# LCSL/nys-koop-lqr

Hardware: AMD Instinct MI355X
Metric: Nyström-Koopman fits/sec (K_nm build + A,B,C solve), N=1e5 m=2000 d=384 (higher is better)
Workload: dtype f64

## Files before the change

include/nyskoop.h:

```cpp
#ifndef NYSKOOP_H
#define NYSKOOP_H

#include <stdint.h>

#ifdef __cplusplus
extern "C" {
#endif

#define NK_ABI_VERSION 2

enum {
  NK_OK = 0,
  NK_ERR_BAD_ARG = -1,
  NK_ERR_HIP = -2,
  NK_ERR_NOT_SPD = -3,
  NK_ERR_OOM = -4,
  NK_ERR_NO_CONVERGENCE = -5,
  NK_ERR_NO_DEVICE = -6
};

enum { NK_KERNEL_RBF = 0, NK_KERNEL_MATERN52 = 1, NK_KERNEL_LINEAR = 2, NK_KERNEL_TPS = 3 };

typedef struct nk_kernel_desc {
  int32_t type;
  int32_t d;
  int32_t n_lengthscale;
  int32_t reserved;
  const double* lengthscale;
  double sigma0;
} nk_kernel_desc;

typedef struct nk_fit_stats {
  double ms_total;
  double ms_upload;
  double ms_kmat;
  double ms_gram;
  double ms_sqrt;
  double ms_solve;
  double ms_gram_kernel_avg;
  int32_t gram_kernel_launches;
  int32_t sqrt_iters;
  double sqrt_residual;
  double gram_flops;
  double kmat_pairs;
  int32_t rank_inner;
  int32_t rank_inner_rec;
  double pivot_ratio_inner;
  double pivot_ratio_inner_rec;
  int32_t refined;
  int32_t reserved_;
  double refine_ratio_inner;
  double refine_ratio_inner_rec;
} nk_fit_stats;

typedef struct nk_ctx nk_ctx;
typedef struct nk_model nk_model;

int nk_version(void);
const char* nk_last_error(void);
int nk_device_count(void);
int nk_create(int device, nk_ctx** out);
int nk_destroy(nk_ctx* ctx);
int nk_synchronize(nk_ctx* ctx);
void* nk_stream(nk_ctx* ctx);
int nk_set_kmat_mode(nk_ctx* ctx, int mode);
int nk_set_strict_spd(nk_ctx* ctx, int strict);
int nk_set_refine(nk_ctx* ctx, double pivot_ratio, int32_t steps);
#define NK_DTYPE_F64 0
#define NK_DTYPE_F32 1
int nk_set_compute_dtype(nk_ctx* ctx, int dtype);
int nk_wait_stream(nk_ctx* ctx, void* producer_stream);
int nk_group_create(int device, int size, nk_ctx** members);
typedef struct nk_cv_unit {
  const nk_kernel_desc* kernel;
  double gamma;
  double jitter;
  int32_t m;
  int32_t reserved;
  int64_t test_begin, test_end;
  const int64_t* landmark_rows;
} nk_cv_unit;
int nk_cv_grid(nk_ctx* const* members, int32_t n_members, const double* X, int64_t ldx, const double* Y, int64_t ldy,
               int64_t n, int32_t d, int32_t p, const nk_cv_unit* units, int32_t n_units, double* scores, int32_t* status);
typedef struct nk_spline_cv_unit {
  double gamma;
  int32_t m;
  int32_t reserved;
  int64_t test_begin, test_end;
  const double* centers;
} nk_spline_cv_unit;
int nk_spline_cv_grid(nk_ctx* const* members, int32_t n_members, const double* X, int64_t ldx, const double* Y,
                      int64_t ldy, int64_t n, int32_t d, int32_t p, const nk_spline_cv_unit* units, int32_t n_units,
                      double* scores, int32_t* status);
typedef struct nk_sysid_unit {
  const nk_kernel_desc* kernel;
  double gamma, jitter;
  int32_t m, n_ranges;
  const int64_t* row_ranges;
  const int64_t* landmark_rows;
  const double* centers;
  const int32_t* traj;
  int32_t n_traj, reserved;
} nk_sysid_unit;
int nk_sysid_grid(nk_ctx* const* members, int32_t n_members, const double* X, int64_t ldx, const double* Y, int64_t ldy,
                  int64_t n, int32_t d, int32_t p, const double* trajs, const double* U, int32_t n_trajs, int32_t T,
                  const nk_sysid_unit* units, int32_t n_units, double* err_abs, double* err_rel, int32_t* status);
int nk_group_enter(nk_ctx* member);
int nk_group_leave(nk_ctx* member);
int nk_group_stats(nk_ctx* member, uint64_t* out4);
int nk_runtime_counters(uint64_t* out, int32_t n);
int nk_shutdown(void);

void* nk_host_alloc(uint64_t bytes);
void nk_host_free(void* ptr);

int nk_kernel_matrix(nk_ctx* ctx, const nk_kernel_desc* kd,
                     const double* A, int64_t lda, int64_t nA,
                     const double* B, int64_t ldb, int64_t nB,
                     double* out, int64_t ldo);

int nk_nystrom_fit(nk_ctx* ctx, const nk_kernel_desc* kd,
                   const double* X, int64_t ldx, const double* Y, int64_t ldy,
                   int64_t n, int32_t d, int32_t p,
                   const int64_t* row_ranges, int32_t n_ranges,
                   const double* Zin, int64_t ldzi, const double* Zout, int64_t ldzo, int32_t m,
                   double gamma, double jitter,
                   nk_model** model, nk_fit_stats* stats);

int nk_gram_doubles(int32_t m, int32_t d, int32_t p, int64_t* count);
int nk_nystrom_gram(nk_ctx* ctx, const nk_kernel_desc* kd,
                    const double* X, int64_t ldx, const double* Y, int64_t ldy,
                    int64_t n, int32_t d, int32_t p,
                    const int64_t* row_ranges, int32_t n_ranges,
                    const double* Zin, int64_t ldzi, const double* Zout, int64_t ldzo, int32_t m,
                    double* gram, nk_fit_stats* stats);
// ... 100 lines not shown
```

nys_koop_lqr_amd/_lib.py:

```python
import atexit
import ctypes as C
import os
import sys
import threading

import numpy as np

_HERE = os.path.dirname(os.path.abspath(__file__))

NK_KERNEL_RBF, NK_KERNEL_MATERN52, NK_KERNEL_LINEAR, NK_KERNEL_TPS = 0, 1, 2, 3
NK_PLANT_DUFFING, NK_PLANT_DOUBLE_INTEGRATOR, NK_PLANT_HJB = 0, 1, 2
NK_OK = 0
_ERR_NAMES = {-1: "NK_ERR_BAD_ARG", -2: "NK_ERR_HIP", -3: "NK_ERR_NOT_SPD", -4: "NK_ERR_OOM",
              -5: "NK_ERR_NO_CONVERGENCE", -6: "NK_ERR_NO_DEVICE"}


class NyskoopError(RuntimeError):
    def __init__(self, code, msg):
        super().__init__(f"{_ERR_NAMES.get(code, code)}: {msg}")
        self.code = code


class KernelDesc(C.Structure):
    _fields_ = [("type", C.c_int32), ("d", C.c_int32), ("n_lengthscale", C.c_int32), ("reserved", C.c_int32),
                ("lengthscale", C.POINTER(C.c_double)), ("sigma0", C.c_double)]


class CvUnit(C.Structure):
    _fields_ = [("kernel", C.POINTER(KernelDesc)), ("gamma", C.c_double), ("jitter", C.c_double), ("m", C.c_int32),
                ("reserved", C.c_int32), ("test_begin", C.c_int64), ("test_end", C.c_int64),
                ("landmark_rows", C.POINTER(C.c_int64))]


class SplineCvUnit(C.Structure):
    _fields_ = [("gamma", C.c_double), ("m", C.c_int32), ("reserved", C.c_int32), ("test_begin", C.c_int64),
                ("test_end", C.c_int64), ("centers", C.POINTER(C.c_double))]


class SysidUnit(C.Structure):
    _fields_ = [("kernel", C.POINTER(KernelDesc)), ("gamma", C.c_double), ("jitter", C.c_double), ("m", C.c_int32),
                ("n_ranges", C.c_int32), ("row_ranges", C.POINTER(C.c_int64)), ("landmark_rows", C.POINTER(C.c_int64)),
                ("centers", C.POINTER(C.c_double)), ("traj", C.POINTER(C.c_int32)), ("n_traj", C.c_int32),
                ("reserved", C.c_int32)]


class PlantUnit(C.Structure):
    _fields_ = [("model", C.c_void_p), ("K", C.c_void_p), ("x0", C.c_void_p), ("x_ref", C.c_void_p),
                ("uopt", C.c_int32), ("reserved", C.c_int32)]


class DareProblem(C.Structure):
    _fields_ = [("m", C.c_int32), ("p", C.c_int32), ("A", C.c_void_p), ("lda", C.c_int64), ("B", C.c_void_p),
                ("ldb", C.c_int64), ("Q", C.c_void_p), ("ldq", C.c_int64), ("R", C.c_void_p), ("ldr", C.c_int64),
                ("out_K", C.c_void_p), ("out_P", C.c_void_p), ("out_delta", C.c_void_p)]


class FitStats(C.Structure):
    _fields_ = [("ms_total", C.c_double), ("ms_upload", C.c_double), ("ms_kmat", C.c_double),
                ("ms_gram", C.c_double), ("ms_sqrt", C.c_double), ("ms_solve", C.c_double),
                ("ms_gram_kernel_avg", C.c_double), ("gram_kernel_launches", C.c_int32),
                ("sqrt_iters", C.c_int32), ("sqrt_residual", C.c_double), ("gram_flops", C.c_double),
                ("kmat_pairs", C.c_double), ("rank_inner", C.c_int32), ("rank_inner_rec", C.c_int32),
                ("pivot_ratio_inner", C.c_double), ("pivot_ratio_inner_rec", C.c_double), ("refined", C.c_int32),
                ("reserved_", C.c_int32), ("refine_ratio_inner", C.c_double), ("refine_ratio_inner_rec", C.c_double)]

    def as_dict(self):
        return {k: getattr(self, k) for k, _ in self._fields_}


_P = C.c_void_p
_I64 = C.c_int64
_I32 = C.c_int32
_D = C.c_double

SIGNATURES = {
    "nk_version": (C.c_int, []),
    "nk_last_error": (C.c_char_p, []),
    "nk_device_count": (C.c_int, []),
    "nk_create": (C.c_int, [C.c_int, C.POINTER(_P)]),
    "nk_destroy": (C.c_int, [_P]),
    "nk_synchronize": (C.c_int, [_P]),
    "nk_stream": (_P, [_P]),
    "nk_set_kmat_mode": (C.c_int, [_P, C.c_int]),
    "nk_set_strict_spd": (C.c_int, [_P, C.c_int]),
    "nk_set_refine": (C.c_int, [_P, C.c_double, C.c_int32]),
    "nk_wait_stream": (C.c_int, [_P, _P]),
    "nk_shutdown": (C.c_int, []),
    "nk_group_create": (C.c_int, [C.c_int, C.c_int, C.POINTER(_P)]),
    "nk_group_enter": (C.c_int, [_P]),
    "nk_group_leave": (C.c_int, [_P]),
    "nk_set_compute_dtype": (C.c_int, [_P, C.c_int]),
    "nk_group_stats": (C.c_int, [_P, C.POINTER(C.c_uint64)]),
    "nk_runtime_counters": (C.c_int, [C.POINTER(C.c_uint64), C.c_int32]),
    "nk_cv_grid": (C.c_int, [C.POINTER(_P), _I32, _P, _I64, _P, _I64, _I64, _I32, _I32, C.POINTER(CvUnit), _I32,
                             C.POINTER(_D), C.POINTER(_I32)]),
    "nk_spline_cv_grid": (C.c_int, [C.POINTER(_P), _I32, _P, _I64, _P, _I64, _I64, _I32, _I32, C.POINTER(SplineCvUnit),
                                    _I32, C.POINTER(_D), C.POINTER(_I32)]),
    "nk_sysid_grid": (C.c_int, [C.POINTER(_P), _I32, _P, _I64, _P, _I64, _I64, _I32, _I32, _P, _P, _I32, _I32,
                                C.POINTER(SysidUnit), _I32, C.POINTER(_D), C.POINTER(_D), C.POINTER(_I32)]),
    "nk_host_alloc": (_P, [C.c_uint64]),
    "nk_host_free": (None, [_P]),
    "nk_kernel_matrix": (C.c_int, [_P, C.POINTER(KernelDesc), _P, _I64, _I64, _P, _I64, _I64, _P, _I64]),
    "nk_nystrom_fit": (C.c_int, [_P, C.POINTER(KernelDesc), _P, _I64, _P, _I64, _I64, _I32, _I32,
                                 C.POINTER(_I64), _I32, _P, _I64, _P, _I64, _I32, _D, _D,
                                 C.POINTER(_P), C.POINTER(FitStats)]),
    "nk_gram_doubles": (C.c_int, [_I32, _I32, _I32, C.POINTER(_I64)]),
    "nk_nystrom_gram": (C.c_int, [_P, C.POINTER(KernelDesc), _P, _I64, _P, _I64, _I64, _I32, _I32,
                                  C.POINTER(_I64), _I32, _P, _I64, _P, _I64, _I32, _P, C.POINTER(FitStats)]),
    "nk_nystrom_solve": (C.c_int, [_P, C.POINTER(KernelDesc), _P, _I64, _P, _I64, _I32, _I32, _I32, _P, _I64, _D, _D,
                                   C.POINTER(_P), C.POINTER(FitStats)]),
    "nk_model_create": (C.c_int, [_P, C.POINTER(KernelDesc), _P, _I64, _I32, _I32, _I32, _D, _P, _P, _P, _P,
                                  C.POINTER(_P)]),
    "nk_spline_fit": (C.c_int, [_P, _P, _I64, _P, _I64, _I64, _I32, _I32, C.POINTER(_I64), _I32, _P, _I64, _I32, _D,
                                C.POINTER(_P), C.POINTER(FitStats)]),
    "nk_spline_model_create": (C.c_int, [_P, _P, _I64, _I32, _I32, _I32, _P, _P, _P, _P, C.POINTER(_P)]),
    "nk_model_destroy": (C.c_int, [_P]),
    "nk_model_get": (C.c_int, [_P, _P, C.c_char, _P, _I64]),
    "nk_model_dims": (C.c_int, [_P, C.POINTER(_I32), C.POINTER(_I32), C.POINTER(_I32)]),
    "nk_model_get_ops": (C.c_int, [_P, _P, _P, _I64, _P, _I64, _P, _I64]),
    "nk_model_get_ops_async": (C.c_int, [_P, _P, _P, _I64, _P, _I64, _P, _I64]),
    "nk_model_wait": (C.c_int, [_P]),
    "nk_lift": (C.c_int, [_P, _P, _P, _I64, _I64, _P, _I64]),
    "nk_predict": (C.c_int, [_P, _P, _P, _I64, _I64, _P, _I64]),
    "nk_score_neg_rmse": (C.c_int, [_P, _P, _P, _I64, _P, _I64, _I64, C.POINTER(_D)]),
    "nk_rollout": (C.c_int, [_P, _P, _P, _I64, _P, _I32, _I32, _P, _P]),
    "nk_rollout_err": (C.c_int, [_P, _P, _P, _P, _I32, _I32, C.POINTER(_D), C.POINTER(_D)]),
    "nk_closed_loop": (C.c_int, [_P, _P, _P, _P, _P, _I32, _P, _P]),
    "nk_closed_loop_batch": (C.c_int, [_P, _P, _P, _P, _P, _I32, _I32, _P, _P]),
    "nk_plant_step": (C.c_int, [C.c_int, _D, _P, _P, _P]),
    "nk_plant_loop": (C.c_int, [_P, _P, C.c_int, _D, _P, _P, _P, _I32, _I32, _P, _P]),
    "nk_plant_loop_multi": (C.c_int, [_P, C.c_int, _D, _I32, C.POINTER(PlantUnit), _I32, _P, _I32, _P, _P, _P]),
    "nk_dare_batch": (C.c_int, [_P, C.POINTER(DareProblem), _I32, _D, _I32, C.POINTER(_I32), C.POINTER(_I32)]),
    "nk_model_lqr_gain_batch": (C.c_int, [_P, C.POINTER(_P), _I32, _D, _P, _D, _I32, _P, C.POINTER(_I32),
                                          C.POINTER(_I32)]),
    "nk_model_lqr_cost": (C.c_int, [_P, _P, _D, _P, _I64]),
    "nk_linear_rollout": (C.c_int, [_P, _P, _P, _P, _I32, _I32, _I32, _P, _P, _I32, _I32, _P, _P]),
    "nk_gemm_f32": (C.c_int, [_P, _I64, _I64, _I64, _P, _I64, _P, _I64, _P, _I64]),
    "nk_gemm": (C.c_int, [_P, C.c_int, C.c_int, _I64, _I64, _I64, _D, _P, _I64, _P, _I64, _D, _P, _I64]),
    "nk_sqrtm_spd": (C.c_int, [_P, _P, _I64, _I32, _P, _P, C.POINTER(_I32), C.POINTER(_D)]),
    "nk_solve_spd": (C.c_int, [_P, _P, _I64, _I32, _P, _I64, _I32, _P, _I64]),
    "nk_bench_gram": (C.c_int, [_P, _I64, _I32, _I32, _I32, _I32, C.POINTER(_D), C.POINTER(_D)]),
    "nk_chol_aug": (C.c_int, [_P, _I32, _P, _P, _P, _P, _P, _P, _P, _P, _P]),
}

_lib = None
_lib_lock = threading.Lock()

# ... 553 lines not shown
```

nys_koop_lqr_amd/csrc/nk_api.hip:

```cpp
#include "nk_common.h"
#include "nk_api_internal.h"

#include <cmath>
#include <cstdarg>
#include <cstdio>
#include <cstring>
#include <cstdlib>
#include <algorithm>
#include <mutex>
#include <set>

namespace nk {

static thread_local std::string g_err;

void set_error(const char* fmt, ...) {
  char buf[1024];
  va_list ap;
  va_start(ap, fmt);
  vsnprintf(buf, sizeof(buf), fmt, ap);
  va_end(ap);
  g_err = buf;
}

// ... 279 lines not shown
      NK_TRY(launch_gemm(ctx, false, true, len, d, p, 1.0, Xaug + r0 * ldx + d, ldx, mdl->W + m, m + p, 1.0,
                         out + r0 * ldo, ldo));
  }
  arena_release(ctx, mk);
  return NK_OK;
}


float ev_ms(nk_ctx* ctx, int a, int b) {
  float ms = 0.f;
  (void)hipEventElapsedTime(&ms, ctx->ev[a], ctx->ev[b]);
  return ms;
}


int small_reserve(nk_ctx* ctx, size_t bytes) {
  if (ctx->h_stage_bytes >= bytes) return NK_OK;
  if (ctx->h_stage) (void)hipHostFree(ctx->h_stage);
  ctx->h_stage = nullptr;
  ctx->h_stage_bytes = 0;
  NK_HIP(hipHostMalloc(reinterpret_cast<void**>(&ctx->h_stage), bytes, hipHostMallocDefault));
  ctx->h_stage_bytes = bytes;
  return NK_OK;
}
const double* small_in(SmallStage& st, const double* host, int64_t ld, int64_t rows, int64_t cols) {
  double* dst = reinterpret_cast<double*>(reinterpret_cast<char*>(st.ctx->h_stage) + st.off);
  for (int64_t r = 0; r < rows; ++r) memcpy(dst + r * cols, host + r * ld, (size_t)cols * 8);
  st.off += (((size_t)rows * cols * 8) + 255) & ~(size_t)255;
  return dst;
}
double* small_out(SmallStage& st, double* user, int64_t user_ld, int64_t rows, int64_t cols) {
  double* dst = reinterpret_cast<double*>(reinterpret_cast<char*>(st.ctx->h_stage) + st.off);
  st.off += (((size_t)rows * cols * 8) + 255) & ~(size_t)255;
  st.outs.push_back(SmallStage::Out{dst, user, user_ld, rows, cols});
  return dst;
}
void small_finish(SmallStage& st) {
  for (auto& o : st.outs)
    for (int64_t r = 0; r < o.rows; ++r) memcpy(o.user + r * o.user_ld, o.stage + r * o.cols, (size_t)o.cols * 8);
}

}

using namespace nk;

extern "C" {

int nk_version(void) { return NK_ABI_VERSION; }

const char* nk_last_error(void) { return g_err.c_str(); }

int nk_device_count(void) {
  int n = 0;
  if (hipGetDeviceCount(&n) != hipSuccess) {
    (void)hipGetLastError();
    return 0;
  }
  return n;
}

int nk_create(int device, nk_ctx** out) {
  NK_REQUIRE(out != nullptr, "nk_create: null output pointer");
  *out = nullptr;
  int n = nk_device_count();
  if (n <= 0) {
    set_error("no HIP device visible: libnyskoop has no CPU fallback");
    return NK_ERR_NO_DEVICE;
  }
  NK_REQUIRE(device >= 0 && device < n, "nk_create: device %d out of range (0..%d)", device, n - 1);
  NK_HIP(hipSetDevice(device));
  hipDeviceProp_t prop;
  NK_HIP(hipGetDeviceProperties(&prop, device));
  if (strncmp(prop.gcnArchName, "gfx950", 6) != 0) {
    set_error("device %d is %s; libnyskoop is built for gfx950 (MI355X) only", device, prop.gcnArchName);
    return NK_ERR_NO_DEVICE;
  }
  nk_ctx* ctx = new nk_ctx();
  ctx->device = device;
  ctx->num_cu = prop.multiProcessorCount;
  int prio_lo = 0, prio_hi = 0;
  NK_HIP(hipDeviceGetStreamPriorityRange(&prio_lo, &prio_hi));
  const int prio_mid = (prio_lo - prio_hi >= 2) ? (prio_lo + prio_hi) / 2 : prio_hi;
  NK_HIP(hipStreamCreateWithPriority(&ctx->stream_main, hipStreamNonBlocking, prio_mid));
  NK_HIP(hipStreamCreateWithPriority(&ctx->stream_side, hipStreamNonBlocking, prio_lo));
  NK_HIP(hipStreamCreateWithPriority(&ctx->stream_prep, hipStreamNonBlocking, prio_hi));
  NK_HIP(hipStreamCreateWithFlags(&ctx->stream_copy, hipStreamNonBlocking));
  NK_HIP(hipStreamCreateWithPriority(&ctx->stream_la[0], hipStreamNonBlocking, prio_hi));
  NK_HIP(hipStreamCreateWithPriority(&ctx->stream_la[1], hipStreamNonBlocking, prio_mid));
  for (int q = 0; q < 2; ++q)
    for (int i = 0; i < 4; ++i) NK_HIP(hipEventCreateWithFlags(&ctx->ev_la[q][i], hipEventDisableTiming));
  ctx->stream = ctx->stream_main;
  ctx->cur_arena = &ctx->arena;
  NK_HIP(hipEventCreateWithFlags(&ctx->ev_fork, hipEventDisableTiming));
  NK_HIP(hipEventCreateWithFlags(&ctx->ev_join, hipEventDisableTiming));
  NK_HIP(hipEventCreateWithFlags(&ctx->ev_chain, hipEventDisableTiming));
  NK_HIP(hipMalloc(reinterpret_cast<void**>(&ctx->d_info), 256));
  ctx->d_piv = reinterpret_cast<unsigned long long*>(ctx->d_info + 16);
  NK_HIP(hipMalloc(reinterpret_cast<void**>(&ctx->d_scalars), 64 * sizeof(double)));
  NK_HIP(hipHostMalloc(reinterpret_cast<void**>(&ctx->h_scalars), 64 * sizeof(double), hipHostMallocMapped | hipHostMallocCoherent));
  NK_HIP(hipHostMalloc(reinterpret_cast<void**>(&ctx->h_info), 256, hipHostMallocMapped | hipHostMallocCoherent));
  ctx->h_piv = reinterpret_cast<unsigned long long*>(ctx->h_info + 16);
  for (int i = 0; i < EV_COUNT; ++i) NK_HIP(hipEventCreate(&ctx->ev[i]));
  NK_HIP(hipEventCreateWithFlags(&ctx->ev_ext, hipEventDisableTiming));
  for (int i = 0; i < 8; ++i) NK_HIP(hipEventCreateWithFlags(&ctx->ev_up[i], hipEventDisableTiming));
  const char* km = getenv("NYSKOOP_KMAT");
  ctx->kmat_mode = (km && strcmp(km, "direct") == 0) ? 1 : 0;
  const char* st = getenv("NYSKOOP_STRICT_SPD");
  ctx->strict_spd = (st && atoi(st) != 0) ? 1 : 0;
  if (const char* rp = getenv("NYSKOOP_REFINE_PIVOT")) ctx->refine_pivot = atof(rp);
  if (const char* rs = getenv("NYSKOOP_REFINE_STEPS")) ctx->refine_steps = std::max(0, atoi(rs));
  {
    std::lock_guard<std::mutex> lk(g_reg_mu);
    g_ctxs.insert(ctx);
  }
  *out = ctx;
  return NK_OK;
}

static void destroy_ctx_unregistered(nk_ctx* ctx) {
  (void)hipSetDevice(ctx->device);
  if (tl_ctx == ctx) tl_ctx = nullptr;
  group_detach(ctx);
  (void)hipStreamSynchronize(ctx->stream_main);
  (void)hipStreamSynchronize(ctx->stream_side);
  (void)hipStreamSynchronize(ctx->stream_prep);
  (void)hipStreamSynchronize(ctx->stream_copy);
  for (int q = 0; q < 2; ++q) {
    if (ctx->stream_la[q]) { (void)hipStreamSynchronize(ctx->stream_la[q]); (void)hipStreamDestroy(ctx->stream_la[q]); }
    for (int i = 0; i < 4; ++i) if (ctx->ev_la[q][i]) (void)hipEventDestroy(ctx->ev_la[q][i]);
  }
  for (auto& c : ctx->arena.chunks) (void)hipFree(c.base);
  for (auto& c : ctx->arena_side.chunks) (void)hipFree(c.base);
  (void)hipEventDestroy(ctx->ev_fork);
  (void)hipEventDestroy(ctx->ev_join);
  if (ctx->ev_chain) (void)hipEventDestroy(ctx->ev_chain);
  if (ctx->ev_ext) (void)hipEventDestroy(ctx->ev_ext);
  for (int i = 0; i < 8; ++i) if (ctx->ev_up[i]) (void)hipEventDestroy(ctx->ev_up[i]);
  (void)hipStreamDestroy(ctx->stream_side);
  (void)hipStreamDestroy(ctx->stream_prep);
  (void)hipStreamDestroy(ctx->stream_copy);
  (void)hipFree(ctx->d_info);
  for (int i = 0; i < 2; ++i) if (ctx->d_flow[i]) (void)hipFree(ctx->d_flow[i]);
  (void)hipFree(ctx->d_scalars);
  if (ctx->d_zeros) (void)hipFree(ctx->d_zeros);
  if (ctx->h_stage) (void)hipHostFree(ctx->h_stage);
  (void)hipHostFree(ctx->h_scalars);
  (void)hipHostFree(ctx->h_info);
  for (int i = 0; i < EV_COUNT; ++i) (void)hipEventDestroy(ctx->ev[i]);
  (void)hipStreamDestroy(ctx->stream_main);
  delete ctx;
}

int nk_destroy(nk_ctx* ctx) {
  if (!ctx) return NK_OK;
  {
    std::lock_guard<std::mutex> lk(g_reg_mu);
    if (g_ctxs.erase(ctx) == 0) return NK_OK;
  }
  destroy_ctx_unregistered(ctx);
  return NK_OK;
}

static int model_wait_unchecked(nk_model* mdl);
static void destroy_model_unregistered(nk_model* model, bool to_pool) {
  (void)model_wait_unchecked(model);
  if (to_pool) {
    pool_give(model->device, model->bytes, model->buf);
// ... 705 lines not shown
```

nys_koop_lqr_amd/csrc/nk_chol_flow.hip:

```cpp
#include <cstdio>
#include <cstdlib>

#include "nk_common.h"
#include "nk_panel_body.h"
#include "nk_potrf_body.h"

namespace nk {

namespace {

constexpr int FLOW_THREADS = 256;
constexpr int FLOW_HDR = 16;
constexpr int FLOW_POLL_LIMIT = 1 << 22;

struct FlowSys {
  double* P;
  int64_t ldp;
  int m, extra;
  double* Linv;
  double* pivlog;
  int* info;
  unsigned long long* piv;
  int* flags;
  int nblk;
  int nex;
};
struct FlowArgs {
  FlowSys s[2];
  int nsys;
  int total;
  int fix;
  int test_giveup;
  int* hdr;
};

__device__ __forceinline__ int ld_flag(const int* f) { return __hip_atomic_load(f, __ATOMIC_RELAXED, __HIP_MEMORY_SCOPE_AGENT); }

__device__ __forceinline__ int col_items(const FlowSys& s, int c) {
  if (c < 0 || c >= s.nblk) return 0;
  return max(0, s.nblk - c - 2) + s.nex;
}

__device__ void item_of(const FlowArgs& a, int t, int& q, int& i, int& k) {
  for (int g = 0;; ++g) {
    for (int p = 0; p < a.nsys; ++p)
      if (g < a.s[p].nblk) {
        if (t == 0) { q = p; i = k = g; return; }
        --t;
      }
    for (int p = 0; p < a.nsys; ++p) {
      const int n = col_items(a.s[p], g - 1);
      if (t < n) {
        q = p; k = g - 1;
        const int nsq = max(0, a.s[p].nblk - k - 2);
        i = t < nsq ? k + 2 + t : a.s[p].nblk + (t - nsq);
        return;
      }
      t -= n;
    }
  }
}

__device__ __forceinline__ void tile_rows(const FlowSys& s, int i, int& r0, int& r1) {
  if (i < s.nblk) { r0 = CHOL_NB * i; r1 = min(r0 + CHOL_NB, s.m); }
  else { r0 = s.m + CHOL_NB * (i - s.nblk); r1 = min(r0 + CHOL_NB, s.m + s.extra); }
}

typedef d4 Quarter[2][2];

__device__ __forceinline__ void load_quarter(const FlowSys& s, int r0, int r1, int c0, int c1, int wm, int wn, int l15, int l4,
                                             Quarter& C) {
#pragma unroll
  for (int a = 0; a < 2; ++a)
#pragma unroll
    for (int b = 0; b < 2; ++b)
#pragma unroll
      for (int reg = 0; reg < 4; ++reg) {
        const int row = r0 + 32 * wm + 16 * a + l4 + 4 * reg, col = c0 + 32 * wn + 16 * b + l15;
        C[a][b][reg] = (row < r1 && col < c1) ? s.P[(int64_t)row * s.ldp + col] : 0.0;
      }
}
__device__ __forceinline__ void store_quarter(const FlowSys& s, int r0, int r1, int c0, int c1, int wm, int wn, int l15, int l4,
                                              const Quarter& C) {
#pragma unroll
  for (int a = 0; a < 2; ++a)
#pragma unroll
    for (int b = 0; b < 2; ++b)
#pragma unroll
      for (int reg = 0; reg < 4; ++reg) {
        const int row = r0 + 32 * wm + 16 * a + l4 + 4 * reg, col = c0 + 32 * wn + 16 * b + l15;
        if (row < r1 && col < c1) s.P[(int64_t)row * s.ldp + col] = C[a][b][reg];
      }
}

__device__ __forceinline__ void update_quarter(const FlowSys& s, int r0, int r1, int c0, int c1, int j, int wm, int wn, int l15,
                                               int l4, Quarter& C) {
  const double* pa[2];
  const double* pb[2];
#pragma unroll
  for (int a = 0; a < 2; ++a) {
    pa[a] = s.P + (int64_t)min(r0 + 32 * wm + 16 * a + l15, r1 - 1) * s.ldp + CHOL_NB * j + 8 * l4;
    pb[a] = s.P + (int64_t)min(c0 + 32 * wn + 16 * a + l15, c1 - 1) * s.ldp + CHOL_NB * j + 8 * l4;
  }
  d4 acc[2][2];
#pragma unroll
  for (int a = 0; a < 2; ++a)
#pragma unroll
    for (int b = 0; b < 2; ++b) acc[a][b] = d4{0.0, 0.0, 0.0, 0.0};
#pragma unroll
  for (int h = 0; h < 2; ++h) {
    double x[2][8], y[2][8];
#pragma unroll
    for (int a = 0; a < 2; ++a)
#pragma unroll
      for (int ks = 0; ks < 8; ++ks) {
        x[a][ks] = pa[a][32 * h + ks];
        y[a][ks] = pb[a][32 * h + ks];
      }
#pragma unroll
    for (int ks = 0; ks < 8; ++ks)
#pragma unroll
      for (int a = 0; a < 2; ++a)
#pragma unroll
        for (int b = 0; b < 2; ++b) acc[a][b] = __builtin_amdgcn_mfma_f64_16x16x4f64(x[a][ks], y[b][ks], acc[a][b], 0, 0, 0);
  }
#pragma unroll
  for (int a = 0; a < 2; ++a)
#pragma unroll
    for (int b = 0; b < 2; ++b)
#pragma unroll
      for (int reg = 0; reg < 4; ++reg) C[a][b][reg] -= acc[a][b][reg];
  asm volatile("" ::: "memory");
}

__device__ __forceinline__ void give_up(const FlowArgs& a) {
  __hip_atomic_store(a.hdr + 1, 1, __ATOMIC_RELAXED, __HIP_MEMORY_SCOPE_AGENT);
  for (int q = 0; q < a.nsys; ++q) atomicExch(a.s[q].info, CHOL_FLOW_GIVEUP);
}

__device__ int wait_tiles(const FlowArgs& a, const FlowSys& s, int ia, int ib, int jlo, int jhi, int* sh) {
  if (threadIdx.x < 64) {
    const int lane = threadIdx.x;
    int res = -1;
    for (int polls = 0;; ++polls) {
      const int j = jlo + lane;
      bool ok = true;
      if (j < jhi) {
        ok = ld_flag(s.flags + ia * s.nblk + j) != 0;
        if (ib >= 0) ok = ok && ld_flag(s.flags + ib * s.nblk + j) != 0;
      }
      const unsigned long long ready = __ballot(ok);
      const int run = ~ready == 0ull ? 64 : __builtin_ctzll(~ready);
      if (run > 0) { res = min(jlo + run, jhi); break; }
      if (ld_flag(a.hdr + 1) != 0) break;
      if (polls >= FLOW_POLL_LIMIT) {
        if (lane == 0) give_up(a);
        break;
      }
      __builtin_amdgcn_s_sleep(2);
    }
    if (lane == 0) {
      if (res > 0) __builtin_amdgcn_fence(__ATOMIC_ACQUIRE, "agent");
      asm volatile("s_waitcnt vmcnt(0)" ::: "memory");
      sh[0] = res;
    }
  }
  __syncthreads();
  const int r = sh[0];
  __syncthreads();
  return r;
}

__device__ __forceinline__ void publish(const FlowSys& s, int i, int k) {
  asm volatile("s_waitcnt vmcnt(0)" ::: "memory");
  __syncthreads();
  if (threadIdx.x == 0) {
    __builtin_amdgcn_fence(__ATOMIC_RELEASE, "agent");
    asm volatile("s_waitcnt vmcnt(0)" ::: "memory");
    __hip_atomic_store(s.flags + i * s.nblk + k, 1, __ATOMIC_RELAXED, __HIP_MEMORY_SCOPE_AGENT);
  }
}

__device__ __forceinline__ void local_sync() {
  asm volatile("s_waitcnt vmcnt(0)" ::: "memory");
  __syncthreads();
}

__device__ __forceinline__ void panel_tile(const FlowArgs& a, const FlowSys& s, int r0, int r1, int k, int wave, int lane) {
  PanelSys ps;
  ps.P = s.P + (int64_t)r0 * s.ldp + CHOL_NB * k;
  ps.ldp = s.ldp;
  ps.Linv = s.Linv + (size_t)k * CHOL_WS;
  ps.rows = r1 - r0;
  ps.nb = min(CHOL_NB, s.m - CHOL_NB * k);
  ps.fix = a.fix;
  ps.nblocks = 1;
  chol_panel_rows(ps, 16 * wave, lane);
  __builtin_amdgcn_s_setprio(0);
}

__device__ __noinline__ void flow_potrf(double* A, int64_t lda, int nb, double* Linv, int* info, unsigned long long* piv,
                                       double* plog, int blk, int lane) {
  PotrfBatch pb;
  pb.A[0] = A; pb.lda[0] = lda; pb.nb[0] = nb; pb.Linv[0] = Linv; pb.info[0] = info; pb.piv[0] = piv; pb.plog[0] = plog;
  pb.A[1] = nullptr; pb.lda[1] = 0; pb.nb[1] = 0; pb.Linv[1] = nullptr; pb.info[1] = nullptr; pb.piv[1] = nullptr;
  pb.plog[1] = nullptr;
  potrf_diag_kernel_body<true>(pb, blk, 0, lane);
  __builtin_amdgcn_s_setprio(0);
}

__global__ void __launch_bounds__(FLOW_THREADS) chol_flow_kernel(FlowArgs a) {
  __shared__ int sh[4];
  const int lane = threadIdx.x & 63;
  const int wave = __builtin_amdgcn_readfirstlane(threadIdx.x >> 6);
  const int wm = wave >> 1, wn = wave & 1;
  const int l15 = lane & 15, l4 = lane >> 4;
  for (;;) {
    if (threadIdx.x == 0) sh[1] = atomicAdd(a.hdr, 1);
    __syncthreads();
    const int t = sh[1];
    __syncthreads();
    if (t >= a.total) return;
    if (t == a.test_giveup) {
      if (threadIdx.x == 0) give_up(a);
      return;
    }
    int q = 0, i = 0, k = 0;
    item_of(a, t, q, i, k);
    const FlowSys s = q ? a.s[1] : a.s[0];
    int r0, r1;
    tile_rows(s, i, r0, r1);
    const int c0 = CHOL_NB * k, c1 = min(c0 + CHOL_NB, s.m);
    if (i == k) {
      if (k > 0) {
        const int p0 = c0 - CHOL_NB;
        Quarter Cp, Cd;
        load_quarter(s, r0, r1, p0, c0, wm, wn, l15, l4, Cp);
        load_quarter(s, r0, r1, c0, c1, wm, wn, l15, l4, Cd);
        bool ok = true;
        for (int j = 0; j < k - 1 && ok;) {
          const int J = wait_tiles(a, s, k, k - 1, j, k - 1, sh);
          if (J < 0) { ok = false; break; }
          for (; j < J; ++j) {
            update_quarter(s, r0, r1, p0, c0, j, wm, wn, l15, l4, Cp);
            update_quarter(s, r0, r1, c0, c1, j, wm, wn, l15, l4, Cd);
          }
        }
        if (!ok) continue;
        store_quarter(s, r0, r1, p0, c0, wm, wn, l15, l4, Cp);
        store_quarter(s, r0, r1, c0, c1, wm, wn, l15, l4, Cd);
        local_sync();
        if (wait_tiles(a, s, k - 1, -1, k - 1, k, sh) < 0) continue;
        panel_tile(a, s, r0, r1, k - 1, wave, lane);
        publish(s, k, k - 1);
        __syncthreads();
        load_quarter(s, r0, r1, c0, c1, wm, wn, l15, l4, Cd);
        update_quarter(s, r0, r1, c0, c1, k - 1, wm, wn, l15, l4, Cd);
        store_quarter(s, r0, r1, c0, c1, wm, wn, l15, l4, Cd);
        local_sync();
      }
      if (wave == 0)
        flow_potrf(s.P + (int64_t)c0 * s.ldp + c0, s.ldp, c1 - c0, s.Linv + (size_t)k * CHOL_WS, s.info, s.piv,
                   s.pivlog ? s.pivlog + c0 : nullptr, k, lane);
      publish(s, k, k);
      __syncthreads();
    } else {
      if (k > 0) {
        Quarter C;
        load_quarter(s, r0, r1, c0, c1, wm, wn, l15, l4, C);
        bool ok = true;
        for (int j = 0; j < k && ok;) {
          const int J = wait_tiles(a, s, i, k, j, k, sh);
          if (J < 0) { ok = false; break; }
          for (; j < J; ++j) update_quarter(s, r0, r1, c0, c1, j, wm, wn, l15, l4, C);
        }
        if (!ok) continue;
        store_quarter(s, r0, r1, c0, c1, wm, wn, l15, l4, C);
        local_sync();
      }
      if (wait_tiles(a, s, k, -1, k, k + 1, sh) < 0) continue;
      panel_tile(a, s, r0, r1, k, wave, lane);
      publish(s, i, k);
      __syncthreads();
    }
  }
}

}

bool chol_flow_enabled() {
  const char* e = getenv("NYSKOOP_CHOL_FLOW");
  return !(e && e[0] == '0');
}

static int flow_test_giveup(const CholSys* sys, int nsys, int total) {
  const char* e = getenv("NYSKOOP_CHOL_FLOW_TEST_GIVEUP");
  if (!e || !e[0]) return -1;
  long ticket = -1, want_nsys = 0, want_extra = 0;
  if (sscanf(e, "%ld,%ld,%ld", &ticket, &want_nsys, &want_extra) < 1) return -1;
  if (want_nsys > 0 && want_nsys != nsys) return -1;
  if (want_extra > 0 && want_extra != sys[0].extra) return -1;
  return (ticket >= 0 && ticket < total) ? (int)ticket : -1;
}

int cholesky_flow_pair(nk_ctx* ctx, const CholSys* sys, int nsys) {
  constexpr int NB = CHOL_NB;
  NK_REQUIRE(nsys >= 1 && nsys <= 2, "cholesky_flow_pair: 1..2 systems");
  FlowArgs a;
  memset(&a, 0, sizeof(a));
  a.nsys = nsys;
  a.fix = chol_fix_enabled();
  size_t words = FLOW_HDR;
  for (int q = 0; q < nsys; ++q) {
    const CholSys& y = sys[q];
    FlowSys& s = a.s[q];
    s.P = y.P; s.ldp = y.ldp; s.m = y.m; s.extra = y.extra; s.Linv = y.Linv; s.pivlog = y.pivlog;
    s.info = ctx->d_info + info_base(ctx) + q;
    s.piv = ctx->d_piv + 2 * (info_base(ctx) + q);
    s.nblk = (y.m + NB - 1) / NB;
    s.nex = (y.extra + NB - 1) / NB;
    words += (size_t)(s.nblk + s.nex) * s.nblk;
    for (int c = 0; c < s.nblk; ++c) a.total += 1 + std::max(0, s.nblk - c - 2) + s.nex;
  }
  const int slot = info_base(ctx) / 2;
  if (ctx->flow_words[slot] < words) {
    if (ctx->d_flow[slot]) NK_HIP(hipFree(ctx->d_flow[slot]));
    ctx->d_flow[slot] = nullptr;
    ctx->flow_words[slot] = 0;
    NK_HIP(hipMalloc(reinterpret_cast<void**>(&ctx->d_flow[slot]), words * sizeof(int)));
    ctx->flow_words[slot] = words;
  }
  a.test_giveup = flow_test_giveup(sys, nsys, a.total);
  a.hdr = ctx->d_flow[slot];
  int* f = a.hdr + FLOW_HDR;
  for (int q = 0; q < nsys; ++q) {
    a.s[q].flags = f;
    f += (size_t)(a.s[q].nblk + a.s[q].nex) * a.s[q].nblk;
  }
  NK_HIP(hipMemsetAsync(a.hdr, 0, words * sizeof(int), ctx->stream));
  const int grid = std::max(1, std::min(a.total, ctx->num_cu / 2));
  hipLaunchKernelGGL(chol_flow_kernel, dim3((unsigned)grid), dim3(FLOW_THREADS), 0, ctx->stream, a);
  NK_HIP(hipGetLastError());
  count_event(CNT_CHOL_FLOW);
  return NK_OK;
}

}
```

nys_koop_lqr_amd/csrc/nk_common.h:

```cpp
#pragma once
#include <hip/hip_runtime.h>
#include <stdint.h>
#include <stddef.h>
#include <string>
#include <vector>

#include "nyskoop.h"
#include "nk_lockstep.h"

namespace nk {

void set_error(const char* fmt, ...);

#define NK_HIP(call)                                                                         \
  do {                                                                                       \
    hipError_t e_ = (call);                                                                  \
    if (e_ != hipSuccess) {                                                                  \
      nk::set_error("%s failed: %s (%s:%d)", #call, hipGetErrorString(e_), __FILE__, __LINE__); \
      return e_ == hipErrorOutOfMemory ? NK_ERR_OOM : NK_ERR_HIP;                            \
    }                                                                                        \
  } while (0)

#define NK_TRY(call)            \
  do {                          \
    int rc_ = (call);           \
    if (rc_ != NK_OK) return rc_; \
  } while (0)

#define NK_REQUIRE(cond, ...)     \
  do {                            \
    if (!(cond)) {                \
      nk::set_error(__VA_ARGS__); \
      return NK_ERR_BAD_ARG;      \
    }                             \
  } while (0)

struct ArenaChunk {
  char* base = nullptr;
  size_t cap = 0;
  size_t off = 0;
};
struct Arena {
  std::vector<ArenaChunk> chunks;
  int cur = 0;
};
struct ArenaMark {
  int chunk;
  size_t off;
};

}

enum {
  EV_FIT_BEGIN = 0,
  EV_STAGED = 1,
  EV_KMAT_DONE = 2,
  EV_GRAM_DONE = 3,
  EV_SOLVE_BEGIN = 4,
  EV_FIT_END = 5,
  EV_SQRT_BEGIN = 6,
  EV_SQRT_END = 7,
  EV_LANDMARKS = 8,
  EV_SQRT_PREPARED = 9,
  EV_SQRT_RESID = 10,
  EV_SQRT_SCALARS = 11,
  EV_FORK = 12,
  EV_YPREP_DONE = 13,
  EV_GEMM_T0 = 14,
  EV_GEMM_T1 = 15,
  EV_COUNT = 16
};

struct nk_member_state;
struct nk_ctx {
  int device = 0;
  hipStream_t stream = nullptr;
  hipStream_t stream_main = nullptr;
  hipStream_t stream_side = nullptr;
  hipStream_t stream_copy = nullptr;
  hipStream_t stream_prep = nullptr;
  nk::Arena arena;
  nk::Arena arena_side;
  nk::Arena* cur_arena = nullptr;
  hipStream_t stream_la[2] = {nullptr, nullptr};
  hipEvent_t ev_la[2][4] = {};
  int compute_f32 = 0;
  hipEvent_t ev_fork = nullptr, ev_join = nullptr, ev_chain = nullptr;
  int* d_info = nullptr;
  unsigned long long* d_piv = nullptr;
  unsigned long long* h_piv = nullptr;
  double* d_scalars = nullptr;
  double* h_scalars = nullptr;
  int* h_info = nullptr;
  double* d_zeros = nullptr;
  hipEvent_t ev[EV_COUNT];
  int num_cu = 256;
  int kmat_mode = 0;
  double refine_pivot = 0.0;
  int refine_steps = 2;
  int strict_spd = 0;
  hipEvent_t ev_ext = nullptr;
  hipEvent_t ev_up[8] = {};
  nk_group* group = nullptr;
  nk_member_state* gstate = nullptr;
  int* d_flow[2] = {nullptr, nullptr};
  size_t flow_words[2] = {0, 0};
  bool spline_defer_svd = false;
  bool chol_flow_off = false;
  double* h_stage = nullptr;
  size_t h_stage_bytes = 0;
};

enum { NK_MODEL_NYSTROM = 0, NK_MODEL_SPLINE = 1 };
struct nk_model {
  int device = 0;
  int32_t m = 0, d = 0, p = 0;
  int32_t ktype = 0;
  double sigma0 = 0.0;
  double jitter = 0.0;
  double* buf = nullptr;
  size_t bytes = 0;
  double *A = nullptr, *B = nullptr, *C = nullptr, *W = nullptr, *S = nullptr, *Sinv = nullptr, *Z = nullptr,
         *winv = nullptr;
  bool has_ops = false;
  int32_t kind = 0;
  hipEvent_t ev_fetch = nullptr;
};

namespace nk {

struct SideScope {
  nk_ctx* c;
  hipStream_t s0;
  Arena* a0;
  explicit SideScope(nk_ctx* ctx, hipStream_t s = nullptr) : c(ctx), s0(ctx->stream), a0(ctx->cur_arena) {
    c->stream = s ? s : c->stream_side;
    c->cur_arena = &c->arena_side;
  }
  ~SideScope() {
    c->stream = s0;
    c->cur_arena = a0;
  }
};

struct ChainOnly {
  nk_ctx* c;
  bool b0;
  explicit ChainOnly(nk_ctx* ctx) : c(ctx), b0(ctx->chol_flow_off) { c->chol_flow_off = true; }
  ~ChainOnly() { c->chol_flow_off = b0; }
};

inline int info_base(const nk_ctx* c) { return c->stream != c->stream_main ? 2 : 0; }

// ... 51 lines not shown
  if ((0x000fffff & (2 + hx)) < 3) {
    if (f == 0.0) return k == 0 ? 0.0 : dk * ln2_hi + dk * ln2_lo;
    const double R = f * f * (0.5 - 0.33333333333333333 * f);
    return k == 0 ? f - R : dk * ln2_hi - ((R - dk * ln2_lo) - f);
  }
  const double s = f / (2.0 + f);
  const double z = s * s;
  const double w = z * z;
  const double t1 = w * (Lg2 + w * (Lg4 + w * Lg6));
  const double t2 = z * (Lg1 + w * (Lg3 + w * (Lg5 + w * Lg7)));
  const double R = t2 + t1;
  if (((hx - 0x6147a) | (0x6b851 - hx)) > 0) {
    const double hfsq = 0.5 * f * f;
    return k == 0 ? f - (hfsq - s * (hfsq + R)) : dk * ln2_hi - ((hfsq - (s * (hfsq + R) + dk * ln2_lo)) - f);
  }
  return k == 0 ? f - s * (f - R) : dk * ln2_hi - ((s * (f - R) - dk * ln2_lo) - f);
}
__host__ __device__ __forceinline__ double tps_value(double r2) {
#pragma clang fp contract(off)
  return r2 > 0.0 ? r2 * log_pos(sqrt(r2)) : 0.0;
}

nk_group* group_new(int device, int size);
void group_attach(nk_group* g, int slot, nk_ctx* c);
void group_detach(nk_ctx* c);
int group_enter(nk_ctx* c);
int group_leave(nk_ctx* c);
void group_stats(nk_ctx* c, uint64_t out[4]);
enum { CNT_CHAIN_GIVEUP = 0, CNT_JACOBI_GIVEUP = 1, CNT_RANK_TRUNCATED = 2, CNT_SQRT_RETRY = 3, CNT_REFINED = 4,
       CNT_CHOL_FLOW_GIVEUP = 5, CNT_CHOL_FLOW = 6, CNT_N = 7 };
void count_event(int which);
uint64_t read_counter(int which);
hipError_t real_stream_sync(hipStream_t s);
hipError_t real_event_sync(hipEvent_t e);

int arena_reset(nk_ctx* ctx);
ArenaMark arena_mark(nk_ctx* ctx);
void arena_release(nk_ctx* ctx, ArenaMark mk);
int arena_alloc(nk_ctx* ctx, size_t bytes, void** out);
template <typename T>
inline int arena_alloc_t(nk_ctx* ctx, size_t count, T** out) {
  return arena_alloc(ctx, count * sizeof(T), reinterpret_cast<void**>(out));
}
bool is_device_ptr(const void* p);

int launch_kmat(nk_ctx* ctx, int ktype, const double* A, int64_t lda, int64_t nA, const double* B, int64_t ldb,
                int64_t nB, int d, const double* winv, double sigma0, double* out, int64_t ldo);

enum { TRI_FULL = 0, TRI_UPPER_MIRROR = 1, TRI_LOWER = 2 };
struct GemmOpts {
  int tri = TRI_FULL;
  int splitk = 0;
};
int launch_gemm(nk_ctx* ctx, bool transA, bool transB, int64_t M, int64_t N, int64_t K, double alpha, const double* A,
                int64_t lda, const double* B, int64_t ldb, double beta, double* C, int64_t ldc,
                const GemmOpts& opts = GemmOpts(), float* ms_kernel = nullptr);

struct GemmCall {
  int64_t M = 0, N = 0, K = 0;
  double alpha = 1.0, beta = 0.0;
  const double* A = nullptr;
  const double* B = nullptr;
  double* C = nullptr;
  int64_t lda = 0, ldb = 0, ldc = 0;
  GemmOpts opts;
};
int launch_gemm_pair(nk_ctx* ctx, bool transA, bool transB, const GemmCall* calls, int ncalls);

struct TnSkip;
int launch_add_diag(nk_ctx* ctx, double* A, int64_t lda, int n, double v);
int launch_copy2d(nk_ctx* ctx, const double* src, int64_t lds, double* dst, int64_t ldd, int64_t rows, int64_t cols);
int launch_axpby2d(nk_ctx* ctx, double a, const double* X, int64_t ldx, double b, double* Y, int64_t ldy,
                   int64_t rows, int64_t cols);
int launch_scale_add_identity(nk_ctx* ctx, double a, const double* X, int64_t ldx, double c, double* Y, int64_t ldy,
                              int n, const TnSkip* skip = nullptr);
int launch_fill(nk_ctx* ctx, double* A, int64_t lda, int64_t rows, int64_t cols, double v);
int launch_frob_minus_identity(nk_ctx* ctx, const double* M, int64_t ldm, int n, double* d_out,
                               const TnSkip* skip = nullptr);
int launch_max_abs_rowsum(nk_ctx* ctx, const double* M, int64_t ldm, int n, double* d_out);
int launch_colsum_sqdiff(nk_ctx* ctx, const double* P, int64_t ldp, const double* Y, int64_t ldy, int64_t rows,
                         int cols, double* d_colsum);

int sqrtm_spd(nk_ctx* ctx, const double* P, int64_t ldp, int m, double* S, double* Sinv, int* iters, double* resid);
struct SqrtPlan {
  const double* P = nullptr;
  int64_t ldp = 0;
  int m = 0;
  double* W = nullptr;
  double* Linv = nullptr;
  double* X0 = nullptr;
  double* X0t = nullptr;
  double* d_sc = nullptr;
  ArenaMark mark{0, 0};
  bool deferred = false;
  int rc = 0, iters = 0, kmax = 0;
  double resid = 0.0;
  double lambda_min_hint = 0.0;
  bool early = false;
  int info_slot = 2;
  bool flow_gave_up = false;
  hipEvent_t pause_event = nullptr;
  int pause_step = -1;
};
constexpr int NK_SQRT_RETRY = 1;
int sqrtm_spd_coupled(nk_ctx* ctx, const double* P, int64_t ldp, int m, double* S, double* Sinv, int* iters, double* resid);
int sqrtm_prepare(nk_ctx* ctx, const double* P, int64_t ldp, int m, SqrtPlan* plan);
int sqrtm_finish(nk_ctx* ctx, SqrtPlan* plan, double* S, double* Sinv);
int sqrtm_verdict(nk_ctx* ctx, SqrtPlan* plan, int* iters, double* resid);
int cholesky_lower(nk_ctx* ctx, double* P, int64_t ldp, int m, double* Linv );
int cholesky_solve(nk_ctx* ctx, const double* L, int64_t ldl, int m, const double* Linv, double* R, int64_t ldr,
                   int nrhs);
struct CholSys {
  double* P = nullptr;
  int64_t ldp = 0;
  int m = 0;
  int extra = 0;
  bool backward = true;
  double* Linv = nullptr;
  double* pivlog = nullptr;
  double* R = nullptr;
  int64_t ldr = 0;
  int nrhs = 0;
};
int cholesky_lower_pair(nk_ctx* ctx, const CholSys* sys, int nsys);
int cholesky_lower_pair_async(nk_ctx* ctx, const CholSys* sys, int nsys);
int cholesky_check_pair(nk_ctx* ctx, const CholSys* sys, int nsys);
int cholesky_solve_pair(nk_ctx* ctx, const CholSys* sys, int nsys);
int cholesky_aug_pair_async(nk_ctx* ctx, const CholSys* sys, int nsys, hipEvent_t pause = nullptr, int pause_step = -1);
constexpr int CHOL_NB = 64;
constexpr int CHOL_WS = 2 * CHOL_NB * CHOL_NB + 8;
constexpr double CHOL_FIX_KAPPA = 8.0 * CHOL_NB;
inline int chol_fix_enabled() {
  const char* e = getenv("NYSKOOP_CHOL_FIX");
  return (e && e[0] == '0') ? 0 : ((e && e[0] == '2') ? 2 : 1);
}
bool launch_chol_trail_pair(nk_ctx* ctx, const GemmCall* calls, int ncalls, int* rc);
bool launch_chol_trail_potrf_pair(nk_ctx* ctx, const GemmCall* calls, int ncalls, const int* nb, double* const* Linv, int blk,
                                  double* const* plog, int* rc);
inline bool chol_fuse_enabled() {
  const char* e = getenv("NYSKOOP_CHOL_FUSE");
  return !(e && e[0] == '0');
}
bool chol_flow_enabled();
int cholesky_flow_pair(nk_ctx* ctx, const CholSys* sys, int nsys);
constexpr int CHOL_FLOW_GIVEUP = -0x40000000;
bool launch_chol_panel_pair(nk_ctx* ctx, const GemmCall* calls, int ncalls, int* rc);
int launch_trsm_right_lower_pair(nk_ctx* ctx, const CholSys* sys, int nsys);

struct PinvInfo {
  int rank = 0, sweeps = 0;
  bool converged = false;
  double sigma_max = 0.0, sigma_min_kept = 0.0, sigma_min = 0.0;
};
int pinv_right_divide(nk_ctx* ctx, const double* P, int64_t ldp, int m, const double* E, int64_t lde, int rows,
                      double* E_out, int64_t ldeo, double rcond, PinvInfo* info);
int cholesky_fail_flags(nk_ctx* ctx, const CholSys* sys, int nsys, int* failed , double* piv_ratio = nullptr);

int launch_lifted_step(nk_ctx* ctx, const double* G, int64_t ldg, int m, int mz, int pu, const double* z, int64_t zstride,
                       const double* u, int64_t ustride, const double* bias, double* out, int64_t ostride, int batch);

struct ChainArgs {
  const double* G = nullptr; int64_t ldg = 0; int m = 0, pu = 0;
  const double* z0 = nullptr; int64_t z0_stride = 0;
  bool lift = false;
  const double* x0 = nullptr; int64_t x0_stride = 0;
  const double* Zl = nullptr; int d = 0; const double* winv = nullptr; const double* Sinv = nullptr; int ktype = 0;
  double sigma0 = 0.0;
  const double* U = nullptr; int64_t u_stride = 0;
  const double* bias = nullptr; int64_t bias_stride = 0;
  double* Zall = nullptr; int64_t z_stride = 0;
  int T = 0, batch = 0;
};
int launch_ref_minus_traj(nk_ctx* ctx, const double* ref, int64_t ref_stride, const double* Phi, int64_t phi_stride,
                          double* D, int64_t d_stride, int steps, int m, int batch);
bool lifted_chain_ok(int m, int pu, int d_lift);
int traj_err_tile(int m);
int launch_traj_err(nk_ctx* ctx, const double* Zall, int64_t z_stride, const double* Cop, int64_t ldc, const double* Xtrue,
                    int64_t x_stride, int m, int d, int T, int batch, double* out);
int launch_lifted_chain(nk_ctx* ctx, const ChainArgs& a);
bool lifted_chain_mw_ok(const nk_ctx* ctx, int m, int pu);
int chain_mw_workgroups(int m);
int chain_mw_group(int m, int batch);
int launch_lifted_chain_mw(nk_ctx* ctx, const ChainArgs& a);
int lifted_chain_mw_reset(nk_ctx* ctx);
int lifted_chain_mw_fetch_status(nk_ctx* ctx);
bool lifted_chain_mw_timed_out(nk_ctx* ctx, int* row, int* step, int* traj);

int plant_loop_max_m();
int launch_plant_loop(nk_ctx* ctx, const nk_model* mdl, int plant, double Ts, const double* w, const double* x0,
                      int64_t x0_stride, const double* xref, int64_t xref_stride, int steps, int batch, double* out_x,
                      int64_t ldx, double* out_u, int64_t ldu);
struct PlantLoopUnit {
  const double* Z;
  const double* winv;
  const double* w;
  const double* x0;
  const double* xref;
  double* out_x;
  double* out_u;
  const double* u_opt;
  double* score;
  int64_t ldx, ldu;
  double sigma0sq;
  int m, reserved;
};
int launch_plant_loop_multi(nk_ctx* ctx, int plant, double Ts, int steps, PlantLoopUnit* units, const int* ktypes,
                            int n_units);

constexpr int DARE_MAX_M = 256;
constexpr int DARE_MAX_P = 8;
struct DareRec {
  const double* A; int64_t lda;
  const double* B; int64_t ldb;
  const double* Q; int64_t ldq;
  const double* C; int64_t ldc;
  const double* R;
  double c;
  double* ws;
  double* outK;
  double* outP;
  double* delta;
  int* status;
  int* iters;
  int m, p, M, d;
  int q_only;
  int reserved;
};
inline int dare_pad(int m) { return (m + 15) & ~15; }
inline size_t dare_ws_doubles(int M) { return (size_t)7 * M * M; }
int launch_dare(nk_ctx* ctx, const DareRec* table_dev, int count, double tol, int max_iter);

}

namespace nk {
enum { KTRIM_NONE = 0, KTRIM_B_UPPER = 1 , KTRIM_A_LOWER = 2  };
struct TnProblem {
  const double* A = nullptr;
  const double* B = nullptr;
  double* C = nullptr;
  int64_t lda = 0, ldb = 0, ldc = 0;
  int M = 0, N = 0;
  int tri = TRI_FULL;
  int ktrim = 0;
  double alpha = 1.0, beta = 0.0;
  double* Ct = nullptr;
  int64_t ldct = 0;
  const double* A_even = nullptr;
  const double* B_even = nullptr;
  double* Caff = nullptr;
  double aff_a = 0.0, aff_c = 0.0;
};
struct TnSkip {
  const double* state = nullptr;
  int step = 0;
  const double* select = nullptr;
  double* resid_partials = nullptr;
  int* resid_count = nullptr;
};
bool tn_fast_ok(const TnProblem& p);
struct TnProblemF {
  const float* A = nullptr;
  const float* B = nullptr;
  double* C = nullptr;
  int64_t lda = 0, ldb = 0, ldc = 0;
  int M = 0, N = 0;
  int tri = TRI_FULL;
  double beta = 0.0;
};
bool tnf_fast_ok(const TnProblemF& p);
int launch_gemm_tn_f32_multi(nk_ctx* ctx, const TnProblemF* probs, int nprob, int64_t K, int splitk ,
                             float* ms_kernel = nullptr, bool sync_timing = true);
int prep_rows_f32(nk_ctx* ctx, const double* X, int64_t ldx, int64_t rows, int d, const double* winv, const double* center,
                  float* Xt, int64_t ldt, float* sq);
int launch_cvt_f64_f32(nk_ctx* ctx, const double* src, int64_t lds_, float* dst, int64_t ldd, int64_t rows, int cols);
int launch_kmat_gram_f32(nk_ctx* ctx, int ktype, const float* At, int64_t ldat, const float* sqa, int64_t nA, const float* Bt,
                         int64_t ldbt, const float* sqb, int64_t nB, int d, double sigma0, float* out, int64_t ldo);
int launch_gemm_tn_multi(nk_ctx* ctx, const TnProblem* probs, int nprob, int64_t K, int splitk ,
                         float* ms_kernel = nullptr, bool sync_timing = true, const TnSkip* skip = nullptr);
int launch_transpose(nk_ctx* ctx, const double* src, int64_t lds, double* dst, int64_t ldd, int rows, int cols);
constexpr int refine_partial_blocks() { return 512; }
int launch_refine_apply(nk_ctx* ctx, const double* dX, int64_t ldd, double* X, int64_t ldx, int64_t rows, int64_t cols, int step,
                        double* state, double* partial);
int launch_resid_dd(nk_ctx* ctx, const double* X, int64_t ldx, const double* P, int64_t ldp, const double* R, int64_t ldr,
                    double* Res, int64_t ldres, int nr, int mq);
int launch_colmean(nk_ctx* ctx, const double* Z, int64_t ldz, int rows, int d, double* mean);
int prep_rows(nk_ctx* ctx, const double* X, int64_t ldx, int64_t rows, int d, const double* winv, const double* center,
              double* Xt, int64_t ldt, double* sq);
int launch_kmat_gram(nk_ctx* ctx, int ktype, const double* At, int64_t ldat, const double* sqa, int64_t nA,
                     const double* Bt, int64_t ldbt, const double* sqb, int64_t nB, int d, double sigma0, double* out,
                     int64_t ldo);
}

#if defined(__HIPCC__)
namespace nk {
typedef unsigned chain_u2 __attribute__((ext_vector_type(2)));
template <int CTRL> __device__ __forceinline__ double dpp_f64(double v) {
  int lo = __double2loint(v), hi = __double2hiint(v);
  lo = __builtin_amdgcn_update_dpp(0, lo, CTRL, 0xf, 0xf, true);
  hi = __builtin_amdgcn_update_dpp(0, hi, CTRL, 0xf, 0xf, true);
  return __hiloint2double(hi, lo);
}
__device__ __forceinline__ void swap16_f64(double& a, double& b) {
  const chain_u2 lo = __builtin_amdgcn_permlane16_swap((unsigned)__double2loint(a), (unsigned)__double2loint(b), false, false);
  const chain_u2 hi = __builtin_amdgcn_permlane16_swap((unsigned)__double2hiint(a), (unsigned)__double2hiint(b), false, false);
  a = __hiloint2double((int)hi.x, (int)lo.x);
  b = __hiloint2double((int)hi.y, (int)lo.y);
}
__device__ __forceinline__ void swap32_f64(double& a, double& b) {
  const chain_u2 lo = __builtin_amdgcn_permlane32_swap((unsigned)__double2loint(a), (unsigned)__double2loint(b), false, false);
  const chain_u2 hi = __builtin_amdgcn_permlane32_swap((unsigned)__double2hiint(a), (unsigned)__double2hiint(b), false, false);
  a = __hiloint2double((int)hi.x, (int)lo.x);
  b = __hiloint2double((int)hi.y, (int)lo.y);
}
__device__ __forceinline__ double wave_sum64_dpp(double c) {
  c += dpp_f64<0xB1>(c);
  c += dpp_f64<0x4E>(c);
  c += dpp_f64<0x141>(c);
  c += dpp_f64<0x140>(c);
  double a = c, b = c;
  swap16_f64(a, b);
  c = a + b;
  a = c; b = c;
  swap32_f64(a, b);
  return a + b;
}

__device__ __forceinline__ double chain_kfun(int ktype, double acc, double sigma0sq) {
  if (ktype == NK_KERNEL_RBF) return exp_nonpos(-0.5 * acc);
  if (ktype == NK_KERNEL_MATERN52) {
    const double t = sqrt(acc) * 2.23606797749978969641;
    return (1.0 + t + t * t / 3.0) * exp_nonpos(-t);
  }
  return acc + sigma0sq;
}

}
#endif
```

nys_koop_lqr_amd/csrc/nk_fit.hip:

```cpp
#include "nk_common.h"
#include "nk_api_internal.h"

#include <cmath>
#include <cstring>
#include <cstdlib>
#include <algorithm>
#include <initializer_list>

using namespace nk;

static inline size_t gram_block1(int m, int p) { return (((size_t)(2 * m + p) * (m + p)) + 1) & ~(size_t)1; }
static inline size_t gram_doubles(int m, int d, int p) { return gram_block1(m, p) + (size_t)(m + d) * m; }


static int select_rows(const char* who, const int64_t* row_ranges, int32_t n_ranges, int64_t n, std::vector<int64_t>* rng,
                       int64_t* n_eff) {
  if (row_ranges && n_ranges > 0) {
    for (int i = 0; i < n_ranges; ++i) {
      const int64_t b = row_ranges[2 * i], e = row_ranges[2 * i + 1];
      NK_REQUIRE(0 <= b && b <= e && e <= n, "%s: row range %d = [%lld,%lld) outside [0,%lld)", who, i, (long long)b,
                 (long long)e, (long long)n);
      if (e > b) { rng->push_back(b); rng->push_back(e); }
    }
  } else {
    rng->push_back(0); rng->push_back(n);
  }
  *n_eff = 0;
  for (size_t i = 0; i < rng->size(); i += 2) *n_eff += (*rng)[i + 1] - (*rng)[i];
  NK_REQUIRE(*n_eff > 0, "%s: no training rows selected", who);
  return NK_OK;
}

static int gather_ranges(nk_ctx* ctx, int d, int p, int64_t n_eff, std::vector<int64_t>* rng, MatIn* x, MatIn* y) {
  if (!(rng->size() > 2 && (double)n_eff * (2.0 * d + p) * 8.0 <= 256e6)) return NK_OK;
  const int64_t ldxg = (d + p + 1) & ~(int64_t)1, ldyg = (d + 1) & ~(int64_t)1;
  double *xg = nullptr, *yg = nullptr;
  NK_TRY(arena_alloc_t(ctx, (size_t)n_eff * ldxg, &xg));
  NK_TRY(arena_alloc_t(ctx, (size_t)n_eff * ldyg, &yg));
  int64_t o = 0;
  for (size_t i = 0; i < rng->size(); i += 2) {
    const int64_t b = (*rng)[i], len = (*rng)[i + 1] - (*rng)[i];
    NK_TRY(launch_copy2d(ctx, x->ptr + b * x->ld, x->ld, xg + o * ldxg, ldxg, len, d + p));
    NK_TRY(launch_copy2d(ctx, y->ptr + b * y->ld, y->ld, yg + o * ldyg, ldyg, len, d));
    o += len;
  }
  x->ptr = xg; x->ld = ldxg; y->ptr = yg; y->ld = ldyg;
  rng->assign({(int64_t)0, n_eff});
  return NK_OK;
}

static int64_t pass_rows_for(int64_t ldf, double bytes_per_elem) {
  const char* b = getenv("NYSKOOP_F_BUDGET_GB");
  const double budget = (b ? atof(b) : 48.0) * 1073741824.0;
  int64_t pass_rows = (int64_t)(budget / ((double)ldf * bytes_per_elem));
  if (pass_rows < 1024) pass_rows = 1024;
  return pass_rows & ~(int64_t)1023;
}

struct Piece { int64_t b, len; };
static std::vector<std::vector<Piece>> plan_passes(const std::vector<int64_t>& rng, int64_t pass_rows) {
  std::vector<std::vector<Piece>> passes(1);
  int64_t used = 0;
  for (size_t i = 0; i < rng.size(); i += 2) {
    int64_t b = rng[i];
    const int64_t e = rng[i + 1];
    while (b < e) {
      if (used == pass_rows) { passes.emplace_back(); used = 0; }
      const int64_t len = std::min(e - b, pass_rows - used);
      passes.back().push_back(Piece{b, len});
      used += len;
      b += len;
    }
  }
  return passes;
}

struct KernelBlocks {
  int ktype = 0;
  double sigma0 = 0.0;
  int d = 0, p = 0, m = 0;
  const double* winv = nullptr;
  bool gram_form = false;
  MatIn zi, zo;
  double *center = nullptr, *Rt = nullptr, *sqr = nullptr, *Zto = nullptr, *sqzo = nullptr, *Zti = nullptr, *sqzi = nullptr;
  int64_t ldt = 0, ldzt = 0;
  int64_t ldf = 0, off_out = 0;
  int copy_inputs(nk_ctx* ctx, const double* xs, int64_t ldx, int64_t len, double* Fo) const {
    if (p > 0) NK_TRY(launch_copy2d(ctx, xs + d, ldx, Fo + m, ldf, len, p));
    return NK_OK;
  }
  int piece(nk_ctx* ctx, const double* xs, int64_t ldx, const double* ys, int64_t ldy, int64_t len, double* Fo) const {
    if (gram_form) {
      NK_TRY(prep_rows(ctx, xs, ldx, len, d, winv, center, Rt, ldt, sqr));
      NK_TRY(launch_kmat_gram(ctx, ktype, Rt, ldt, sqr, len, Zti, ldzt, sqzi, m, d, sigma0, Fo, ldf));
      NK_TRY(prep_rows(ctx, ys, ldy, len, d, winv, center, Rt, ldt, sqr));
      NK_TRY(launch_kmat_gram(ctx, ktype, Rt, ldt, sqr, len, Zto, ldzt, sqzo, m, d, sigma0, Fo + off_out, ldf));
    } else {
      NK_TRY(launch_kmat(ctx, ktype, xs, ldx, len, zi.ptr, zi.ld, m, d, winv, sigma0, Fo, ldf));
      NK_TRY(launch_kmat(ctx, ktype, ys, ldy, len, zo.ptr, zo.ld, m, d, winv, sigma0, Fo + off_out, ldf));
    }
    return copy_inputs(ctx, xs, ldx, len, Fo);
  }
};

static void fill_gram_stats(nk_ctx* ctx, nk_fit_stats* stats, bool staged, bool gram_deferred, float ms_gram_kernel,
                            int gram_launches) {
  memset(stats, 0, sizeof(*stats));
  stats->ms_upload = staged ? ev_ms(ctx, EV_FIT_BEGIN, EV_STAGED) : 0.0;
  stats->ms_kmat = ev_ms(ctx, EV_STAGED, EV_KMAT_DONE);
  stats->ms_gram = ev_ms(ctx, EV_KMAT_DONE, EV_GRAM_DONE);
  if (gram_deferred) ms_gram_kernel = ev_ms(ctx, EV_GEMM_T0, EV_GEMM_T1);
  stats->ms_gram_kernel_avg = gram_launches ? ms_gram_kernel / gram_launches : 0.0;
  stats->gram_kernel_launches = gram_launches;
}

struct FitGuard {
  nk_model* m = nullptr;
  hipStream_t s[5] = {};
  int ns = 0;
  void arm(nk_model* mdl, std::initializer_list<hipStream_t> streams) {
    m = mdl;
    for (hipStream_t q : streams) s[ns++] = q;
  }
  ~FitGuard() {
    if (m) {
      for (int i = 0; i < ns; ++i) (void)hipStreamSynchronize(s[i]);
      nk_model_destroy(m);
    }
  }
};


enum { FIT_FULL = 0, FIT_GRAM = 1, FIT_SOLVE = 2 };

struct NystromFit {
  nk_ctx* ctx; const nk_kernel_desc* kd;
  const double* X; int64_t ldx; const double* Y; int64_t ldy; int64_t n; int32_t d, p;
  const int64_t* row_ranges; int32_t n_ranges;
  const double* Zin; int64_t ldzi; const double* Zout; int64_t ldzo; int32_t m;
  double gamma, jitter; nk_model** model; nk_fit_stats* stats; int mode; double* gram_io;
  HostTrace tr;
  std::vector<int64_t> rng;
  int64_t n_eff = 0;
  bool same_centers = false;
  int mp = 0;
  double gamma_n = 0.0;
  nk_model* mdl = nullptr;
  FitGuard guard;
  MatIn x, y, zi, zo;
  int host_passes = 1;
  double *Kmm = nullptr, *Kj = nullptr, *Kj_in = nullptr, *Kxo = nullptr;
  bool landmarks_aside = false;
  double *G1 = nullptr, *G2 = nullptr, *G3 = nullptr, *G4 = nullptr;
  int64_t ldd = 0;
  float ms_gram_kernel = 0.f;
  int gram_launches = 0;
  bool gram_deferred = false, timed = false;
  bool f32 = false, overlap_prep = false, multi_pass = false, pipelined = false;
  KernelBlocks kb;
  std::vector<std::vector<Piece>> passes;
  int64_t f_rows = 0, maxlen = 0, ldt32 = 0, ldzt32 = 0, ldy32 = 0;
  double *F = nullptr, *Rt2 = nullptr, *sqr2 = nullptr;
  float *F32 = nullptr, *Rt32 = nullptr, *sq32 = nullptr, *Zt32 = nullptr, *sqz32 = nullptr, *Y32 = nullptr;
  SqrtPlan splan;
  int it = 0;
  double resid = 0.0;
  double *Sinvt = nullptr, *T1t = nullptr, *X1 = nullptr;
  double *Gsave = nullptr, *V1 = nullptr, *Wc = nullptr, *Ct = nullptr;
  CholSys sys[2];
  int chol_failed[2] = {0, 0}, rank_sys[2] = {0, 0}, refined[2] = {0, 0};
  double piv_ratio[2] = {1.0, 1.0}, refine_ratio[2] = {0.0, 0.0};
  bool redo_products = false;

  int run();
  int validate(), stage_rows(), stage_landmarks(), landmark_matrices(), alloc_gram(), load_gram(), prepare_features(), run_passes();
  int upload_pass(size_t ip), pass_f32(size_t ip), pass_f64(size_t ip), blocks_overlapped(const Piece& pc, double* Fo);
  int return_gram();
  int queue_sqrt_prep(), assemble_and_factor(), queue_sqrt_side(), sqrt_products(), operator_products();
  int settle_factorisations(), refine(), settle_sqrt();
  void read_refinement(), write_stats();
};

int NystromFit::validate() {
  NK_TRY(check_ctx(ctx));
  tr.mark("check_ctx/arena_reset");
  NK_REQUIRE(kd && Zout, "nk_nystrom_fit: null argument");
  NK_REQUIRE(mode == FIT_SOLVE || (X && Y), "nk_nystrom_fit: null data pointer");
  NK_REQUIRE(mode == FIT_GRAM || model != nullptr, "nk_nystrom_fit: null model pointer");
  NK_REQUIRE(mode == FIT_FULL || gram_io != nullptr, "nk_nystrom_gram/solve: null accumulator");
  NK_REQUIRE(n > 0 && d > 0 && p >= 0 && m > 0, "nk_nystrom_fit: sizes must be positive (n=%lld d=%d p=%d m=%d)",
             (long long)n, d, p, m);
  NK_REQUIRE(mode == FIT_SOLVE || (ldx >= d + p && ldy >= d), "nk_nystrom_fit: leading dimension too small");
  NK_REQUIRE(ldzo >= d, "nk_nystrom_fit: leading dimension too small");
  NK_REQUIRE(std::isfinite(gamma) && std::isfinite(jitter), "nk_nystrom_fit: gamma/jitter not finite");
  NK_REQUIRE(kd->type != NK_KERNEL_TPS, "nk_nystrom_fit: the thin-plate spline has no Nystrom fit (nk_spline_fit)");
  if (model) *model = nullptr;
  NK_TRY(select_rows("nk_nystrom_fit", row_ranges, n_ranges, n, &rng, &n_eff));
  same_centers = (Zin == nullptr) || (Zin == Zout && ldzi == ldzo);
  mp = m + p;
  gamma_n = gamma * (double)n_eff;

  NK_TRY(model_alloc(ctx, m, d, p, &mdl));
  guard.arm(mdl, {ctx->stream_main, ctx->stream_side, ctx->stream_prep, ctx->stream_la[0], ctx->stream_la[1]});
  mdl->ktype = kd->type; mdl->sigma0 = kd->sigma0; mdl->jitter = jitter;
  tr.mark("validate + model_alloc");
  return NK_OK;
}

int NystromFit::stage_rows() {
  const char* e = getenv("NYSKOOP_HOST_PASSES");
  const int want = e ? atoi(e) : 6;
  if (want > 1 && rng.size() == 2 && !ctx_recording(ctx) && (double)n_eff * (2.0 * d + p) * 8.0 >= 64e6 &&
      !is_device_ptr(X) && !is_device_ptr(Y))
    host_passes = want > 8 ? 8 : want;
  if (host_passes > 1) {
    x.ld = (d + p + 1) & ~(int64_t)1;
    y.ld = (d + 1) & ~(int64_t)1;
    double *xd = nullptr, *yd = nullptr;
    NK_TRY(arena_alloc_t(ctx, (size_t)n * x.ld, &xd));
    NK_TRY(arena_alloc_t(ctx, (size_t)n * y.ld, &yd));
    x.ptr = xd; y.ptr = yd; x.staged = y.staged = true;
  } else {
    NK_TRY(stage_in(ctx, X, ldx, n, d + p, &x));
    NK_TRY(stage_in(ctx, Y, ldy, n, d, &y));
  }
  return gather_ranges(ctx, d, p, n_eff, &rng, &x, &y);
}

int NystromFit::stage_landmarks() {
  NK_TRY(stage_in(ctx, Zout, ldzo, m, d, &zo));
  if (same_centers) zi = zo; else NK_TRY(stage_in(ctx, Zin, ldzi, m, d, &zi));
  NK_TRY(launch_copy2d(ctx, zo.ptr, zo.ld, mdl->Z, d, m, d));
  NK_HIP(hipEventRecord(ctx->ev[EV_STAGED], ctx->stream));
  tr.mark("staging issued");
  return NK_OK;
}

int NystromFit::landmark_matrices() {
  NK_TRY(arena_alloc_t(ctx, (size_t)m * m, &Kmm));
  NK_TRY(arena_alloc_t(ctx, (size_t)m * m, &Kj));
  if (same_centers) {
    Kj_in = Kj;
    Kxo = Kmm;
  } else {
    NK_TRY(arena_alloc_t(ctx, (size_t)m * m, &Kj_in));
    NK_TRY(arena_alloc_t(ctx, (size_t)m * m, &Kxo));
  }
  {
    const char* la = getenv("NYSKOOP_LANDMARKS_ASIDE");
    landmarks_aside = mode == FIT_FULL && n_eff >= 20000 && m >= 1024 && !ctx_recording(ctx) && !(la && la[0] == '0');
  }
  hipStream_t s0 = ctx->stream;
  if (landmarks_aside) {
    NK_HIP(hipEventRecord(ctx->ev[EV_FORK], ctx->stream));
    ctx->stream = ctx->stream_prep;
    NK_HIP(hipStreamWaitEvent(ctx->stream, ctx->ev[EV_FORK], 0));
  }
  int rc_l = launch_kmat(ctx, kd->type, zo.ptr, zo.ld, m, zo.ptr, zo.ld, m, d, mdl->winv, kd->sigma0, Kmm, m);
  if (rc_l == NK_OK) rc_l = launch_copy2d(ctx, Kmm, m, Kj, m, m, m);
  if (rc_l == NK_OK) rc_l = launch_add_diag(ctx, Kj, m, m, jitter);
// ... 51 lines not shown
      NK_TRY(arena_alloc_t(ctx, (size_t)d * kb.ldt, &kb.Rt));
      NK_TRY(arena_alloc_t(ctx, (size_t)maxlen, &kb.sqr));
    }
    if (overlap_prep && !f32) {
      NK_TRY(arena_alloc_t(ctx, (size_t)d * kb.ldt, &Rt2));
      NK_TRY(arena_alloc_t(ctx, (size_t)maxlen, &sqr2));
    }
    NK_TRY(arena_alloc_t(ctx, (size_t)d * kb.ldzt, &kb.Zto));
    NK_TRY(arena_alloc_t(ctx, (size_t)m, &kb.sqzo));
    if (kd->type == NK_KERNEL_LINEAR) NK_TRY(launch_fill(ctx, kb.center, d, 1, d, 0.0));
    else NK_TRY(launch_colmean(ctx, zo.ptr, zo.ld, m, d, kb.center));
    NK_TRY(prep_rows(ctx, zo.ptr, zo.ld, m, d, mdl->winv, kb.center, kb.Zto, kb.ldzt, kb.sqzo));
    if (same_centers) {
      kb.Zti = kb.Zto; kb.sqzi = kb.sqzo;
    } else {
      NK_TRY(arena_alloc_t(ctx, (size_t)d * kb.ldzt, &kb.Zti));
      NK_TRY(arena_alloc_t(ctx, (size_t)m, &kb.sqzi));
      NK_TRY(prep_rows(ctx, zi.ptr, zi.ld, m, d, mdl->winv, kb.center, kb.Zti, kb.ldzt, kb.sqzi));
    }
  }
  F32 = reinterpret_cast<float*>(F);
  ldt32 = (maxlen + 3) & ~(int64_t)3; ldzt32 = (m + 3) & ~3; ldy32 = (d + 3) & ~3;
  if (f32) {
    NK_REQUIRE(same_centers, "fp32 engine: separate input landmarks are not supported");
    double* tmp = nullptr;
    NK_TRY(arena_alloc_t(ctx, ((size_t)d * ldt32 + 1) / 2 + 2, &tmp)); Rt32 = reinterpret_cast<float*>(tmp);
    NK_TRY(arena_alloc_t(ctx, ((size_t)maxlen + 1) / 2 + 2, &tmp)); sq32 = reinterpret_cast<float*>(tmp);
    NK_TRY(arena_alloc_t(ctx, ((size_t)d * ldzt32 + 1) / 2 + 2, &tmp)); Zt32 = reinterpret_cast<float*>(tmp);
    NK_TRY(arena_alloc_t(ctx, ((size_t)m + 1) / 2 + 2, &tmp)); sqz32 = reinterpret_cast<float*>(tmp);
    NK_TRY(arena_alloc_t(ctx, ((size_t)f_rows * ldy32 + 1) / 2 + 2, &tmp)); Y32 = reinterpret_cast<float*>(tmp);
    NK_TRY(prep_rows_f32(ctx, zo.ptr, zo.ld, m, d, mdl->winv, kb.center, Zt32, ldzt32, sqz32));
  }
  multi_pass = passes.size() > 1;
  pipelined = host_passes > 1;
  return NK_OK;
}

int NystromFit::upload_pass(size_t ip) {
  for (const Piece& pc : passes[ip]) {
    NK_HIP(hipMemcpy2DAsync(const_cast<double*>(x.ptr) + pc.b * x.ld, (size_t)x.ld * 8, X + pc.b * ldx, (size_t)ldx * 8,
                            (size_t)(d + p) * 8, (size_t)pc.len, hipMemcpyHostToDevice, ctx->stream_side));
    NK_HIP(hipMemcpy2DAsync(const_cast<double*>(y.ptr) + pc.b * y.ld, (size_t)y.ld * 8, Y + pc.b * ldy, (size_t)ldy * 8,
                            (size_t)d * 8, (size_t)pc.len, hipMemcpyHostToDevice, ctx->stream_side));
  }
  NK_HIP(hipEventRecord(ctx->ev_up[ip & 7], ctx->stream_side));
  return NK_OK;
}

int NystromFit::run_passes() {
  if (pipelined) {
    NK_HIP(hipEventRecord(ctx->ev[EV_FORK], ctx->stream));
    NK_HIP(hipStreamWaitEvent(ctx->stream_side, ctx->ev[EV_FORK], 0));
    NK_TRY(upload_pass(0));
  }
  for (size_t ip = 0; ip < passes.size(); ++ip) {
    if (pipelined) NK_HIP(hipStreamWaitEvent(ctx->stream, ctx->ev_up[ip & 7], 0));
    NK_TRY(f32 ? pass_f32(ip) : pass_f64(ip));
    if (pipelined && ip + 1 < passes.size()) NK_TRY(upload_pass(ip + 1));
  }
  return NK_OK;
}

int NystromFit::pass_f32(size_t ip) {
  const std::vector<Piece>& ps = passes[ip];
  const double beta = ip == 0 ? 0.0 : 1.0;
  const int64_t ldf = kb.ldf, off_out = kb.off_out;
  int64_t o32 = 0;
  for (const Piece& pc : ps) {
    const double* xs = x.ptr + pc.b * x.ld;
    const double* ys = y.ptr + pc.b * y.ld;
    NK_TRY(prep_rows_f32(ctx, xs, x.ld, pc.len, d, mdl->winv, kb.center, Rt32, ldt32, sq32));
    NK_TRY(launch_kmat_gram_f32(ctx, kd->type, Rt32, ldt32, sq32, pc.len, Zt32, ldzt32, sqz32, m, d, kd->sigma0,
                                F32 + o32 * ldf, ldf));
    NK_TRY(prep_rows_f32(ctx, ys, y.ld, pc.len, d, mdl->winv, kb.center, Rt32, ldt32, sq32));
    NK_TRY(launch_kmat_gram_f32(ctx, kd->type, Rt32, ldt32, sq32, pc.len, Zt32, ldzt32, sqz32, m, d, kd->sigma0,
                                F32 + o32 * ldf + off_out, ldf));
    if (p > 0) NK_TRY(launch_cvt_f64_f32(ctx, xs + d, x.ld, F32 + o32 * ldf + m, ldf, pc.len, p));
    NK_TRY(launch_cvt_f64_f32(ctx, ys, y.ld, Y32 + o32 * ldy32, ldy32, pc.len, d));
    o32 += pc.len;
  }
  if (ip == 0) {
    NK_HIP(hipEventRecord(ctx->ev[EV_KMAT_DONE], ctx->stream));
    tr.mark("kmat issued");
  }
  TnProblemF pf[4];
  pf[0].A = F32; pf[0].B = F32; pf[0].lda = pf[0].ldb = ldf; pf[0].M = pf[0].N = mp; pf[0].C = G1; pf[0].ldc = mp;
  pf[0].tri = TRI_UPPER_MIRROR;
  pf[1].A = F32 + off_out; pf[1].B = F32; pf[1].lda = pf[1].ldb = ldf; pf[1].M = m; pf[1].N = mp; pf[1].C = G2; pf[1].ldc = mp;
  pf[2].A = F32 + off_out; pf[2].B = F32 + off_out; pf[2].lda = pf[2].ldb = ldf; pf[2].M = pf[2].N = m; pf[2].C = G3;
  pf[2].ldc = m; pf[2].tri = TRI_UPPER_MIRROR;
  pf[3].A = Y32; pf[3].lda = ldy32; pf[3].M = d; pf[3].N = m; pf[3].C = G4; pf[3].ldc = m; pf[3].B = F32 + off_out;
  pf[3].ldb = ldf;
  for (int q = 0; q < 4; ++q) pf[q].beta = beta;
  float ms1 = 0.f;
  NK_TRY(launch_gemm_tn_f32_multi(ctx, pf, 4, o32, 0, timed ? &ms1 : nullptr, multi_pass));
  if (multi_pass) ms_gram_kernel += ms1; else gram_deferred = timed;
  gram_launches += 1;
  return NK_OK;
}

int NystromFit::blocks_overlapped(const Piece& pc, double* Fo) {
  const double* xs = x.ptr + pc.b * x.ld;
  const double* ys = y.ptr + pc.b * y.ld;
  NK_HIP(hipEventRecord(ctx->ev[EV_FORK], ctx->stream));
  {
    SideScope side(ctx);
    NK_HIP(hipStreamWaitEvent(ctx->stream, ctx->ev[EV_FORK], 0));
    NK_TRY(prep_rows(ctx, ys, y.ld, pc.len, d, mdl->winv, kb.center, Rt2, kb.ldt, sqr2));
    NK_HIP(hipEventRecord(ctx->ev[EV_YPREP_DONE], ctx->stream));
  }
  NK_TRY(prep_rows(ctx, xs, x.ld, pc.len, d, mdl->winv, kb.center, kb.Rt, kb.ldt, kb.sqr));
  NK_TRY(launch_kmat_gram(ctx, kd->type, kb.Rt, kb.ldt, kb.sqr, pc.len, kb.Zti, kb.ldzt, kb.sqzi, m, d, kd->sigma0, Fo, kb.ldf));
  NK_HIP(hipStreamWaitEvent(ctx->stream, ctx->ev[EV_YPREP_DONE], 0));
  NK_TRY(launch_kmat_gram(ctx, kd->type, Rt2, kb.ldt, sqr2, pc.len, kb.Zto, kb.ldzt, kb.sqzo, m, d, kd->sigma0,
                          Fo + kb.off_out, kb.ldf));
  return kb.copy_inputs(ctx, xs, x.ld, pc.len, Fo);
}

int NystromFit::pass_f64(size_t ip) {
  const std::vector<Piece>& ps = passes[ip];
  const double beta = ip == 0 ? 0.0 : 1.0;
  const int64_t ldf = kb.ldf, off_out = kb.off_out;
  int64_t o = 0;
  for (const Piece& pc : ps) {
    if (overlap_prep) NK_TRY(blocks_overlapped(pc, F + o * ldf));
    else NK_TRY(kb.piece(ctx, x.ptr + pc.b * x.ld, x.ld, y.ptr + pc.b * y.ld, y.ld, pc.len, F + o * ldf));
    o += pc.len;
  }
  const int64_t rows = o;
  if (ip == 0) {
    NK_HIP(hipEventRecord(ctx->ev[EV_KMAT_DONE], ctx->stream));
    tr.mark("kmat issued");
  }
  TnProblem pr[4];
  pr[0].A = F; pr[0].B = F; pr[0].lda = pr[0].ldb = ldf; pr[0].M = pr[0].N = mp; pr[0].C = G1; pr[0].ldc = mp;
  pr[0].tri = TRI_UPPER_MIRROR;
  pr[1].A = F + off_out; pr[1].B = F; pr[1].lda = pr[1].ldb = ldf; pr[1].M = m; pr[1].N = mp; pr[1].C = G2;
  pr[1].ldc = mp;
  pr[2].A = F + off_out; pr[2].B = F + off_out; pr[2].lda = pr[2].ldb = ldf; pr[2].M = pr[2].N = m; pr[2].C = G3;
  pr[2].ldc = m; pr[2].tri = TRI_UPPER_MIRROR;
  pr[3].A = y.ptr + ps[0].b * y.ld; pr[3].lda = y.ld; pr[3].M = d; pr[3].N = m; pr[3].C = G4; pr[3].ldc = m;
  pr[3].B = F + off_out; pr[3].ldb = ldf;
  for (int q = 0; q < 4; ++q) pr[q].beta = beta;
  const bool single = ps.size() == 1;
  const bool fast = tn_fast_ok(pr[0]) && tn_fast_ok(pr[1]) && tn_fast_ok(pr[2]);
  const bool fast_y = fast && tn_fast_ok(pr[3]);
  bool y_done = false;
  if (fast) {
    const int np = (single && fast_y) ? 4 : 3;
    float ms1 = 0.f;
    NK_TRY(launch_gemm_tn_multi(ctx, pr, np, rows, 0, (timed && !pipelined) ? &ms1 : nullptr, multi_pass));
    if (multi_pass) ms_gram_kernel += ms1; else gram_deferred = timed;
    gram_launches += 1;
    y_done = np == 4;
  } else {
    GemmOpts sym;
    sym.tri = TRI_UPPER_MIRROR;
    float t3[3] = {0.f, 0.f, 0.f};
    NK_TRY(launch_gemm(ctx, true, false, mp, mp, rows, 1.0, F, ldf, F, ldf, beta, G1, mp, sym, timed ? &t3[0] : nullptr));
    NK_TRY(launch_gemm(ctx, true, false, m, mp, rows, 1.0, F + off_out, ldf, F, ldf, beta, G2, mp, GemmOpts(),
                       timed ? &t3[1] : nullptr));
    NK_TRY(launch_gemm(ctx, true, false, m, m, rows, 1.0, F + off_out, ldf, F + off_out, ldf, beta, G3, m, sym,
                       timed ? &t3[2] : nullptr));
    ms_gram_kernel += t3[0] + t3[1] + t3[2];
    gram_launches += 3;
  }
  if (!y_done) {
    int64_t oo = 0;
    bool first = true;
    for (const Piece& pc : ps) {
      NK_TRY(launch_gemm(ctx, true, false, d, m, pc.len, 1.0, y.ptr + pc.b * y.ld, y.ld, F + oo * ldf + off_out, ldf,
                         (first && ip == 0) ? 0.0 : 1.0, G4, m));
      oo += pc.len;
      first = false;
    }
  }
  return NK_OK;
}

int NystromFit::return_gram() {
  NK_HIP(hipMemcpyAsync(gram_io, G1, gram_doubles(m, d, p) * sizeof(double),
                        is_device_ptr(gram_io) ? hipMemcpyDeviceToDevice : hipMemcpyDeviceToHost, ctx->stream));
  NK_HIP(hipStreamSynchronize(ctx->stream));
  if (stats) {
    fill_gram_stats(ctx, stats, x.staged || y.staged, gram_deferred, ms_gram_kernel, gram_launches);
    stats->ms_total = ev_ms(ctx, EV_FIT_BEGIN, EV_GRAM_DONE);
  }
  if (ctx->arena.chunks.size() > 1 || ctx->arena_side.chunks.size() > 1) NK_TRY(arena_reset(ctx));
  return NK_OK;
}


int NystromFit::sqrt_products() {
  NK_TRY(launch_transpose(ctx, mdl->Sinv, m, Sinvt, m, m, m));
  if (same_centers) {
    NK_TRY(launch_copy2d(ctx, mdl->S, m, T1t, m, m, m));
    NK_TRY(launch_axpby2d(ctx, -jitter, mdl->Sinv, m, 1.0, T1t, m, m, m));
  } else {
    NK_TRY(launch_transpose(ctx, Kxo, m, X1, m, m, m));
    NK_TRY(launch_gemm(ctx, true, false, m, m, m, 1.0, X1, m, mdl->Sinv, m, 0.0, T1t, m));
  }
  return NK_OK;
}

int NystromFit::queue_sqrt_prep() {
  SideScope prep(ctx, ctx->stream_prep);
  NK_HIP(hipStreamWaitEvent(ctx->stream, ctx->ev[EV_LANDMARKS], 0));
  splan.lambda_min_hint = jitter > 0.0 ? jitter : 0.0;
  if (mode == FIT_FULL && n_eff >= 20000 && m >= 1024) {
    static const double frac = getenv("NYSKOOP_PREP_PAUSE") ? atof(getenv("NYSKOOP_PREP_PAUSE")) : 0.0;
    const int nb = (m + CHOL_NB - 1) / CHOL_NB;
    if (frac < 1.0) {
      splan.pause_event = ctx->ev_fork;
      splan.pause_step = std::max(0, std::min(nb - 1, (int)(frac * nb)));
    }
  }
  NK_TRY(sqrtm_prepare(ctx, Kj, m, m, &splan));
  NK_HIP(hipEventRecord(ctx->ev[EV_SQRT_PREPARED], ctx->stream));
  return NK_OK;
}

int NystromFit::assemble_and_factor() {
  if (landmarks_aside) NK_HIP(hipStreamWaitEvent(ctx->stream, ctx->ev[EV_LANDMARKS], 0));
  NK_TRY(launch_axpby2d(ctx, gamma_n, Kj_in, m, 1.0, G1, mp, m, m));
  if (p > 0) NK_TRY(launch_add_diag(ctx, G1 + (int64_t)m * mp + m, mp, p, gamma_n));
  NK_TRY(launch_axpby2d(ctx, gamma_n, Kj, m, 1.0, G3, m, m, m));
  NK_TRY(arena_alloc_t(ctx, gram_doubles(m, d, p), &Gsave));
  NK_HIP(hipMemcpyAsync(Gsave, G1, gram_doubles(m, d, p) * sizeof(double), hipMemcpyDeviceToDevice, ctx->stream));
  double *Linv = nullptr, *Linv2 = nullptr, *pivlog = nullptr;
  const int nblk = (mp + CHOL_NB - 1) / CHOL_NB;
  NK_TRY(arena_alloc_t(ctx, (size_t)nblk * CHOL_WS, &Linv));
  NK_TRY(arena_alloc_t(ctx, (size_t)nblk * CHOL_WS, &Linv2));
  NK_TRY(arena_alloc_t(ctx, (size_t)m * m, &V1));
  NK_TRY(arena_alloc_t(ctx, (size_t)m * m, &Sinvt));
  NK_TRY(arena_alloc_t(ctx, (size_t)m * m, &T1t));
  NK_TRY(arena_alloc_t(ctx, (size_t)m * m, &X1));
  NK_TRY(arena_alloc_t(ctx, (size_t)m * ldd, &Wc));
  NK_TRY(arena_alloc_t(ctx, (size_t)m * ldd, &Ct));
  NK_TRY(arena_alloc_t(ctx, (size_t)mp + m + 4, &pivlog));
  sys[0].P = G1; sys[0].ldp = mp; sys[0].m = mp; sys[0].Linv = Linv; sys[0].extra = m;
  sys[1].P = G3; sys[1].ldp = m; sys[1].m = m; sys[1].Linv = Linv2; sys[1].extra = d;
  sys[0].pivlog = pivlog; sys[1].pivlog = pivlog + mp + (mp & 1);
  NK_TRY(cholesky_aug_pair_async(ctx, sys, 2));
  tr.mark("cholesky + solves issued");
  return NK_OK;
}

int NystromFit::queue_sqrt_side() {
  SideScope side(ctx);
  NK_HIP(hipStreamWaitEvent(ctx->stream, ctx->ev_fork, 0));
  NK_HIP(hipStreamWaitEvent(ctx->stream, ctx->ev[EV_SQRT_PREPARED], 0));
  NK_HIP(hipEventRecord(ctx->ev[EV_SQRT_BEGIN], ctx->stream));
  NK_TRY(sqrtm_finish(ctx, &splan, mdl->S, mdl->Sinv));
  NK_HIP(hipEventRecord(ctx->ev[EV_SQRT_END], ctx->stream));
  NK_TRY(sqrt_products());
  NK_HIP(hipEventRecord(ctx->ev_join, ctx->stream));
  return NK_OK;
}

int NystromFit::operator_products() {
  NK_TRY(launch_transpose(ctx, G2, mp, V1, m, m, m));
  NK_TRY(launch_gemm(ctx, true, false, m, m, m, 1.0, V1, m, T1t, m, 0.0, X1, m));
  NK_TRY(launch_gemm(ctx, true, false, m, m, m, 1.0, Sinvt, m, X1, m, 0.0, mdl->A, mp));
  if (p > 0) NK_TRY(launch_gemm(ctx, true, false, m, p, m, 1.0, Sinvt, m, G2 + m, mp, 0.0, mdl->B, mp));
  NK_TRY(launch_transpose(ctx, G4, m, Wc, ldd, d, m));
  NK_TRY(launch_gemm(ctx, true, false, m, d, m, 1.0, mdl->S, m, Wc, ldd, 0.0, Ct, ldd));
  NK_TRY(launch_transpose(ctx, Ct, ldd, mdl->C, m, m, d));
  NK_TRY(launch_gemm(ctx, true, false, d, mp, m, 1.0, Ct, ldd, mdl->A, mp, 0.0, mdl->W, mp));
  return NK_OK;
}

int NystromFit::settle_factorisations() {
  NK_TRY(cholesky_fail_flags(ctx, sys, 2, chol_failed, piv_ratio));
  tr.mark("final sync");
  bool chol_rerun = false;
  if (chol_failed[0] == CHOL_FLOW_GIVEUP || chol_failed[1] == CHOL_FLOW_GIVEUP) {
    ChainOnly chain(ctx);
    NK_HIP(hipMemcpyAsync(G1, Gsave, gram_doubles(m, d, p) * sizeof(double), hipMemcpyDeviceToDevice, ctx->stream));
    NK_TRY(cholesky_aug_pair_async(ctx, sys, 2));
    NK_TRY(cholesky_fail_flags(ctx, sys, 2, chol_failed, piv_ratio));
    chol_rerun = true;
  }
  rank_sys[0] = mp; rank_sys[1] = m;
  redo_products = chol_rerun;
  if (ctx->strict_spd == 2) chol_failed[0] = chol_failed[1] = -1;
  if (chol_failed[0] || chol_failed[1]) {
    if (ctx->strict_spd == 1) {
      set_error("Cholesky: system %d is numerically rank deficient (non-positive or rounding-level pivot; the reference's "
                "lstsq truncates here) and strict mode is on", chol_failed[0] ? 0 : 1);
      return NK_ERR_NOT_SPD;
    }
    const double rcond = 2.220446049250313e-16;
    for (int q = 0; q < 2; ++q) {
      if (!chol_failed[q]) continue;
      PinvInfo pi;
      if (q == 0)
        NK_TRY(pinv_right_divide(ctx, Gsave, mp, mp, Gsave + (size_t)mp * mp, mp, m, G2, mp, rcond, &pi));
      else
        NK_TRY(pinv_right_divide(ctx, Gsave + gram_block1(m, p), m, m, Gsave + gram_block1(m, p) + (size_t)m * m, m, d, G4,
                                 m, rcond, &pi));
      if (!pi.converged) {
        set_error("rank-revealing fallback: Jacobi SVD of system %d did not converge in %d sweeps", q, pi.sweeps);
        return NK_ERR_NO_CONVERGENCE;
      }
      rank_sys[q] = pi.rank;
    }
    count_event(CNT_RANK_TRUNCATED);
    redo_products = true;
  }
  return NK_OK;
}

int NystromFit::refine() {
  const double refine_below = ctx->refine_pivot;
  const int refine_steps = ctx->refine_steps;
  double* refine_state = nullptr;
  NK_TRY(arena_alloc_t(ctx, (size_t)8, &refine_state));
  for (int q = 0; q < 2 && refine_steps > 0; ++q) {
    if (chol_failed[q] || !(piv_ratio[q] > 0.0) || piv_ratio[q] >= refine_below) continue;
    const int mq = sys[q].m, nr = sys[q].extra;
    const size_t off = q == 0 ? 0 : gram_block1(m, p);
    const double* Pq = Gsave + off;
    const double* Rq = Gsave + off + (size_t)mq * mq;
    double* Xq = G1 + off + (size_t)mq * mq;
    const ArenaMark mk = arena_mark(ctx);
    double *Res = nullptr, *ResT = nullptr, *partial = nullptr;
    const int64_t ldt_ = nr + (nr & 1);
    NK_TRY(arena_alloc_t(ctx, (size_t)nr * mq, &Res));
    NK_TRY(arena_alloc_t(ctx, (size_t)mq * ldt_, &ResT));
    NK_TRY(arena_alloc_t(ctx, (size_t)2 * refine_partial_blocks(), &partial));
    CholSys cs = sys[q];
    cs.R = ResT; cs.ldr = ldt_; cs.nrhs = nr;
    for (int step = 0; step < refine_steps; ++step) {
      NK_TRY(launch_resid_dd(ctx, Xq, mq, Pq, mq, Rq, mq, Res, mq, nr, mq));
      NK_TRY(launch_transpose(ctx, Res, mq, ResT, ldt_, nr, mq));
      NK_TRY(cholesky_solve_pair(ctx, &cs, 1));
      NK_TRY(launch_transpose(ctx, ResT, ldt_, Res, mq, mq, nr));
      NK_TRY(launch_refine_apply(ctx, Res, mq, Xq, mq, nr, mq, step, refine_state + 4 * q, partial));
    }
    NK_HIP(hipMemcpyAsync(ctx->h_scalars + 16 + 4 * q, refine_state + 4 * q, 4 * sizeof(double), hipMemcpyDeviceToHost,
                          ctx->stream));
    arena_release(ctx, mk);
    refined[q] = -1;
    redo_products = true;
  }
  return NK_OK;
}

int NystromFit::settle_sqrt() {
  const int vr = sqrtm_verdict(ctx, &splan, &it, &resid);
  if (vr == NK_SQRT_RETRY && splan.flow_gave_up) {
    ChainOnly chain(ctx);
    SqrtPlan again;
    again.lambda_min_hint = splan.lambda_min_hint;
    NK_TRY(sqrtm_prepare(ctx, Kj, m, m, &again));
    NK_TRY(sqrtm_finish(ctx, &again, mdl->S, mdl->Sinv));
    NK_HIP(hipStreamSynchronize(ctx->stream));
    const int vr2 = sqrtm_verdict(ctx, &again, &it, &resid);
    if (vr2 == NK_SQRT_RETRY) {
      count_event(CNT_SQRT_RETRY);
      NK_TRY(sqrtm_spd_coupled(ctx, Kj, m, m, mdl->S, mdl->Sinv, &it, &resid));
    } else {
      NK_TRY(vr2);
    }
    NK_TRY(sqrt_products());
    redo_products = true;
  } else if (vr == NK_SQRT_RETRY) {
    count_event(CNT_SQRT_RETRY);
    NK_TRY(sqrtm_spd_coupled(ctx, Kj, m, m, mdl->S, mdl->Sinv, &it, &resid));
    NK_TRY(sqrt_products());
    redo_products = true;
  } else {
    NK_TRY(vr);
  }
  return NK_OK;
}

void NystromFit::read_refinement() {
  for (int q = 0; q < 2; ++q)
    if (refined[q] < 0) {
      refined[q] = (int)ctx->h_scalars[16 + 4 * q + 2];
      refine_ratio[q] = ctx->h_scalars[16 + 4 * q + 3];
    }
  if (refined[0] > 0 || refined[1] > 0) count_event(CNT_REFINED);
}

void NystromFit::write_stats() {
  fill_gram_stats(ctx, stats, x.staged || y.staged, gram_deferred, ms_gram_kernel, gram_launches);
  stats->ms_total = ev_ms(ctx, EV_FIT_BEGIN, EV_FIT_END);
  stats->ms_sqrt = ev_ms(ctx, EV_SQRT_BEGIN, EV_SQRT_END);
  stats->ms_solve = ev_ms(ctx, EV_SOLVE_BEGIN, EV_FIT_END);
  stats->sqrt_iters = it;
  stats->sqrt_residual = resid;
  const double ne = (double)n_eff;
  const double t128 = 128.0;
  auto tiles = [&](double v) { return std::ceil(v / t128); };
  const double tmp_ = tiles(mp), tm_ = tiles(m);
  stats->gram_flops = 2.0 * ne * t128 * t128 * (tmp_ * (tmp_ + 1) / 2 + tm_ * tmp_ + tm_ * (tm_ + 1) / 2) +
                      2.0 * ne * (double)d * m;
  stats->kmat_pairs = 2.0 * ne * m * d + (same_centers ? 1.0 : 3.0) * (double)m * m * d;
  stats->rank_inner = rank_sys[0];
  stats->rank_inner_rec = rank_sys[1];
  stats->pivot_ratio_inner = piv_ratio[0];
  stats->pivot_ratio_inner_rec = piv_ratio[1];
  stats->refined = refined[0] + 16 * refined[1];
  stats->refine_ratio_inner = refine_ratio[0];
  stats->refine_ratio_inner_rec = refine_ratio[1];
}


int NystromFit::run() {
  NK_TRY(validate());
  NK_HIP(hipEventRecord(ctx->ev[EV_FIT_BEGIN], ctx->stream));
  NK_TRY(make_winv(ctx, kd, d, mdl->winv));
  if (mode != FIT_SOLVE) NK_TRY(stage_rows());
  NK_TRY(stage_landmarks());
  if (mode != FIT_GRAM) NK_TRY(landmark_matrices());
  NK_TRY(alloc_gram());
  if (mode == FIT_SOLVE) {
    NK_TRY(load_gram());
  } else {
    NK_TRY(prepare_features());
    NK_TRY(run_passes());
  }
  NK_HIP(hipEventRecord(ctx->ev[EV_GRAM_DONE], ctx->stream));
  if (mode == FIT_GRAM) return return_gram();

  NK_HIP(hipEventRecord(ctx->ev_fork, ctx->stream));
  tr.mark("gram issued");
  NK_TRY(queue_sqrt_prep());
  NK_TRY(assemble_and_factor());
  NK_TRY(queue_sqrt_side());
  NK_HIP(hipStreamWaitEvent(ctx->stream, ctx->ev_join, 0));
  NK_HIP(hipEventRecord(ctx->ev[EV_SOLVE_BEGIN], ctx->stream));
  tr.mark("side stream joined (queued)");
  NK_TRY(operator_products());
  NK_HIP(hipEventRecord(ctx->ev[EV_FIT_END], ctx->stream));
  tr.mark("solve issued");

  NK_TRY(settle_factorisations());
  NK_TRY(refine());
  NK_TRY(settle_sqrt());
  if (redo_products) {
    NK_TRY(operator_products());
    NK_HIP(hipStreamSynchronize(ctx->stream));
  }
  read_refinement();
  mdl->has_ops = true;
  if (stats) write_stats();
  tr.mark("stats");
  if (ctx->arena.chunks.size() > 1 || ctx->arena_side.chunks.size() > 1) NK_TRY(arena_reset(ctx));
  guard.m = nullptr;
  *model = mdl;
  return NK_OK;
}

extern "C" {

int nk_nystrom_fit(nk_ctx* ctx, const nk_kernel_desc* kd, const double* X, int64_t ldx, const double* Y, int64_t ldy,
                   int64_t n, int32_t d, int32_t p, const int64_t* row_ranges, int32_t n_ranges, const double* Zin,
                   int64_t ldzi, const double* Zout, int64_t ldzo, int32_t m, double gamma, double jitter,
                   nk_model** model, nk_fit_stats* stats) {
  NK_REQUIRE(model != nullptr, "nk_nystrom_fit: null argument");
  NystromFit f{ctx, kd, X, ldx, Y, ldy, n, d, p, row_ranges, n_ranges, Zin, ldzi, Zout, ldzo, m, gamma, jitter, model, stats,
               FIT_FULL, nullptr};
  return f.run();
}

int nk_gram_doubles(int32_t m, int32_t d, int32_t p, int64_t* count) {
  NK_REQUIRE(count && m > 0 && d > 0 && p >= 0, "nk_gram_doubles: bad argument");
  *count = (int64_t)gram_doubles(m, d, p);
  return NK_OK;
}

int nk_nystrom_gram(nk_ctx* ctx, const nk_kernel_desc* kd, const double* X, int64_t ldx, const double* Y, int64_t ldy,
                    int64_t n, int32_t d, int32_t p, const int64_t* row_ranges, int32_t n_ranges, const double* Zin,
                    int64_t ldzi, const double* Zout, int64_t ldzo, int32_t m, double* gram, nk_fit_stats* stats) {
  NystromFit f{ctx, kd, X, ldx, Y, ldy, n, d, p, row_ranges, n_ranges, Zin, ldzi, Zout, ldzo, m, 0.0, 0.0, nullptr, stats,
               FIT_GRAM, gram};
  return f.run();
}

int nk_nystrom_solve(nk_ctx* ctx, const nk_kernel_desc* kd, const double* Zin, int64_t ldzi, const double* Zout,
                     int64_t ldzo, int32_t m, int32_t d, int32_t p, const double* gram, int64_t n_total, double gamma,
                     double jitter, nk_model** model, nk_fit_stats* stats) {
  NK_REQUIRE(model != nullptr, "nk_nystrom_solve: null argument");
  NystromFit f{ctx, kd, nullptr, 0, nullptr, 0, n_total, d, p, nullptr, 0, Zin, ldzi, Zout, ldzo, m, gamma, jitter, model, stats,
               FIT_SOLVE, const_cast<double*>(gram)};
  return f.run();
}

static constexpr double SPLINE_SVD_WINDOW_PER_ROW = 2.0;

int nk_spline_fit(nk_ctx* ctx, const double* X, int64_t ldx, const double* Y, int64_t ldy, int64_t n, int32_t d, int32_t p,
                  const int64_t* row_ranges, int32_t n_ranges, const double* centers, int64_t ldc, int32_t m, double gamma,
                  nk_model** model, nk_fit_stats* stats) {
  NK_TRY(check_ctx(ctx));
  NK_REQUIRE(X && Y && centers && model, "nk_spline_fit: null argument");
  NK_REQUIRE(n > 0 && d > 0 && p >= 0 && m > 0, "nk_spline_fit: sizes must be positive (n=%lld d=%d p=%d m=%d)",
             (long long)n, d, p, m);
  NK_REQUIRE(ldx >= d + p && ldy >= d && ldc >= d, "nk_spline_fit: leading dimension too small");
  NK_REQUIRE(std::isfinite(gamma), "nk_spline_fit: gamma not finite");
  *model = nullptr;
  std::vector<int64_t> rng;
  int64_t n_eff = 0;
  NK_TRY(select_rows("nk_spline_fit", row_ranges, n_ranges, n, &rng, &n_eff));
  const int mp = m + p;
  const double gamma_n = gamma * (double)n_eff;

  nk_model* mdl = nullptr;
  NK_TRY(model_alloc(ctx, m, d, p, &mdl, NK_MODEL_SPLINE));
// ... 161 lines not shown
```

nys_koop_lqr_amd/csrc/nk_gemm_tn.hip:

```cpp
#include "nk_common.h"
#include "nk_tn_kstep.inc"
#include "nk_tn_shared.h"

#include <cstdlib>
#include <cstring>

namespace nk {

typedef double d4 __attribute__((ext_vector_type(4)));

constexpr int TBK = 16;
constexpr int TSTRIDE = 144;
constexpr int TSTAGE = 2 * TBK * TSTRIDE;
constexpr int TN_LDS_BYTES = 2 * TSTAGE * 8;

struct TnDev {
  const double* A;
  const double* B;
  int64_t lda, ldb;
  int M, N;
  int tiles_n;
  int tri;
  int ktrim;
  int tile_begin;
// ... 352 lines not shown
    for (int off = 32; off > 0; off >>= 1) rsum += __shfl_down(rsum, off, 64);
    if ((threadIdx.x & 63) == 0) wsum[threadIdx.x >> 6] = rsum;
    __syncthreads();
    if (threadIdx.x == 0) {
      const double w = (wsum[0] + wsum[1]) + (wsum[2] + wsum[3]);
      P.resid_partials[blockIdx.x] = mirror ? 2.0 * w : w;
    }
  }
  if (!transposed) return;
  __syncthreads();
  const int c = threadIdx.x >> 1, rb = (threadIdx.x & 1) * 8;
  const int col = col0 + c;
  if (col >= pr.N) return;
#pragma unroll
  for (int q = 0; q < 8; ++q) {
    const int row = row0 + rb + q;
    if (row >= pr.M) break;
    const double v = sh[rb + q][c];
    if (mirror) pr.C[(int64_t)col * pr.ldc + row] = v;
    if (pr.Ct) pr.Ct[(int64_t)col * pr.ldct + row] = v;
    if (mirror && pr.Caff) pr.Caff[(int64_t)col * pr.ldc + row] = pr.aff_a * v;
  }
}
__global__ void __launch_bounds__(256) gemm_tn_reduce_kernel(TnRedParams P) { gemm_tn_reduce_kernel_body(P); }
__global__ void __launch_bounds__(256) gemm_tn_reduce_kernel_batched(const nk::ArgPack<TnRedParams>* table) {
  gemm_tn_reduce_kernel_body(table[blockIdx.z].v);
}
static nk::TwinReg gemm_tn_reduce_twin_reg(reinterpret_cast<const void*>(static_cast<void (*)(TnRedParams)>(gemm_tn_reduce_kernel)),
                                           reinterpret_cast<const void*>(gemm_tn_reduce_kernel_batched),
                                           sizeof(nk::ArgPack<TnRedParams>), "gemm_tn_reduce_kernel");

int launch_tn_reduce(nk_ctx* ctx, const TnRedParams& R, int ntiles) {
  hipLaunchKernelGGL(gemm_tn_reduce_kernel, dim3((unsigned)ntiles * RPARTS), dim3(256), 0, ctx->stream, R);
  NK_HIP(hipGetLastError());
  return NK_OK;
}

__device__ __forceinline__ void transpose_kernel_body(const double* __restrict__ src, int64_t lds_, double* __restrict__ dst, int64_t ldd, int rows, int cols) {
  __shared__ double tile[32][33];
  const int bx = blockIdx.x * 32, by = blockIdx.y * 32;
  const int tx = threadIdx.x & 31, ty = threadIdx.x >> 5;
  for (int r = ty; r < 32; r += 8) {
    const int row = by + r, col = bx + tx;
    if (row < rows && col < cols) tile[r][tx] = src[(int64_t)row * lds_ + col];
  }
  __syncthreads();
  for (int r = ty; r < 32; r += 8) {
    const int orow = bx + r, ocol = by + tx;
    if (orow < cols && ocol < rows) dst[(int64_t)orow * ldd + ocol] = tile[tx][r];
  }
}
__global__ void __launch_bounds__(256) transpose_kernel(const double* __restrict__ src, int64_t lds_, double* __restrict__ dst, int64_t ldd, int rows, int cols) { transpose_kernel_body(src, lds_, dst, ldd, rows, cols); }
NK_BATCHED_TWIN(transpose_kernel, (256), const double*, int64_t, double*, int64_t, int, int)

int launch_transpose(nk_ctx* ctx, const double* src, int64_t lds_, double* dst, int64_t ldd, int rows, int cols) {
  if (rows <= 0 || cols <= 0) return NK_OK;
  dim3 grid((cols + 31) / 32, (rows + 31) / 32);
  hipLaunchKernelGGL(transpose_kernel, grid, dim3(256), 0, ctx->stream, src, lds_, dst, ldd, rows, cols);
  NK_HIP(hipGetLastError());
  return NK_OK;
}

static inline bool aligned16(const void* p) { return (reinterpret_cast<uintptr_t>(p) & 15) == 0; }

bool tn_fast_ok(const TnProblem& p) {
  return p.M >= 2 && p.N >= 2 && aligned16(p.A) && aligned16(p.B) && p.lda % 2 == 0 && p.ldb % 2 == 0 &&
         p.lda >= ((p.M + 1) & ~1) && p.ldb >= ((p.N + 1) & ~1);
}

static bool g_tn_attr_set = false;
static int tn_use_asm() {
  const char* e = getenv("NYSKOOP_TN_ASM");
  return (e && e[0] == '0') ? 0 : 1;
}

int tn_ensure_zero_page(nk_ctx* ctx) {
  if (ctx->d_zeros) return NK_OK;
  NK_HIP(hipMalloc(reinterpret_cast<void**>(&ctx->d_zeros), 4096));
  NK_HIP(hipMemset(ctx->d_zeros, 0, 4096));
  return NK_OK;
}

int launch_gemm_tn_multi(nk_ctx* ctx, const TnProblem* probs, int nprob, int64_t K, int splitk, float* ms_kernel,
                         bool sync_timing, const TnSkip* skip) {
  NK_REQUIRE(nprob >= 1 && nprob <= TN_MAXP, "gemm_tn_multi: 1..4 problems");
  NK_REQUIRE(K >= 0 && K < (1LL << 31), "gemm_tn_multi: K out of range");
  NK_TRY(tn_ensure_zero_page(ctx));
  TnParams P;
  TnRedParams R;
  int ntiles = 0;
  for (int q = 0; q < nprob; ++q) {
    const TnProblem& s = probs[q];
    NK_REQUIRE(tn_fast_ok(s), "gemm_tn_multi: problem %d violates the alignment contract", q);
    NK_REQUIRE(s.tri == TRI_FULL || (s.tri == TRI_UPPER_MIRROR && s.M == s.N), "gemm_tn_multi: bad tri mode");
    const int tmn = (s.M + TBM - 1) / TBM, tnn = (s.N + TBM - 1) / TBM;
    TnDev& d = P.p[q];
    d.A = s.A; d.B = s.B; d.lda = s.lda; d.ldb = s.ldb; d.M = s.M; d.N = s.N;
    d.tiles_n = tnn; d.tri = s.tri; d.ktrim = s.ktrim; d.tile_begin = ntiles;
    d.C = s.C; d.ldc = s.ldc; d.alpha = s.alpha; d.beta = s.beta; d.Ct = s.Ct; d.ldct = s.ldct;
    d.A_even = s.A_even; d.B_even = s.B_even;
    d.Caff = s.Caff; d.aff_a = s.aff_a; d.aff_c = s.aff_c;
    TnRed& r = R.p[q];
    r.Caff = s.Caff; r.aff_a = s.aff_a; r.aff_c = s.aff_c;
    r.Ct = s.Ct; r.ldct = s.ldct;
    r.C = s.C; r.ldc = s.ldc; r.M = s.M; r.N = s.N; r.tiles_n = tnn; r.tri = s.tri; r.tile_begin = ntiles;
    r.alpha = s.alpha; r.beta = s.beta;
    ntiles += s.tri == TRI_FULL ? tmn * tnn : tmn * (tmn + 1) / 2;
  }
  for (int q = nprob; q < TN_MAXP; ++q) {
    P.p[q] = P.p[0];
    P.p[q].tile_begin = 1 << 30;
    R.p[q] = R.p[0];
    R.p[q].tile_begin = 1 << 30;
  }
  const int ktiles_total = (int)((K + TBK - 1) / TBK);
  const bool want_resid = skip && skip->resid_partials != nullptr;
  if (splitk <= 0) {
    const int slots = 2 * ctx->num_cu;
    const int max_split = ktiles_total / 8 > 1 ? ktiles_total / 8 : 1;
    double best = 1e300;
    splitk = 1;
    for (int c = 1; c <= 64 && c <= max_split; ++c) {
      const int64_t wgs = (int64_t)ntiles * c;
      const double steps = (double)((ktiles_total + c - 1) / c);
      const int64_t full = wgs / slots, rem = wgs % slots;
      double t = full * 2.44 * steps;
      if (rem > 0) t += (rem <= ctx->num_cu ? 2.35 : 2.44) * steps;
      t *= 4096.0;
      if (c > 1) t += (double)wgs * (TBM * TBM * 8.0 * 2.0) / 4.0e12 * 2.4e9;
      t += 2000.0 * c / 8.0;
      if (c % 8 == 0) t *= 0.97;
      if (t < best) { best = t; splitk = c; }
    }
  }
  if (want_resid && splitk < 2) splitk = 2;
  if (nprob >= 3 && getenv("NYSKOOP_TN_SPLITK")) splitk = atoi(getenv("NYSKOOP_TN_SPLITK"));
  P.kmask = getenv("NYSKOOP_TN_KMASK") ? (int)strtol(getenv("NYSKOOP_TN_KMASK"), nullptr, 0) : -1;
  P.use_asm = tn_use_asm();
  P.nprob = nprob; P.ntiles = ntiles; P.K = (int)K; P.splitk = splitk;
  P.klen = ((ktiles_total + splitk - 1) / splitk) * TBK;
  if (P.klen == 0) P.klen = TBK;
  P.zeros = ctx->d_zeros;
  const ArenaMark mark = arena_mark(ctx);
  double* slab = nullptr;
  if (splitk > 1) NK_TRY(arena_alloc_t(ctx, (size_t)ntiles * splitk * TBM * TBM, &slab));
  P.slab = slab;
  R.nprob = nprob; R.splitk = splitk; R.slab = slab;
  P.skip_state = R.skip_state = skip ? skip->state : nullptr;
  P.skip_step = R.skip_step = skip ? skip->step : 0;
  P.select_state = skip ? skip->select : nullptr;
  R.resid_partials = (skip && splitk > 1 && nprob == 1) ? skip->resid_partials : nullptr;
  if (skip && skip->resid_count) *skip->resid_count = R.resid_partials ? ntiles * RPARTS : 0;
  if (!g_tn_attr_set) {
    NK_HIP(hipFuncSetAttribute(reinterpret_cast<const void*>(gemm_tn_f64_kernel<0>),
                               hipFuncAttributeMaxDynamicSharedMemorySize, TN_LDS_BYTES));
    NK_HIP(hipFuncSetAttribute(reinterpret_cast<const void*>(gram_fused_f64_kernel),
                               hipFuncAttributeMaxDynamicSharedMemorySize, TN_LDS_BYTES));
    NK_HIP(hipFuncSetAttribute(reinterpret_cast<const void*>(gemm_tn_f64_kernel<1>),
                               hipFuncAttributeMaxDynamicSharedMemorySize, TN_LDS_BYTES));
    NK_HIP(hipFuncSetAttribute(reinterpret_cast<const void*>(gemm_tn_f64_kernel<2>),
                               hipFuncAttributeMaxDynamicSharedMemorySize, TN_LDS_BYTES));
    NK_HIP(hipFuncSetAttribute(reinterpret_cast<const void*>(gemm_tn_f64_kernel<3>),
                               hipFuncAttributeMaxDynamicSharedMemorySize, TN_LDS_BYTES));
    NK_HIP(hipFuncSetAttribute(reinterpret_cast<const void*>(gemm_tn_f64_kernel<4>),
                               hipFuncAttributeMaxDynamicSharedMemorySize, TN_LDS_BYTES));
    NK_HIP(hipFuncSetAttribute(reinterpret_cast<const void*>(gemm_tn_f64_kernel_batched<0>),
                               hipFuncAttributeMaxDynamicSharedMemorySize, TN_LDS_BYTES));
    NK_HIP(hipFuncSetAttribute(reinterpret_cast<const void*>(gemm_tn_f64_kernel_batched<1>),
                               hipFuncAttributeMaxDynamicSharedMemorySize, TN_LDS_BYTES));
    NK_HIP(hipFuncSetAttribute(reinterpret_cast<const void*>(gemm_tn_f64_kernel_batched<2>),
                               hipFuncAttributeMaxDynamicSharedMemorySize, TN_LDS_BYTES));
    NK_HIP(hipFuncSetAttribute(reinterpret_cast<const void*>(gemm_tn_f64_kernel_batched<3>),
                               hipFuncAttributeMaxDynamicSharedMemorySize, TN_LDS_BYTES));
    NK_HIP(hipFuncSetAttribute(reinterpret_cast<const void*>(gemm_tn_f64_kernel_batched<4>),
                               hipFuncAttributeMaxDynamicSharedMemorySize, TN_LDS_BYTES));
    NK_HIP(hipFuncSetAttribute(reinterpret_cast<const void*>(gram_fused_f64_kernel_batched),
                               hipFuncAttributeMaxDynamicSharedMemorySize, TN_LDS_BYTES));
    g_tn_attr_set = true;
  }
  if (ms_kernel) NK_HIP(hipEventRecord(ctx->ev[EV_GEMM_T0], ctx->stream));
  P.sqa = P.sqb = nullptr; P.out = nullptr; P.ldo = 0; P.ktype = 0; P.sigma0sq = 0.0;
  if (nprob >= 3)
    hipLaunchKernelGGL(gram_fused_f64_kernel, dim3((unsigned)(ntiles * splitk)), dim3(256), TN_LDS_BYTES, ctx->stream, P);
  else
    hipLaunchKernelGGL(gemm_tn_f64_kernel<0>, dim3((unsigned)(ntiles * splitk)), dim3(256), TN_LDS_BYTES, ctx->stream, P);
  NK_HIP(hipGetLastError());
  if (ms_kernel) NK_HIP(hipEventRecord(ctx->ev[EV_GEMM_T1], ctx->stream));
  if (splitk > 1) {
    hipLaunchKernelGGL(gemm_tn_reduce_kernel, dim3((unsigned)ntiles * RPARTS), dim3(256), 0, ctx->stream, R);
    NK_HIP(hipGetLastError());
  }
  if (ms_kernel && sync_timing) {
    NK_HIP(hipEventSynchronize(ctx->ev[EV_GEMM_T1]));
    NK_HIP(hipEventElapsedTime(ms_kernel, ctx->ev[EV_GEMM_T0], ctx->ev[EV_GEMM_T1]));
  }
  arena_release(ctx, mark);
  return NK_OK;
}


__device__ __forceinline__ void prep_rows_kernel_body(const double* __restrict__ X, int64_t ldx, int rows, int d, const double* __restrict__ winv, const double* __restrict__ center, double* __restrict__ Xt, int64_t ldt) {
  __shared__ double tile[32][33];
  const int k0 = blockIdx.x * 32, r0 = blockIdx.y * 32;
  const int tx = threadIdx.x & 31, ty = threadIdx.x >> 5;
  for (int r = ty; r < 32; r += 8) {
    const int row = r0 + r, k = k0 + tx;
    if (row < rows && k < d) tile[r][tx] = (X[(int64_t)row * ldx + k] - center[k]) * winv[k];
  }
  __syncthreads();
  for (int r = ty; r < 32; r += 8) {
    const int k = k0 + r, row = r0 + tx;
    if (k < d && row < rows) Xt[(int64_t)k * ldt + row] = tile[tx][r];
  }
}
__global__ void __launch_bounds__(256) prep_rows_kernel(const double* __restrict__ X, int64_t ldx, int rows, int d, const double* __restrict__ winv, const double* __restrict__ center, double* __restrict__ Xt, int64_t ldt) { prep_rows_kernel_body(X, ldx, rows, d, winv, center, Xt, ldt); }
NK_BATCHED_TWIN(prep_rows_kernel, (256), const double*, int64_t, int, int, const double*, const double*, double*, int64_t)
__device__ __forceinline__ void colsq_kernel_body(const double* __restrict__ Xt, int64_t ldt, int rows, int d, double* __restrict__ sq) {
  __shared__ double part[4][64];
  const int lane = threadIdx.x & 63, w = threadIdx.x >> 6;
  const int i = blockIdx.x * 64 + lane;
  double s0 = 0.0, s1 = 0.0, s2 = 0.0, s3 = 0.0;
  if (i < rows) {
    int k = w;
    for (; k + 12 < d; k += 16) {
      const double v0 = Xt[(int64_t)k * ldt + i], v1 = Xt[(int64_t)(k + 4) * ldt + i];
      const double v2 = Xt[(int64_t)(k + 8) * ldt + i], v3 = Xt[(int64_t)(k + 12) * ldt + i];
      s0 = fma(v0, v0, s0); s1 = fma(v1, v1, s1); s2 = fma(v2, v2, s2); s3 = fma(v3, v3, s3);
    }
    for (; k < d; k += 4) {
      const double v = Xt[(int64_t)k * ldt + i];
      s0 = fma(v, v, s0);
    }
  }
  part[w][lane] = (s0 + s1) + (s2 + s3);
  __syncthreads();
  if (w == 0 && i < rows) sq[i] = (part[0][lane] + part[1][lane]) + (part[2][lane] + part[3][lane]);
}
__global__ void __launch_bounds__(256) colsq_kernel(const double* __restrict__ Xt, int64_t ldt, int rows, int d, double* __restrict__ sq) { colsq_kernel_body(Xt, ldt, rows, d, sq); }
NK_BATCHED_TWIN(colsq_kernel, (256), const double*, int64_t, int, int, double*)
__device__ __forceinline__ void colsum_partial_kernel_body(const double* __restrict__ Z, int64_t ldz, int rows, int d, int rows_per_chunk, double* __restrict__ partial) {
  const int k = blockIdx.x * blockDim.x + threadIdx.x;
  if (k >= d) return;
  const int r0 = blockIdx.y * rows_per_chunk;
  const int r1 = min(rows, r0 + rows_per_chunk);
  double s = 0.0;
  for (int r = r0; r < r1; ++r) s += Z[(int64_t)r * ldz + k];
  partial[(int64_t)blockIdx.y * d + k] = s;
}
__global__ void __launch_bounds__(256) colsum_partial_kernel(const double* __restrict__ Z, int64_t ldz, int rows, int d, int rows_per_chunk, double* __restrict__ partial) { colsum_partial_kernel_body(Z, ldz, rows, d, rows_per_chunk, partial); }
NK_BATCHED_TWIN(colsum_partial_kernel, (256), const double*, int64_t, int, int, int, double*)
__device__ __forceinline__ void colmean_finish_kernel_body(const double* __restrict__ partial, int chunks, int rows, int d, double* __restrict__ mean) {
  const int k = blockIdx.x * blockDim.x + threadIdx.x;
  if (k >= d) return;
  double s = 0.0;
  for (int c = 0; c < chunks; ++c) s += partial[(int64_t)c * d + k];
  mean[k] = s / rows;
}
__global__ void __launch_bounds__(256) colmean_finish_kernel(const double* __restrict__ partial, int chunks, int rows, int d, double* __restrict__ mean) { colmean_finish_kernel_body(partial, chunks, rows, d, mean); }
NK_BATCHED_TWIN(colmean_finish_kernel, (256), const double*, int, int, int, double*)

int launch_colmean(nk_ctx* ctx, const double* Z, int64_t ldz, int rows, int d, double* mean) {
  const ArenaMark mk = arena_mark(ctx);
  const int rpc = 32;
  const int chunks = (rows + rpc - 1) / rpc;
  double* partial = nullptr;
  NK_TRY(arena_alloc_t(ctx, (size_t)chunks * d, &partial));
  hipLaunchKernelGGL(colsum_partial_kernel, dim3((d + 255) / 256, chunks), dim3(256), 0, ctx->stream, Z, ldz, rows, d, rpc,
                     partial);
  hipLaunchKernelGGL(colmean_finish_kernel, dim3((d + 255) / 256), dim3(256), 0, ctx->stream, partial, chunks, rows, d, mean);
  NK_HIP(hipGetLastError());
// ... 74 lines not shown
```

nys_koop_lqr_amd/csrc/nk_linalg.hip:

```cpp
#include "nk_common.h"

#include <algorithm>
#include <cmath>
#include <cstring>
#include <vector>

namespace nk {

__device__ __forceinline__ void add_diag_kernel_body(double* A, int64_t lda, int n, double v) {
  int i = blockIdx.x * blockDim.x + threadIdx.x;
  if (i < n) A[(int64_t)i * lda + i] += v;
}
__global__ void __launch_bounds__(256) add_diag_kernel(double* A, int64_t lda, int n, double v) { add_diag_kernel_body(A, lda, n, v); }
NK_BATCHED_TWIN(add_diag_kernel, (256), double*, int64_t, int, double)
__device__ __forceinline__ void copy2d_kernel_body(const double* __restrict__ src, int64_t lds, double* __restrict__ dst, int64_t ldd, int64_t rows, int64_t cols) {
  const int64_t total = rows * cols;
  for (int64_t e = blockIdx.x * (int64_t)blockDim.x + threadIdx.x; e < total; e += (int64_t)gridDim.x * blockDim.x) {
    const int64_t r = e / cols, c = e - r * cols;
    dst[r * ldd + c] = src[r * lds + c];
  }
}
__global__ void __launch_bounds__(256) copy2d_kernel(const double* __restrict__ src, int64_t lds, double* __restrict__ dst, int64_t ldd, int64_t rows, int64_t cols) { copy2d_kernel_body(src, lds, dst, ldd, rows, cols); }
NK_BATCHED_TWIN(copy2d_kernel, (256), const double*, int64_t, double*, int64_t, int64_t, int64_t)
__device__ __forceinline__ void axpby2d_kernel_body(double a, const double* __restrict__ X, int64_t ldx, double b, double* __restrict__ Y, int64_t ldy, int64_t rows, int64_t cols) {
// ... 562 lines not shown
      int rc_panel = NK_OK;
      if (!launch_chol_panel_pair(ctx, panel, nsys, &rc_panel)) NK_TRY(launch_gemm_pair(ctx, false, true, panel, nsys));
      NK_TRY(rc_panel);
    }
    if (fuse && jb + 1 < nblk) {
      int rc_f = NK_OK;
      int nbn[2] = {0, 0};
      double* Lin[2] = {nullptr, nullptr};
      double* Pln[2] = {nullptr, nullptr};
      next_block(sys, nsys, jb, nbn, Lin, Pln);
      if (launch_chol_trail_potrf_pair(ctx, trail, nsys, nbn, Lin, jb + 1, Pln, &rc_f)) {
        NK_TRY(rc_f);
        diag_done = true;
        continue;
      }
    }
    {
      int rc_trail = NK_OK;
      if (!launch_chol_trail_pair(ctx, trail, nsys, &rc_trail)) NK_TRY(launch_gemm_pair(ctx, false, true, trail, nsys));
      NK_TRY(rc_trail);
    }
  }
  return NK_OK;
}

int cholesky_check_pair(nk_ctx* ctx, const CholSys* sys, int nsys) {
  int failed[2] = {0, 0};
  NK_TRY(cholesky_fail_flags(ctx, sys, nsys, failed));
  for (int q = 0; q < nsys; ++q)
    if (failed[q] != 0) {
      if (failed[q] > 0)
        set_error("Cholesky: non-positive pivot at index %d of %d (system %d is numerically rank deficient; the "
                  "reference's lstsq would truncate here)", failed[q] - 1, sys[q].m, q);
      else
        set_error("Cholesky: system %d (order %d) has an isolated cluster of rounding-level pivots: an exact null space (the "
                  "reference's lstsq truncates it)", q, sys[q].m);
      return NK_ERR_NOT_SPD;
    }
  return NK_OK;
}

int cholesky_fail_flags(nk_ctx* ctx, const CholSys* sys, int nsys, int* failed, double* piv_ratio) {
  const int ib = info_base(ctx);
  std::vector<double> plog[2];
  NK_HIP(hipMemcpyAsync(ctx->h_info + ib, ctx->d_info + ib, 2 * sizeof(int), hipMemcpyDeviceToHost, ctx->stream));
  NK_HIP(hipMemcpyAsync(ctx->h_piv + 2 * ib, ctx->d_piv + 2 * ib, 4 * sizeof(unsigned long long), hipMemcpyDeviceToHost,
                        ctx->stream));
  for (int q = 0; q < nsys; ++q)
    if (sys[q].pivlog) {
      plog[q].resize((size_t)sys[q].m);
      NK_HIP(hipMemcpyAsync(plog[q].data(), sys[q].pivlog, sizeof(double) * sys[q].m, hipMemcpyDeviceToHost, ctx->stream));
    }
  NK_HIP(hipStreamSynchronize(ctx->stream));
  const double eps = 2.220446049250313e-16;
  for (int q = 0; q < nsys; ++q) {
    failed[q] = ctx->h_info[ib + q];
    if (piv_ratio) piv_ratio[q] = 0.0;
    if (failed[q] == CHOL_FLOW_GIVEUP) {
      if (q == 0) count_event(CNT_CHOL_FLOW_GIVEUP);
      continue;
    }
    if (failed[q] != 0) continue;
    double dmin, dmax;
    memcpy(&dmin, &ctx->h_piv[2 * (ib + q)], 8);
    memcpy(&dmax, &ctx->h_piv[2 * (ib + q) + 1], 8);
    if (!(dmax > 0.0)) continue;
    if (piv_ratio) piv_ratio[q] = dmin / dmax;
    if (dmin <= eps * dmax) { failed[q] = -1; continue; }
    if (plog[q].empty()) continue;
    std::sort(plog[q].begin(), plog[q].end());
    const double window = 8.0 * (double)sys[q].m * eps * dmax;
    size_t k = 0;
    while (k < plog[q].size() && plog[q][k] <= window) ++k;
    if (k > 0 && k < plog[q].size() && plog[q][k] >= 1000.0 * plog[q][k - 1]) failed[q] = -1;
  }
  return NK_OK;
}

int cholesky_lower_pair(nk_ctx* ctx, const CholSys* sys, int nsys) {
  NK_TRY(cholesky_lower_pair_async(ctx, sys, nsys));
  return cholesky_check_pair(ctx, sys, nsys);
}

int cholesky_aug_pair_async(nk_ctx* ctx, const CholSys* sys, int nsys, hipEvent_t pause, int pause_step) {
  constexpr int NB = CHOL_NB;
  NK_REQUIRE(nsys >= 1 && nsys <= 2, "cholesky_aug_pair: 1..2 systems");
  NK_TRY(reset_pivots(ctx));
  int nblk = 0, mmin = sys[0].m;
  for (int q = 0; q < nsys; ++q) {
    nblk = std::max(nblk, (sys[q].m + NB - 1) / NB);
    mmin = std::min(mmin, sys[q].m);
  }
  if (!ctx->chol_flow_off && mmin >= 256 && !ctx_recording(ctx) && chol_flow_enabled()) {
    if (pause != nullptr && pause_step >= 0 && pause_step < nblk) NK_HIP(hipStreamWaitEvent(ctx->stream, pause, 0));
    NK_TRY(cholesky_flow_pair(ctx, sys, nsys));
    NK_TRY(launch_trsm_right_lower_pair(ctx, sys, nsys));
    return NK_OK;
  }
  static const bool la_env = getenv("NYSKOOP_CHOL_LOOKAHEAD") && getenv("NYSKOOP_CHOL_LOOKAHEAD")[0] == '1';
  const int la = ctx->stream == ctx->stream_main ? 1 : -1;
  const bool lookahead = la_env && la >= 0 && nblk >= 4 && !ctx_recording(ctx);
  hipStream_t s_chain = ctx->stream;
  hipStream_t s_rest = lookahead ? ctx->stream_la[la] : ctx->stream;
  hipEvent_t* la_evt = lookahead ? ctx->ev_la[la] : nullptr;
  bool rest_pending = false;
  hipEvent_t last_rest = nullptr;
  if (lookahead) {
    NK_HIP(hipEventRecord(la_evt[1], s_chain));
    NK_HIP(hipStreamWaitEvent(s_rest, la_evt[1], 0));
  }
  const bool fuse = chol_fuse_enabled();
  bool diag_done = false;
  for (int jb = 0; jb < nblk; ++jb) {
    if (pause != nullptr && jb == pause_step) NK_HIP(hipStreamWaitEvent(ctx->stream, pause, 0));
    const int j0 = jb * NB;
    double* Ajj[2] = {nullptr, nullptr};
    double* Li[2] = {nullptr, nullptr};
    double* Pl[2] = {nullptr, nullptr};
    int64_t lda[2] = {0, 0};
    int nbj[2] = {0, 0};
    GemmCall panel[2], trail[2], next[2], rest[2];
    bool any_rest = false;
    for (int q = 0; q < nsys; ++q) {
      const CholSys& y = sys[q];
      if (j0 >= y.m) continue;
      nbj[q] = y.m - j0 < NB ? y.m - j0 : NB;
      Ajj[q] = y.P + (int64_t)j0 * y.ldp + j0;
      lda[q] = y.ldp;
      Li[q] = y.Linv + (size_t)jb * CHOL_WS;
      Pl[q] = y.pivlog ? y.pivlog + j0 : nullptr;
      const int rem = y.m - j0 - nbj[q];
      const int rows = rem + y.extra;
      if (rows > 0) {
        double* pnl = y.P + (int64_t)(j0 + nbj[q]) * y.ldp + j0;
        panel[q].M = rows; panel[q].N = nbj[q]; panel[q].K = nbj[q];
        panel[q].A = pnl; panel[q].lda = y.ldp; panel[q].B = Li[q]; panel[q].ldb = NB;
        panel[q].C = pnl; panel[q].ldc = y.ldp;
        if (rem > 0) {
          trail[q].M = rows; trail[q].N = rem; trail[q].K = nbj[q]; trail[q].alpha = -1.0; trail[q].beta = 1.0;
          trail[q].A = pnl; trail[q].lda = y.ldp; trail[q].B = pnl; trail[q].ldb = y.ldp;
          trail[q].C = y.P + (int64_t)(j0 + nbj[q]) * y.ldp + (j0 + nbj[q]); trail[q].ldc = y.ldp;
          trail[q].opts.tri = TRI_LOWER;
          const int nbn = rem < NB ? rem : NB;
          next[q] = trail[q];
          next[q].N = nbn;
          if (rem > nbn) {
            rest[q] = trail[q];
            rest[q].M = rows - nbn; rest[q].N = rem - nbn;
            rest[q].A = rest[q].B = pnl + (int64_t)nbn * y.ldp;
            rest[q].C = trail[q].C + (int64_t)nbn * y.ldp + nbn;
            any_rest = true;
          }
        }
      }
    }
    if (!diag_done) NK_TRY(launch_potrf_diag_pair(ctx, Ajj, lda, nbj, Li, nsys, jb, Pl));
    diag_done = false;
    {
      int rc_panel = NK_OK;
      if (!launch_chol_panel_pair(ctx, panel, nsys, &rc_panel)) NK_TRY(launch_gemm_pair(ctx, false, true, panel, nsys));
      NK_TRY(rc_panel);
    }
    if (fuse && !lookahead && jb + 1 < nblk) {
      int rc_f = NK_OK;
      int nbn[2] = {0, 0};
      double* Lin[2] = {nullptr, nullptr};
      double* Pln[2] = {nullptr, nullptr};
      next_block(sys, nsys, jb, nbn, Lin, Pln);
      if (launch_chol_trail_potrf_pair(ctx, trail, nsys, nbn, Lin, jb + 1, Pln, &rc_f)) {
        NK_TRY(rc_f);
        diag_done = true;
        continue;
      }
    }
    auto update = [&](const GemmCall* calls) -> int {
      int rc_trail = NK_OK;
      if (!launch_chol_trail_pair(ctx, calls, nsys, &rc_trail)) NK_TRY(launch_gemm_pair(ctx, false, true, calls, nsys));
      return rc_trail;
    };
    if (!lookahead) {
      NK_TRY(update(trail));
    } else {
      hipEvent_t evP = la_evt[jb & 1], evR = la_evt[2 + (jb & 1)], evR_prev = la_evt[2 + ((jb + 1) & 1)];
      NK_HIP(hipEventRecord(evP, s_chain));
      if (rest_pending) NK_HIP(hipStreamWaitEvent(s_chain, evR_prev, 0));
      NK_TRY(update(next));
      rest_pending = false;
      if (any_rest) {
        ctx->stream = s_rest;
        NK_HIP(hipStreamWaitEvent(s_rest, evP, 0));
        const int rc = update(rest);
        if (rc == NK_OK) NK_HIP(hipEventRecord(evR, s_rest));
        last_rest = evR;
        ctx->stream = s_chain;
        NK_TRY(rc);
        rest_pending = true;
      }
    }
  }
  if (lookahead && last_rest) NK_HIP(hipStreamWaitEvent(s_chain, last_rest, 0));
  NK_TRY(launch_trsm_right_lower_pair(ctx, sys, nsys));
  return NK_OK;
}

int cholesky_solve_pair(nk_ctx* ctx, const CholSys* sys, int nsys) {
  constexpr int NB = CHOL_NB;
  NK_REQUIRE(nsys >= 1 && nsys <= 2, "cholesky_solve_pair: 1..2 systems");
  int nblk = 0;
  for (int q = 0; q < nsys; ++q) nblk = std::max(nblk, (sys[q].m + NB - 1) / NB);
  const ArenaMark mk = arena_mark(ctx);
  double* tmp[2] = {nullptr, nullptr};
  for (int q = 0; q < nsys; ++q) NK_TRY(arena_alloc_t(ctx, (size_t)NB * sys[q].ldr, &tmp[q]));
  auto diag_solve = [&](int jb, bool trans) -> int {
    const int j0 = jb * NB;
    GemmCall g1[2], g2[2], g3[2];
    for (int q = 0; q < nsys; ++q) {
      const CholSys& y = sys[q];
      if (j0 >= y.m) continue;
      const int nbj = y.m - j0 < NB ? y.m - j0 : NB;
      const double* Li = y.Linv + (size_t)jb * CHOL_WS;
      const double* Ld = Li + NB * NB;
      double* Rj = y.R + (int64_t)j0 * y.ldr;
      NK_TRY(launch_copy2d(ctx, Rj, y.ldr, tmp[q], y.ldr, nbj, y.nrhs));
      g1[q].M = nbj; g1[q].N = y.nrhs; g1[q].K = nbj; g1[q].A = Li; g1[q].lda = NB; g1[q].B = tmp[q]; g1[q].ldb = y.ldr;
      g1[q].C = Rj; g1[q].ldc = y.ldr;
      g2[q] = g1[q]; g2[q].A = Ld; g2[q].B = Rj; g2[q].C = tmp[q]; g2[q].alpha = -1.0; g2[q].beta = 1.0;
      g3[q] = g1[q]; g3[q].beta = 1.0;
    }
    NK_TRY(launch_gemm_pair(ctx, trans, false, g1, nsys));
    NK_TRY(launch_gemm_pair(ctx, trans, false, g2, nsys));
    NK_TRY(launch_gemm_pair(ctx, trans, false, g3, nsys));
    return NK_OK;
  };
  for (int jb = 0; jb < nblk; ++jb) {
    const int j0 = jb * NB;
    GemmCall upd[2];
    for (int q = 0; q < nsys; ++q) {
      const CholSys& y = sys[q];
      if (j0 >= y.m) continue;
      const int nbj = y.m - j0 < NB ? y.m - j0 : NB;
      double* Rj = y.R + (int64_t)j0 * y.ldr;
      const int rem = y.m - j0 - nbj;
      if (rem > 0) {
        upd[q].M = rem; upd[q].N = y.nrhs; upd[q].K = nbj; upd[q].alpha = -1.0; upd[q].beta = 1.0;
        upd[q].A = y.P + (int64_t)(j0 + nbj) * y.ldp + j0; upd[q].lda = y.ldp; upd[q].B = Rj; upd[q].ldb = y.ldr;
        upd[q].C = y.R + (int64_t)(j0 + nbj) * y.ldr; upd[q].ldc = y.ldr;
      }
    }
    NK_TRY(diag_solve(jb, false));
    NK_TRY(launch_gemm_pair(ctx, false, false, upd, nsys));
  }
  for (int jb = nblk - 1; jb >= 0; --jb) {
    const int j0 = jb * NB;
    GemmCall upd[2];
    for (int q = 0; q < nsys; ++q) {
      const CholSys& y = sys[q];
      if (j0 >= y.m) continue;
      const int nbj = y.m - j0 < NB ? y.m - j0 : NB;
      double* Rj = y.R + (int64_t)j0 * y.ldr;
      if (j0 > 0) {
        upd[q].M = j0; upd[q].N = y.nrhs; upd[q].K = nbj; upd[q].alpha = -1.0; upd[q].beta = 1.0;
        upd[q].A = y.P + (int64_t)j0 * y.ldp; upd[q].lda = y.ldp; upd[q].B = Rj; upd[q].ldb = y.ldr;
        upd[q].C = y.R; upd[q].ldc = y.ldr;
      }
    }
    NK_TRY(diag_solve(jb, true));
    NK_TRY(launch_gemm_pair(ctx, true, false, upd, nsys));
  }
  arena_release(ctx, mk);
  return NK_OK;
}

int cholesky_lower(nk_ctx* ctx, double* P, int64_t ldp, int m, double* Linv) {
  CholSys y;
  y.P = P; y.ldp = ldp; y.m = m; y.Linv = Linv;
  return cholesky_lower_pair(ctx, &y, 1);
}

int cholesky_solve(nk_ctx* ctx, const double* L, int64_t ldl, int m, const double* Linv, double* R, int64_t ldr,
                   int nrhs) {
  CholSys y;
  y.P = const_cast<double*>(L); y.ldp = ldl; y.m = m; y.Linv = const_cast<double*>(Linv); y.R = R; y.ldr = ldr;
  y.nrhs = nrhs;
  return cholesky_solve_pair(ctx, &y, 1);
}

__device__ __forceinline__ void tri_scale_both_kernel_body(const double* __restrict__ L, int64_t ldl, int m, const double* __restrict__ d_c, double* __restrict__ Xt, double* __restrict__ X) {
  __shared__ double tile[32][33];
  const double s = 1.0 / sqrt(d_c[0]);
  const int bx = blockIdx.x * 32, by = blockIdx.y * 32;
  const int tx = threadIdx.x & 31, ty = threadIdx.x >> 5;
  for (int r = ty; r < 32; r += 8) {
    const int i = by + r, j = bx + tx;
    double v = 0.0;
    if (i < m && j <= i) v = L[(int64_t)i * ldl + j] * s;
    if (i < m && j < m) Xt[(int64_t)i * m + j] = v;
    tile[r][tx] = v;
  }
  __syncthreads();
  for (int r = ty; r < 32; r += 8) {
    const int i = bx + r, j = by + tx;
    if (i < m && j < m) X[(int64_t)i * m + j] = tile[tx][r];
  }
}
__global__ void __launch_bounds__(256) tri_scale_both_kernel(const double* __restrict__ L, int64_t ldl, int m, const double* __restrict__ d_c, double* __restrict__ Xt, double* __restrict__ X) { tri_scale_both_kernel_body(L, ldl, m, d_c, Xt, X); }
NK_BATCHED_TWIN(tri_scale_both_kernel, (256), const double*, int64_t, int, const double*, double*, double*)

int sqrtm_prepare(nk_ctx* ctx, const double* P, int64_t ldp, int m, SqrtPlan* plan) {
  plan->P = P; plan->ldp = ldp; plan->m = m;
  plan->mark = arena_mark(ctx);
  const size_t mm = (size_t)m * m;
  const int nblk = (m + CHOL_NB - 1) / CHOL_NB;
  NK_TRY(arena_alloc_t(ctx, 2 * mm, &plan->W));
  NK_TRY(arena_alloc_t(ctx, (size_t)nblk * CHOL_WS, &plan->Linv));
  NK_TRY(arena_alloc_t(ctx, mm, &plan->X0));
  NK_TRY(arena_alloc_t(ctx, mm, &plan->X0t));
  NK_TRY(arena_alloc_t(ctx, (size_t)8, &plan->d_sc));
  NK_TRY(launch_max_abs_rowsum(ctx, P, ldp, m, plan->d_sc));
  {
    const ArenaMark mk = arena_mark(ctx);
    const int blocks = grid_for((int64_t)m * m, ctx->num_cu);
    double* partial = nullptr;
    NK_TRY(arena_alloc_t(ctx, (size_t)2 * blocks, &partial));
    hipLaunchKernelGGL(sumsq_trace_partial_kernel, dim3(blocks), dim3(256), 0, ctx->stream, P, ldp, m, partial, blocks);
    hipLaunchKernelGGL(sum_partials_kernel, dim3(1), dim3(256), 0, ctx->stream, partial, blocks, plan->d_sc + 1);
    hipLaunchKernelGGL(sum_partials_kernel, dim3(1), dim3(256), 0, ctx->stream, partial + blocks, blocks, plan->d_sc + 2);
    NK_HIP(hipGetLastError());
    arena_release(ctx, mk);
  }
  NK_HIP(hipMemcpyAsync(ctx->h_scalars + 12, plan->d_sc, 3 * sizeof(double), hipMemcpyDeviceToHost, ctx->stream));
  NK_HIP(hipEventRecord(ctx->ev[EV_SQRT_SCALARS], ctx->stream));
  double* E = plan->W + mm;
  NK_TRY(launch_copy2d(ctx, P, ldp, plan->W, m, m, m));
  NK_TRY(launch_fill(ctx, E, m, m, m, 0.0));
  NK_TRY(launch_add_diag(ctx, E, m, m, 1.0));
  CholSys y;
  y.P = plan->W; y.ldp = m; y.m = m; y.extra = m; y.backward = false; y.Linv = plan->Linv;
  NK_TRY(cholesky_aug_pair_async(ctx, &y, 1, plan->pause_event, plan->pause_step));
  {
    const ArenaMark mk = arena_mark(ctx);
    const int blocks = grid_for((int64_t)m * m, ctx->num_cu);
    double* partial = nullptr;
    NK_TRY(arena_alloc_t(ctx, (size_t)2 * blocks, &partial));
    hipLaunchKernelGGL(sumsq_trace_partial_kernel, dim3(blocks), dim3(256), 0, ctx->stream, E, (int64_t)m, m, partial, blocks);
    hipLaunchKernelGGL(sum_partials_kernel, dim3(1), dim3(256), 0, ctx->stream, partial, blocks, plan->d_sc + 3);
    NK_HIP(hipGetLastError());
    arena_release(ctx, mk);
  }
  const int tb = (m + 31) / 32;
  hipLaunchKernelGGL(tri_scale_both_kernel, dim3(tb, tb), dim3(256), 0, ctx->stream, plan->W, (int64_t)m, m, plan->d_sc,
                     plan->X0t, plan->X0);
  NK_HIP(hipGetLastError());
  return NK_OK;
}

__device__ __forceinline__ void ns_flag_kernel_body(const double* __restrict__ partial, int count, int m, int step, double* __restrict__ state) {
  __shared__ double sh[4];
  double s = 0.0;
  for (int i = threadIdx.x; i < count; i += blockDim.x) s += partial[i];
  s = wave_sum(s);
  if ((threadIdx.x & 63) == 0) sh[threadIdx.x >> 6] = s;
  __syncthreads();
  if (threadIdx.x == 0) {
    const double r = sqrt((sh[0] + sh[1] + sh[2] + sh[3]) / m);
    state[2] = r;
    if (state[0] == 0.0 && r < 1e-7) {
      state[0] = (double)(step + 1);
      state[1] = r;
    }
  }
}
__global__ void __launch_bounds__(256) ns_flag_kernel(const double* __restrict__ partial, int count, int m, int step, double* __restrict__ state) { ns_flag_kernel_body(partial, count, m, step, state); }
NK_BATCHED_TWIN(ns_flag_kernel, (256), const double*, int, int, int, double*)

static int sqrtm_polar_products(nk_ctx* ctx, SqrtPlan* plan, const double* Q, double* scratch, double c, double* S,
                                double* Sinv, const double* Q_even = nullptr, const double* select = nullptr) {
  const int m = plan->m;
  const size_t mm = (size_t)m * m;
  double* Linv_full = scratch;
  NK_TRY(launch_transpose(ctx, plan->W + mm, m, Linv_full, m, m, m));
  TnProblem pr[2];
  pr[0].A = Q; pr[0].B = plan->X0; pr[0].C = S; pr[0].lda = pr[0].ldb = pr[0].ldc = m; pr[0].M = pr[0].N = m;
  pr[0].alpha = std::sqrt(c);
  pr[0].ktrim = KTRIM_B_UPPER;
  pr[1].ktrim = KTRIM_A_LOWER;
  pr[1].A = Linv_full; pr[1].B = Q; pr[1].C = Sinv; pr[1].lda = pr[1].ldb = pr[1].ldc = m; pr[1].M = pr[1].N = m;
  pr[0].A_even = Q_even;
  pr[1].B_even = Q_even;
  TnSkip sel;
  sel.select = select;
  if (tn_fast_ok(pr[0]) && tn_fast_ok(pr[1]) && m >= 128) {
    NK_TRY(launch_gemm_tn_multi(ctx, pr, 2, m, 0, nullptr, true, select ? &sel : nullptr));
  } else {
    NK_TRY(launch_gemm(ctx, true, false, m, m, m, pr[0].alpha, Q, m, plan->X0, m, 0.0, S, m));
    NK_TRY(launch_gemm(ctx, true, false, m, m, m, 1.0, Linv_full, m, Q, m, 0.0, Sinv, m));
  }
  return NK_OK;
}

int sqrtm_finish(nk_ctx* ctx, SqrtPlan* plan, double* S, double* Sinv) {
  const int m = plan->m;
  const size_t mm = (size_t)m * m;
  const int ib = info_base(ctx);
  plan->deferred = false;
  plan->info_slot = ib;
  plan->rc = NK_OK; plan->iters = 0; plan->resid = 0.0;
  plan->early = plan->lambda_min_hint > 0.0 && m >= 1024 && m % 2 == 0;
  double c, sumsq, trace, linv2 = 0.0;
  if (plan->early) {
    NK_HIP(hipEventSynchronize(ctx->ev[EV_SQRT_SCALARS]));
    c = ctx->h_scalars[12]; sumsq = ctx->h_scalars[13]; trace = ctx->h_scalars[14];
    if (!(c > 0.0) || !std::isfinite(c)) plan->early = false;
  }
  if (!plan->early) {
    NK_HIP(hipMemcpyAsync(ctx->h_scalars, plan->d_sc, 4 * sizeof(double), hipMemcpyDeviceToHost, ctx->stream));
    NK_HIP(hipMemcpyAsync(ctx->h_info + ib, ctx->d_info + ib, sizeof(int), hipMemcpyDeviceToHost, ctx->stream));
    NK_HIP(hipStreamSynchronize(ctx->stream));
    c = ctx->h_scalars[0]; sumsq = ctx->h_scalars[1]; trace = ctx->h_scalars[2]; linv2 = ctx->h_scalars[3];
  }
  if (!plan->early && ctx->h_info[ib] == CHOL_FLOW_GIVEUP) {
    count_event(CNT_CHOL_FLOW_GIVEUP);
    arena_release(ctx, plan->mark);
    ChainOnly chain(ctx);
    SqrtPlan again;
    NK_TRY(sqrtm_prepare(ctx, plan->P, plan->ldp, m, &again));
    const int rc = sqrtm_finish(ctx, &again, S, Sinv);
    *plan = again;
    return rc;
  }
  if (!plan->early &&
      (ctx->h_info[ib] != 0 || !(c > 0.0) || !std::isfinite(c) || !(linv2 > 0.0) || !std::isfinite(linv2))) {
    arena_release(ctx, plan->mark);
    plan->rc = sqrtm_spd_coupled(ctx, plan->P, plan->ldp, m, S, Sinv, &plan->iters, &plan->resid);
    return plan->rc;
  }
  double *Xa = nullptr, *Xta = nullptr, *Xb = nullptr, *Xtb = nullptr, *M = nullptr, *T = nullptr;
  NK_TRY(arena_alloc_t(ctx, mm, &Xa));
  NK_TRY(arena_alloc_t(ctx, mm, &Xta));
  NK_TRY(arena_alloc_t(ctx, mm, &Xb));
  NK_TRY(arena_alloc_t(ctx, mm, &Xtb));
  NK_TRY(arena_alloc_t(ctx, mm, &M));
  NK_TRY(arena_alloc_t(ctx, mm, &T));
  double a_lo = 1.0, b_hi = 1.0;
  {
    const double fro = std::sqrt(sumsq) / c, tr = trace / c;
    const double lam1 = fro < 1.0 ? fro : 1.0;
    if (m > 1 && tr > lam1) a_lo = (tr - lam1) / (m - 1);
    else a_lo = tr / m * 1e-2;
    if (!(a_lo > 0.0) || !std::isfinite(a_lo)) a_lo = 1e-12;
    if (a_lo > 1.0) a_lo = 1.0;
  }
  auto p3 = [](double x) { return x * (3.0 - x) * (3.0 - x) * 0.25; };
  auto advance = [&](double s2, double& a, double& b) {
    const double xa = s2 * a, xb = s2 * b;
    const double lo = p3(xa) < p3(xb) ? p3(xa) : p3(xb);
    b = (xa <= 1.0 && xb >= 1.0) ? 1.0 : (p3(xa) > p3(xb) ? p3(xa) : p3(xb));
    a = lo < b ? lo : b;
  };
  GemmOpts sym;
  sym.tri = TRI_UPPER_MIRROR;
  const double* X = plan->X0;
  const double* Xt = plan->X0t;
  double *Xn = Xa, *Xtn = Xta;
  TnProblem probe;
  probe.A = Xta; probe.B = T; probe.C = Xa; probe.lda = probe.ldb = probe.ldc = m; probe.M = probe.N = m;
  const bool fast = m >= 128 && tn_fast_ok(probe);
  const bool queued = fast && m >= 1024;
  if (plan->early && !queued) {
    set_error("sqrtm: internal: early queueing needs the LDS-DMA path");
    return NK_ERR_BAD_ARG;
  }

  if (queued) {
    double s2s[128];
    bool checks[128];
    int kmax = 0;
    {
      double ta = plan->early ? 0.9 * plan->lambda_min_hint / c : 0.5 / (c * linv2), tb = 1.0;
      if (ta > a_lo) ta = a_lo;
      const double a_sched = std::pow(a_lo, 0.8) * std::pow(ta, 0.2);
      double a = a_sched, b = b_hi;
      int kconv = -1;
      for (int k = 0; k < 100; ++k) {
        if (kconv < 0 && ta >= 1.0 - 1e-9 && tb <= 1.0 + 1e-9) kconv = k;
        checks[k] = a >= 0.5;
        const double s2 = 3.0 / (a + std::sqrt(a * b) + b);
        s2s[k] = s2;
        advance(s2, a, b);
        advance(s2, ta, tb);
        if (kconv >= 0 && k >= kconv + 1) { kmax = k + 1; break; }
      }
      if (kmax == 0) kmax = 100;
    }
    double* state = plan->d_sc + 5;
    NK_HIP(hipMemsetAsync(state, 0, 3 * sizeof(double), ctx->stream));
    double* rpart = nullptr;
    {
      const size_t mt = (size_t)(m + 127) / 128;
      const size_t need = std::max((size_t)grid_for((int64_t)m * m, ctx->num_cu), mt * (mt + 1) / 2 * 8);
      NK_TRY(arena_alloc_t(ctx, need, &rpart));
    }
    for (int k = 0; k < kmax; ++k) {
      TnSkip skip;
      skip.state = state; skip.step = k;
      int npart = 0;
      if (k == 0) {
        NK_TRY(launch_transpose(ctx, plan->P, plan->ldp, M, m, m, m));
        NK_TRY(launch_axpby2d(ctx, 0.5 / c, plan->P, plan->ldp, 0.5 / c, M, m, m, m));
      } else {
        const double s2k = s2s[k], sck = std::sqrt(s2k);
        TnProblem pm;
        pm.A = X; pm.B = X; pm.C = M; pm.lda = pm.ldb = pm.ldc = m; pm.M = pm.N = m; pm.tri = TRI_UPPER_MIRROR;
        pm.Caff = T; pm.aff_a = -0.5 * s2k * sck; pm.aff_c = 1.5 * sck;
        TnSkip skip_m = skip;
        skip_m.resid_partials = rpart; skip_m.resid_count = &npart;
        NK_TRY(launch_gemm_tn_multi(ctx, &pm, 1, m, 0, nullptr, true, &skip_m));
      }
      if (checks[k]) {
        if (npart == 0) {
          npart = grid_for((int64_t)m * m, ctx->num_cu);
          hipLaunchKernelGGL(frob_mi_partial_kernel, dim3(npart), dim3(256), 0, ctx->stream, M, (int64_t)m, m, rpart,
                             skip.state, skip.step);
        }
        hipLaunchKernelGGL(ns_flag_kernel, dim3(1), dim3(256), 0, ctx->stream, rpart, npart, m, k, state);
        NK_HIP(hipGetLastError());
      }
      if (k == 0) {
        const double s2 = s2s[0], sc = std::sqrt(s2);
        NK_TRY(launch_scale_add_identity(ctx, -0.5 * s2 * sc, M, m, 1.5 * sc, T, m, m, &skip));
      }
      TnProblem pr;
      pr.A = Xt; pr.B = T; pr.C = Xn; pr.lda = pr.ldb = pr.ldc = m; pr.M = pr.N = m; pr.Ct = Xtn; pr.ldct = m;
      NK_TRY(launch_gemm_tn_multi(ctx, &pr, 1, m, 1, nullptr, true, &skip));
      X = Xn; Xt = Xtn;
      Xn = (Xn == Xa) ? Xb : Xa;
      Xtn = (Xtn == Xta) ? Xtb : Xta;
    }
    NK_TRY(sqrtm_polar_products(ctx, plan, Xa, T, c, S, Sinv, Xb, state));
    NK_HIP(hipMemcpyAsync(ctx->h_scalars + 8, state, 3 * sizeof(double), hipMemcpyDeviceToHost, ctx->stream));
    if (plan->early)
      NK_HIP(hipMemcpyAsync(ctx->h_info + ib, ctx->d_info + ib, sizeof(int), hipMemcpyDeviceToHost, ctx->stream));
    plan->deferred = true;
    plan->kmax = kmax;
    arena_release(ctx, plan->mark);
    return NK_OK;
  }

  const int maxit = 100;
  double r = 1e300;
  int it = 0;
  bool ok = false;
  for (; it < maxit; ++it) {
    if (it == 0) {
      NK_TRY(launch_transpose(ctx, plan->P, plan->ldp, M, m, m, m));
      NK_TRY(launch_axpby2d(ctx, 0.5 / c, plan->P, plan->ldp, 0.5 / c, M, m, m, m));
    } else {
      NK_TRY(launch_gemm(ctx, true, false, m, m, m, 1.0, X, m, X, m, 0.0, M, m, sym));
    }
    const bool check = a_lo >= 0.5 || it + 2 >= maxit;
    if (check) {
      NK_TRY(launch_frob_minus_identity(ctx, M, m, m, ctx->d_scalars));
      NK_HIP(hipMemcpyAsync(ctx->h_scalars, ctx->d_scalars, sizeof(double), hipMemcpyDeviceToHost, ctx->stream));
      NK_HIP(hipEventRecord(ctx->ev[EV_SQRT_RESID], ctx->stream));
    }
    const double s2 = 3.0 / (a_lo + std::sqrt(a_lo * b_hi) + b_hi);
    const double sc = std::sqrt(s2);
    advance(s2, a_lo, b_hi);
    NK_TRY(launch_scale_add_identity(ctx, -0.5 * s2 * sc, M, m, 1.5 * sc, T, m, m));
    if (fast) {
      TnProblem pr;
      pr.A = Xt; pr.B = T; pr.C = Xn; pr.lda = pr.ldb = pr.ldc = m; pr.M = pr.N = m; pr.Ct = Xtn; pr.ldct = m;
      NK_TRY(launch_gemm_tn_multi(ctx, &pr, 1, m, 0));
    } else {
      NK_TRY(launch_gemm(ctx, true, false, m, m, m, 1.0, Xt, m, T, m, 0.0, Xn, m));
      NK_TRY(launch_transpose(ctx, Xn, m, Xtn, m, m, m));
    }
    X = Xn; Xt = Xtn;
    Xn = (Xn == Xa) ? Xb : Xa;
    Xtn = (Xtn == Xta) ? Xtb : Xta;
    if (check) {
      NK_HIP(hipEventSynchronize(ctx->ev[EV_SQRT_RESID]));
      r = std::sqrt(ctx->h_scalars[0] / m);
      if (!std::isfinite(r)) break;
      if (r < 1e-7) {
        ok = true;
        ++it;
        break;
      }
    }
  }
  plan->iters = it;
  plan->resid = r;
  NK_TRY(x_align());
  if (!ok) {
    set_error("sqrtm: Newton-Schulz did not converge (residual %g after %d iterations)", r, it);
    arena_release(ctx, plan->mark);
    plan->rc = NK_ERR_NO_CONVERGENCE;
    return plan->rc;
  }
  NK_TRY(sqrtm_polar_products(ctx, plan, X, T, c, S, Sinv));
  arena_release(ctx, plan->mark);
  return NK_OK;
}

int sqrtm_verdict(nk_ctx* ctx, SqrtPlan* plan, int* iters, double* resid) {
  if (plan->deferred) {
    const double flag = ctx->h_scalars[8];
    plan->deferred = false;
    const int word = ctx->h_info[plan->info_slot];
    if (plan->early && (word != 0 || flag == 0.0 || !std::isfinite(ctx->h_scalars[10]))) {
      plan->flow_gave_up = word == CHOL_FLOW_GIVEUP;
      if (plan->flow_gave_up) count_event(CNT_CHOL_FLOW_GIVEUP);
      plan->iters = plan->kmax;
      plan->resid = ctx->h_scalars[10];
      plan->rc = NK_SQRT_RETRY;
    } else if (flag == 0.0 || !std::isfinite(ctx->h_scalars[10])) {
      plan->iters = plan->kmax;
      plan->resid = ctx->h_scalars[10];
      plan->rc = NK_ERR_NO_CONVERGENCE;
      set_error("sqrtm: Newton-Schulz did not converge (residual %g after %d iterations)", plan->resid, plan->kmax);
    } else {
      plan->iters = (int)flag;
      plan->resid = ctx->h_scalars[9];
      plan->rc = NK_OK;
    }
  }
  if (iters) *iters = plan->iters;
  if (resid) *resid = plan->resid;
  return plan->rc;
}

int sqrtm_spd(nk_ctx* ctx, const double* P, int64_t ldp, int m, double* S, double* Sinv, int* iters, double* resid) {
  SqrtPlan plan;
  NK_TRY(sqrtm_prepare(ctx, P, ldp, m, &plan));
  NK_TRY(sqrtm_finish(ctx, &plan, S, Sinv));
  NK_HIP(hipStreamSynchronize(ctx->stream));
  return sqrtm_verdict(ctx, &plan, iters, resid);
}

}
```

Measured before the change: 24.75.

## Hoist sqrtm setup into gram pass and overlap with Gram GEMM

Splits the Newton-Schulz square-root preparation into begin, factor and setup phases. The setup (scalars, schedule, buffer allocation, first iteration) is now issued on the prep stream while the K_nm/Gram GEMM runs, and the fork event is recorded from inside the Gram GEMM once its product is done. By default the factorisation stays after the Gram (tail mode), and the first product uses a triangular k-trim. It also adds optional grid and priority controls for the Cholesky flow kernel plus extra timing stats. The aim is to shorten the serial tail after the Gram step, at the cost of more stream and event complexity and contention with the Gram kernel.

```diff
diff --git a/include/nyskoop.h b/include/nyskoop.h
--- a/include/nyskoop.h
+++ b/include/nyskoop.h
@@ -51,6 +51,11 @@
   int32_t reserved_;
   double refine_ratio_inner;
   double refine_ratio_inner_rec;
+  int32_t sqrt_schedule;
+  int32_t reserved2_;
+  double ms_prep_wait;
+  double ms_tail_sqrt;
+  double ms_tail_trsm;
 } nk_fit_stats;
 
 typedef struct nk_ctx nk_ctx;
diff --git a/nys_koop_lqr_amd/_lib.py b/nys_koop_lqr_amd/_lib.py
--- a/nys_koop_lqr_amd/_lib.py
+++ b/nys_koop_lqr_amd/_lib.py
@@ -62,7 +62,9 @@
                 ("sqrt_iters", C.c_int32), ("sqrt_residual", C.c_double), ("gram_flops", C.c_double),
                 ("kmat_pairs", C.c_double), ("rank_inner", C.c_int32), ("rank_inner_rec", C.c_int32),
                 ("pivot_ratio_inner", C.c_double), ("pivot_ratio_inner_rec", C.c_double), ("refined", C.c_int32),
-                ("reserved_", C.c_int32), ("refine_ratio_inner", C.c_double), ("refine_ratio_inner_rec", C.c_double)]
+                ("reserved_", C.c_int32), ("refine_ratio_inner", C.c_double), ("refine_ratio_inner_rec", C.c_double),
+                ("sqrt_schedule", C.c_int32), ("reserved2_", C.c_int32), ("ms_prep_wait", C.c_double),
+                ("ms_tail_sqrt", C.c_double), ("ms_tail_trsm", C.c_double)]
 
     def as_dict(self):
         return {k: getattr(self, k) for k, _ in self._fields_}
diff --git a/nys_koop_lqr_amd/csrc/nk_api.hip b/nys_koop_lqr_amd/csrc/nk_api.hip
--- a/nys_koop_lqr_amd/csrc/nk_api.hip
+++ b/nys_koop_lqr_amd/csrc/nk_api.hip
@@ -385,7 +385,9 @@
   NK_HIP(hipDeviceGetStreamPriorityRange(&prio_lo, &prio_hi));
   const int prio_mid = (prio_lo - prio_hi >= 2) ? (prio_lo + prio_hi) / 2 : prio_hi;
   NK_HIP(hipStreamCreateWithPriority(&ctx->stream_main, hipStreamNonBlocking, prio_mid));
-  NK_HIP(hipStreamCreateWithPriority(&ctx->stream_side, hipStreamNonBlocking, prio_lo));
+  const char* sp = getenv("NYSKOOP_SIDE_PRIORITY");
+  const int prio_side = (sp && strcmp(sp, "hi") == 0) ? prio_hi : ((sp && strcmp(sp, "mid") == 0) ? prio_mid : prio_lo);
+  NK_HIP(hipStreamCreateWithPriority(&ctx->stream_side, hipStreamNonBlocking, prio_side));
   NK_HIP(hipStreamCreateWithPriority(&ctx->stream_prep, hipStreamNonBlocking, prio_hi));
   NK_HIP(hipStreamCreateWithFlags(&ctx->stream_copy, hipStreamNonBlocking));
   NK_HIP(hipStreamCreateWithPriority(&ctx->stream_la[0], hipStreamNonBlocking, prio_hi));
diff --git a/nys_koop_lqr_amd/csrc/nk_chol_flow.hip b/nys_koop_lqr_amd/csrc/nk_chol_flow.hip
--- a/nys_koop_lqr_amd/csrc/nk_chol_flow.hip
+++ b/nys_koop_lqr_amd/csrc/nk_chol_flow.hip
@@ -30,6 +30,7 @@
   int nsys;
   int total;
   int fix;
+  int hi_prio;
   int test_giveup;
   int* hdr;
 };
@@ -196,17 +197,17 @@
   ps.fix = a.fix;
   ps.nblocks = 1;
   chol_panel_rows(ps, 16 * wave, lane);
-  __builtin_amdgcn_s_setprio(0);
+  if (a.hi_prio) __builtin_amdgcn_s_setprio(2); else __builtin_amdgcn_s_setprio(0);
 }
 
 __device__ __noinline__ void flow_potrf(double* A, int64_t lda, int nb, double* Linv, int* info, unsigned long long* piv,
-                                       double* plog, int blk, int lane) {
+                                       double* plog, int blk, int lane, int hi_prio) {
   PotrfBatch pb;
   pb.A[0] = A; pb.lda[0] = lda; pb.nb[0] = nb; pb.Linv[0] = Linv; pb.info[0] = info; pb.piv[0] = piv; pb.plog[0] = plog;
   pb.A[1] = nullptr; pb.lda[1] = 0; pb.nb[1] = 0; pb.Linv[1] = nullptr; pb.info[1] = nullptr; pb.piv[1] = nullptr;
   pb.plog[1] = nullptr;
   potrf_diag_kernel_body<true>(pb, blk, 0, lane);
-  __builtin_amdgcn_s_setprio(0);
+  if (hi_prio) __builtin_amdgcn_s_setprio(2); else __builtin_amdgcn_s_setprio(0);
 }
 
 __global__ void __launch_bounds__(FLOW_THREADS) chol_flow_kernel(FlowArgs a) {
@@ -215,6 +216,7 @@
   const int wave = __builtin_amdgcn_readfirstlane(threadIdx.x >> 6);
   const int wm = wave >> 1, wn = wave & 1;
   const int l15 = lane & 15, l4 = lane >> 4;
+  if (a.hi_prio) __builtin_amdgcn_s_setprio(2);
   for (;;) {
     if (threadIdx.x == 0) sh[1] = atomicAdd(a.hdr, 1);
     __syncthreads();
@@ -261,7 +263,7 @@
       }
       if (wave == 0)
         flow_potrf(s.P + (int64_t)c0 * s.ldp + c0, s.ldp, c1 - c0, s.Linv + (size_t)k * CHOL_WS, s.info, s.piv,
-                   s.pivlog ? s.pivlog + c0 : nullptr, k, lane);
+                   s.pivlog ? s.pivlog + c0 : nullptr, k, lane, a.hi_prio);
       publish(s, k, k);
       __syncthreads();
     } else {
@@ -303,7 +305,7 @@
   return (ticket >= 0 && ticket < total) ? (int)ticket : -1;
 }
 
-int cholesky_flow_pair(nk_ctx* ctx, const CholSys* sys, int nsys) {
+int cholesky_flow_pair(nk_ctx* ctx, const CholSys* sys, int nsys, const FlowOpts& opts) {
   constexpr int NB = CHOL_NB;
   NK_REQUIRE(nsys >= 1 && nsys <= 2, "cholesky_flow_pair: 1..2 systems");
   FlowArgs a;
@@ -338,7 +340,8 @@
     f += (size_t)(a.s[q].nblk + a.s[q].nex) * a.s[q].nblk;
   }
   NK_HIP(hipMemsetAsync(a.hdr, 0, words * sizeof(int), ctx->stream));
-  const int grid = std::max(1, std::min(a.total, ctx->num_cu / 2));
+  const int grid = std::max(1, std::min(a.total, opts.grid > 0 ? opts.grid : ctx->num_cu / 2));
+  a.hi_prio = opts.hi_prio ? 1 : 0;
   hipLaunchKernelGGL(chol_flow_kernel, dim3((unsigned)grid), dim3(FLOW_THREADS), 0, ctx->stream, a);
   NK_HIP(hipGetLastError());
   count_event(CNT_CHOL_FLOW);
diff --git a/nys_koop_lqr_amd/csrc/nk_common.h b/nys_koop_lqr_amd/csrc/nk_common.h
--- a/nys_koop_lqr_amd/csrc/nk_common.h
+++ b/nys_koop_lqr_amd/csrc/nk_common.h
@@ -68,7 +68,8 @@
   EV_YPREP_DONE = 13,
   EV_GEMM_T0 = 14,
   EV_GEMM_T1 = 15,
-  EV_COUNT = 16
+  EV_TRSM_END = 16,
+  EV_COUNT = 17
 };
 
 struct nk_member_state;
@@ -286,6 +287,10 @@
                          int cols, double* d_colsum);
 
 int sqrtm_spd(nk_ctx* ctx, const double* P, int64_t ldp, int m, double* S, double* Sinv, int* iters, double* resid);
+struct FlowOpts {
+  int grid = 0;
+  bool hi_prio = false;
+};
 struct SqrtPlan {
   const double* P = nullptr;
   int64_t ldp = 0;
@@ -305,10 +310,21 @@
   bool flow_gave_up = false;
   hipEvent_t pause_event = nullptr;
   int pause_step = -1;
+  FlowOpts flow;
+  bool skip_linv_norm = false;
+  bool hoisted = false;
+  double c = 0.0;
+  double *Xa = nullptr, *Xta = nullptr, *Xb = nullptr, *Xtb = nullptr, *M = nullptr, *T = nullptr, *rpart = nullptr;
+  double* Linv_full = nullptr;
+  double s2s[128];
+  bool checks[128];
 };
 constexpr int NK_SQRT_RETRY = 1;
 int sqrtm_spd_coupled(nk_ctx* ctx, const double* P, int64_t ldp, int m, double* S, double* Sinv, int* iters, double* resid);
 int sqrtm_prepare(nk_ctx* ctx, const double* P, int64_t ldp, int m, SqrtPlan* plan);
+int sqrtm_prepare_begin(nk_ctx* ctx, const double* P, int64_t ldp, int m, SqrtPlan* plan);
+int sqrtm_prepare_factor(nk_ctx* ctx, SqrtPlan* plan);
+int sqrtm_setup(nk_ctx* ctx, SqrtPlan* plan, bool with_linv);
 int sqrtm_finish(nk_ctx* ctx, SqrtPlan* plan, double* S, double* Sinv);
 int sqrtm_verdict(nk_ctx* ctx, SqrtPlan* plan, int* iters, double* resid);
 int cholesky_lower(nk_ctx* ctx, double* P, int64_t ldp, int m, double* Linv );
@@ -330,7 +346,8 @@
 int cholesky_lower_pair_async(nk_ctx* ctx, const CholSys* sys, int nsys);
 int cholesky_check_pair(nk_ctx* ctx, const CholSys* sys, int nsys);
 int cholesky_solve_pair(nk_ctx* ctx, const CholSys* sys, int nsys);
-int cholesky_aug_pair_async(nk_ctx* ctx, const CholSys* sys, int nsys, hipEvent_t pause = nullptr, int pause_step = -1);
+int cholesky_aug_pair_async(nk_ctx* ctx, const CholSys* sys, int nsys, hipEvent_t pause = nullptr, int pause_step = -1,
+                            const FlowOpts& flow = FlowOpts(), hipEvent_t end = nullptr);
 constexpr int CHOL_NB = 64;
 constexpr int CHOL_WS = 2 * CHOL_NB * CHOL_NB + 8;
 constexpr double CHOL_FIX_KAPPA = 8.0 * CHOL_NB;
@@ -346,7 +363,7 @@
   return !(e && e[0] == '0');
 }
 bool chol_flow_enabled();
-int cholesky_flow_pair(nk_ctx* ctx, const CholSys* sys, int nsys);
+int cholesky_flow_pair(nk_ctx* ctx, const CholSys* sys, int nsys, const FlowOpts& opts = FlowOpts());
 constexpr int CHOL_FLOW_GIVEUP = -0x40000000;
 bool launch_chol_panel_pair(nk_ctx* ctx, const GemmCall* calls, int ncalls, int* rc);
 int launch_trsm_right_lower_pair(nk_ctx* ctx, const CholSys* sys, int nsys);
@@ -480,7 +497,8 @@
 int launch_kmat_gram_f32(nk_ctx* ctx, int ktype, const float* At, int64_t ldat, const float* sqa, int64_t nA, const float* Bt,
                          int64_t ldbt, const float* sqb, int64_t nB, int d, double sigma0, float* out, int64_t ldo);
 int launch_gemm_tn_multi(nk_ctx* ctx, const TnProblem* probs, int nprob, int64_t K, int splitk ,
-                         float* ms_kernel = nullptr, bool sync_timing = true, const TnSkip* skip = nullptr);
+                         float* ms_kernel = nullptr, bool sync_timing = true, const TnSkip* skip = nullptr,
+                         hipEvent_t product_done = nullptr);
 int launch_transpose(nk_ctx* ctx, const double* src, int64_t lds, double* dst, int64_t ldd, int rows, int cols);
 constexpr int refine_partial_blocks() { return 512; }
 int launch_refine_apply(nk_ctx* ctx, const double* dX, int64_t ldd, double* X, int64_t ldx, int64_t rows, int64_t cols, int step,
diff --git a/nys_koop_lqr_amd/csrc/nk_fit.hip b/nys_koop_lqr_amd/csrc/nk_fit.hip
--- a/nys_koop_lqr_amd/csrc/nk_fit.hip
+++ b/nys_koop_lqr_amd/csrc/nk_fit.hip
@@ -11,6 +11,8 @@
 
 static inline size_t gram_block1(int m, int p) { return (((size_t)(2 * m + p) * (m + p)) + 1) & ~(size_t)1; }
 static inline size_t gram_doubles(int m, int d, int p) { return gram_block1(m, p) + (size_t)(m + d) * m; }
+
+static constexpr int SQRT_EARLY_GRID_DIV = 4;
 
 
 static int select_rows(const char* who, const int64_t* row_ranges, int32_t n_ranges, int64_t n, std::vector<int64_t>* rng,
@@ -132,6 +134,8 @@
 
 
 enum { FIT_FULL = 0, FIT_GRAM = 1, FIT_SOLVE = 2 };
+enum { SQRT_LATE = 0, SQRT_EARLY = 1, SQRT_TAIL = 2 };
+static constexpr int SQRT_DEFAULT = SQRT_TAIL;
 
 struct NystromFit {
   nk_ctx* ctx; const nk_kernel_desc* kd;
@@ -162,6 +166,9 @@
   int64_t f_rows = 0, maxlen = 0, ldt32 = 0, ldzt32 = 0, ldy32 = 0;
   double *F = nullptr, *Rt2 = nullptr, *sqr2 = nullptr;
   float *F32 = nullptr, *Rt32 = nullptr, *sq32 = nullptr, *Zt32 = nullptr, *sqz32 = nullptr, *Y32 = nullptr;
+  bool sqrt_large = false;
+  int sqrt_mode = SQRT_LATE;
+  bool fork_in_gram = false;
   SqrtPlan splan;
   int it = 0;
   double resid = 0.0;
@@ -176,6 +183,8 @@
   int validate(), stage_rows(), stage_landmarks(), landmark_matrices(), alloc_gram(), load_gram(), prepare_features(), run_passes();
   int upload_pass(size_t ip), pass_f32(size_t ip), pass_f64(size_t ip), blocks_overlapped(const Piece& pc, double* Fo);
   int return_gram();
+  void plan_sqrt_schedule();
+  int begin_sqrt_prep(), finish_sqrt_prep();
   int queue_sqrt_prep(), assemble_and_factor(), queue_sqrt_side(), sqrt_products(), operator_products();
   int settle_factorisations(), refine(), settle_sqrt();
   void read_refinement(), write_stats();
@@ -393,6 +402,7 @@
   if (ip == 0) {
     NK_HIP(hipEventRecord(ctx->ev[EV_KMAT_DONE], ctx->stream));
     tr.mark("kmat issued");
+    if (sqrt_mode != SQRT_LATE) NK_TRY(finish_sqrt_prep());
   }
   TnProblemF pf[4];
   pf[0].A = F32; pf[0].B = F32; pf[0].lda = pf[0].ldb = ldf; pf[0].M = pf[0].N = mp; pf[0].C = G1; pf[0].ldc = mp;
@@ -442,6 +452,7 @@
   if (ip == 0) {
     NK_HIP(hipEventRecord(ctx->ev[EV_KMAT_DONE], ctx->stream));
     tr.mark("kmat issued");
+    if (sqrt_mode != SQRT_LATE) NK_TRY(finish_sqrt_prep());
   }
   TnProblem pr[4];
   pr[0].A = F; pr[0].B = F; pr[0].lda = pr[0].ldb = ldf; pr[0].M = pr[0].N = mp; pr[0].C = G1; pr[0].ldc = mp;
@@ -460,11 +471,14 @@
   if (fast) {
     const int np = (single && fast_y) ? 4 : 3;
     float ms1 = 0.f;
-    NK_TRY(launch_gemm_tn_multi(ctx, pr, np, rows, 0, (timed && !pipelined) ? &ms1 : nullptr, multi_pass));
+    NK_TRY(launch_gemm_tn_multi(ctx, pr, np, rows, 0, (timed && !pipelined) ? &ms1 : nullptr, multi_pass, nullptr,
+                                sqrt_mode != SQRT_LATE ? ctx->ev_fork : nullptr));
+    fork_in_gram = sqrt_mode != SQRT_LATE;
     if (multi_pass) ms_gram_kernel += ms1; else gram_deferred = timed;
     gram_launches += 1;
     y_done = np == 4;
   } else {
+    fork_in_gram = false;
     GemmOpts sym;
     sym.tri = TRI_UPPER_MIRROR;
     float t3[3] = {0.f, 0.f, 0.f};
@@ -502,6 +516,16 @@
 }
 
 
+void NystromFit::plan_sqrt_schedule() {
+  const char* e = getenv("NYSKOOP_SQRT_EARLY");
+  sqrt_large = mode == FIT_FULL && n_eff >= 20000 && m >= 1024;
+  sqrt_mode = SQRT_LATE;
+  if (sqrt_large && !ctx_recording(ctx)) {
+    sqrt_mode = SQRT_DEFAULT;
+    if (e && e[0] >= '0' && e[0] <= '2') sqrt_mode = e[0] - '0';
+  }
+}
+
 int NystromFit::sqrt_products() {
   NK_TRY(launch_transpose(ctx, mdl->Sinv, m, Sinvt, m, m, m));
   if (same_centers) {
@@ -515,19 +539,46 @@
 }
 
 int NystromFit::queue_sqrt_prep() {
+  if (sqrt_mode == SQRT_EARLY) return NK_OK;
+  SideScope prep(ctx, ctx->stream_prep);
+  if (sqrt_large) {
+    splan.pause_event = ctx->ev_fork;
+    splan.pause_step = 0;
+  }
+  if (sqrt_mode == SQRT_TAIL) {
+    NK_TRY(sqrtm_prepare_factor(ctx, &splan));
+  } else {
+    NK_HIP(hipStreamWaitEvent(ctx->stream, ctx->ev[EV_LANDMARKS], 0));
+    splan.lambda_min_hint = jitter > 0.0 ? jitter : 0.0;
+    NK_TRY(sqrtm_prepare(ctx, Kj, m, m, &splan));
+  }
+  NK_HIP(hipEventRecord(ctx->ev[EV_SQRT_PREPARED], ctx->stream));
+  return NK_OK;
+}
+
+int NystromFit::begin_sqrt_prep() {
   SideScope prep(ctx, ctx->stream_prep);
   NK_HIP(hipStreamWaitEvent(ctx->stream, ctx->ev[EV_LANDMARKS], 0));
   splan.lambda_min_hint = jitter > 0.0 ? jitter : 0.0;
-  if (mode == FIT_FULL && n_eff >= 20000 && m >= 1024) {
-    static const double frac = getenv("NYSKOOP_PREP_PAUSE") ? atof(getenv("NYSKOOP_PREP_PAUSE")) : 0.0;
-    const int nb = (m + CHOL_NB - 1) / CHOL_NB;
-    if (frac < 1.0) {
-      splan.pause_event = ctx->ev_fork;
-      splan.pause_step = std::max(0, std::min(nb - 1, (int)(frac * nb)));
-    }
-  }
-  NK_TRY(sqrtm_prepare(ctx, Kj, m, m, &splan));
-  NK_HIP(hipEventRecord(ctx->ev[EV_SQRT_PREPARED], ctx->stream));
+  splan.skip_linv_norm = splan.lambda_min_hint > 0.0 && m % 2 == 0;
+  NK_TRY(sqrtm_prepare_begin(ctx, Kj, m, m, &splan));
+  if (sqrt_mode == SQRT_EARLY) {
+    const char* g = getenv("NYSKOOP_SQRT_EARLY_GRID");
+    const char* pr = getenv("NYSKOOP_SQRT_EARLY_PRIO");
+    splan.flow.grid = std::max(1, ctx->num_cu / (g ? std::max(1, atoi(g)) : SQRT_EARLY_GRID_DIV));
+    splan.flow.hi_prio = pr && pr[0] == '1';
+    NK_TRY(sqrtm_prepare_factor(ctx, &splan));
+  }
+  return NK_OK;
+}
+
+int NystromFit::finish_sqrt_prep() {
+  SideScope prep(ctx, ctx->stream_prep);
+  NK_TRY(sqrtm_setup(ctx, &splan, sqrt_mode == SQRT_EARLY));
+  if (sqrt_mode == SQRT_EARLY) {
+    NK_HIP(hipEventRecord(ctx->ev[EV_SQRT_PREPARED], ctx->stream));
+    NK_HIP(hipStreamWaitEvent(ctx->stream_main, ctx->ev[EV_SQRT_PREPARED], 0));
+  }
   return NK_OK;
 }
 
@@ -552,7 +603,7 @@
   sys[0].P = G1; sys[0].ldp = mp; sys[0].m = mp; sys[0].Linv = Linv; sys[0].extra = m;
   sys[1].P = G3; sys[1].ldp = m; sys[1].m = m; sys[1].Linv = Linv2; sys[1].extra = d;
   sys[0].pivlog = pivlog; sys[1].pivlog = pivlog + mp + (mp & 1);
-  NK_TRY(cholesky_aug_pair_async(ctx, sys, 2));
+  NK_TRY(cholesky_aug_pair_async(ctx, sys, 2, nullptr, -1, FlowOpts(), ctx->ev[EV_TRSM_END]));
   tr.mark("cholesky + solves issued");
   return NK_OK;
 }
@@ -703,6 +754,10 @@
   stats->ms_solve = ev_ms(ctx, EV_SOLVE_BEGIN, EV_FIT_END);
   stats->sqrt_iters = it;
   stats->sqrt_residual = resid;
+  stats->sqrt_schedule = sqrt_mode;
+  stats->ms_prep_wait = sqrt_mode == SQRT_EARLY ? std::max(0.0, (double)ev_ms(ctx, EV_KMAT_DONE, EV_SQRT_PREPARED)) : 0.0;
+  stats->ms_tail_sqrt = ev_ms(ctx, EV_GRAM_DONE, EV_SQRT_END);
+  stats->ms_tail_trsm = ev_ms(ctx, EV_GRAM_DONE, EV_TRSM_END);
   const double ne = (double)n_eff;
   const double t128 = 128.0;
   auto tiles = [&](double v) { return std::ceil(v / t128); };
@@ -722,6 +777,7 @@
 
 int NystromFit::run() {
   NK_TRY(validate());
+  plan_sqrt_schedule();
   NK_HIP(hipEventRecord(ctx->ev[EV_FIT_BEGIN], ctx->stream));
   NK_TRY(make_winv(ctx, kd, d, mdl->winv));
   if (mode != FIT_SOLVE) NK_TRY(stage_rows());
@@ -732,12 +788,13 @@
     NK_TRY(load_gram());
   } else {
     NK_TRY(prepare_features());
+    if (sqrt_mode != SQRT_LATE) NK_TRY(begin_sqrt_prep());
     NK_TRY(run_passes());
   }
   NK_HIP(hipEventRecord(ctx->ev[EV_GRAM_DONE], ctx->stream));
   if (mode == FIT_GRAM) return return_gram();
 
-  NK_HIP(hipEventRecord(ctx->ev_fork, ctx->stream));
+  if (!fork_in_gram) NK_HIP(hipEventRecord(ctx->ev_fork, ctx->stream));
   tr.mark("gram issued");
   NK_TRY(queue_sqrt_prep());
   NK_TRY(assemble_and_factor());
diff --git a/nys_koop_lqr_amd/csrc/nk_gemm_tn.hip b/nys_koop_lqr_amd/csrc/nk_gemm_tn.hip
--- a/nys_koop_lqr_amd/csrc/nk_gemm_tn.hip
+++ b/nys_koop_lqr_amd/csrc/nk_gemm_tn.hip
@@ -458,7 +458,7 @@
 }
 
 int launch_gemm_tn_multi(nk_ctx* ctx, const TnProblem* probs, int nprob, int64_t K, int splitk, float* ms_kernel,
-                         bool sync_timing, const TnSkip* skip) {
+                         bool sync_timing, const TnSkip* skip, hipEvent_t product_done) {
   NK_REQUIRE(nprob >= 1 && nprob <= TN_MAXP, "gemm_tn_multi: 1..4 problems");
   NK_REQUIRE(K >= 0 && K < (1LL << 31), "gemm_tn_multi: K out of range");
   NK_TRY(tn_ensure_zero_page(ctx));
@@ -562,6 +562,7 @@
     hipLaunchKernelGGL(gemm_tn_f64_kernel<0>, dim3((unsigned)(ntiles * splitk)), dim3(256), TN_LDS_BYTES, ctx->stream, P);
   NK_HIP(hipGetLastError());
   if (ms_kernel) NK_HIP(hipEventRecord(ctx->ev[EV_GEMM_T1], ctx->stream));
+  if (product_done) NK_HIP(hipEventRecord(product_done, ctx->stream));
   if (splitk > 1) {
     hipLaunchKernelGGL(gemm_tn_reduce_kernel, dim3((unsigned)ntiles * RPARTS), dim3(256), 0, ctx->stream, R);
     NK_HIP(hipGetLastError());
diff --git a/nys_koop_lqr_amd/csrc/nk_linalg.hip b/nys_koop_lqr_amd/csrc/nk_linalg.hip
--- a/nys_koop_lqr_amd/csrc/nk_linalg.hip
+++ b/nys_koop_lqr_amd/csrc/nk_linalg.hip
@@ -668,7 +668,8 @@
   return cholesky_check_pair(ctx, sys, nsys);
 }
 
-int cholesky_aug_pair_async(nk_ctx* ctx, const CholSys* sys, int nsys, hipEvent_t pause, int pause_step) {
+int cholesky_aug_pair_async(nk_ctx* ctx, const CholSys* sys, int nsys, hipEvent_t pause, int pause_step, const FlowOpts& flow,
+                            hipEvent_t end) {
   constexpr int NB = CHOL_NB;
   NK_REQUIRE(nsys >= 1 && nsys <= 2, "cholesky_aug_pair: 1..2 systems");
   NK_TRY(reset_pivots(ctx));
@@ -679,8 +680,9 @@
   }
   if (!ctx->chol_flow_off && mmin >= 256 && !ctx_recording(ctx) && chol_flow_enabled()) {
     if (pause != nullptr && pause_step >= 0 && pause_step < nblk) NK_HIP(hipStreamWaitEvent(ctx->stream, pause, 0));
-    NK_TRY(cholesky_flow_pair(ctx, sys, nsys));
+    NK_TRY(cholesky_flow_pair(ctx, sys, nsys, flow));
     NK_TRY(launch_trsm_right_lower_pair(ctx, sys, nsys));
+    if (end) NK_HIP(hipEventRecord(end, ctx->stream));
     return NK_OK;
   }
   static const bool la_env = getenv("NYSKOOP_CHOL_LOOKAHEAD") && getenv("NYSKOOP_CHOL_LOOKAHEAD")[0] == '1';
@@ -786,6 +788,7 @@
   }
   if (lookahead && last_rest) NK_HIP(hipStreamWaitEvent(s_chain, last_rest, 0));
   NK_TRY(launch_trsm_right_lower_pair(ctx, sys, nsys));
+  if (end) NK_HIP(hipEventRecord(end, ctx->stream));
   return NK_OK;
 }
 
@@ -893,6 +896,11 @@
 NK_BATCHED_TWIN(tri_scale_both_kernel, (256), const double*, int64_t, int, const double*, double*, double*)
 
 int sqrtm_prepare(nk_ctx* ctx, const double* P, int64_t ldp, int m, SqrtPlan* plan) {
+  NK_TRY(sqrtm_prepare_begin(ctx, P, ldp, m, plan));
+  return sqrtm_prepare_factor(ctx, plan);
+}
+
+int sqrtm_prepare_begin(nk_ctx* ctx, const double* P, int64_t ldp, int m, SqrtPlan* plan) {
   plan->P = P; plan->ldp = ldp; plan->m = m;
   plan->mark = arena_mark(ctx);
   const size_t mm = (size_t)m * m;
@@ -920,10 +928,16 @@
   NK_TRY(launch_copy2d(ctx, P, ldp, plan->W, m, m, m));
   NK_TRY(launch_fill(ctx, E, m, m, m, 0.0));
   NK_TRY(launch_add_diag(ctx, E, m, m, 1.0));
+  return NK_OK;
+}
+
+int sqrtm_prepare_factor(nk_ctx* ctx, SqrtPlan* plan) {
+  const int m = plan->m;
+  double* E = plan->W + (size_t)m * m;
   CholSys y;
   y.P = plan->W; y.ldp = m; y.m = m; y.extra = m; y.backward = false; y.Linv = plan->Linv;
-  NK_TRY(cholesky_aug_pair_async(ctx, &y, 1, plan->pause_event, plan->pause_step));
-  {
+  NK_TRY(cholesky_aug_pair_async(ctx, &y, 1, plan->pause_event, plan->pause_step, plan->flow));
+  if (!plan->skip_linv_norm) {
     const ArenaMark mk = arena_mark(ctx);
     const int blocks = grid_for((int64_t)m * m, ctx->num_cu);
     double* partial = nullptr;
@@ -963,8 +977,11 @@
                                 double* Sinv, const double* Q_even = nullptr, const double* select = nullptr) {
   const int m = plan->m;
   const size_t mm = (size_t)m * m;
-  double* Linv_full = scratch;
-  NK_TRY(launch_transpose(ctx, plan->W + mm, m, Linv_full, m, m, m));
+  const double* Linv_full = plan->Linv_full;
+  if (!Linv_full) {
+    NK_TRY(launch_transpose(ctx, plan->W + mm, m, scratch, m, m, m));
+    Linv_full = scratch;
+  }
   TnProblem pr[2];
   pr[0].A = Q; pr[0].B = plan->X0; pr[0].C = S; pr[0].lda = pr[0].ldb = pr[0].ldc = m; pr[0].M = pr[0].N = m;
   pr[0].alpha = std::sqrt(c);
@@ -984,16 +1001,119 @@
   return NK_OK;
 }
 
+static inline double ns_p3(double x) { return x * (3.0 - x) * (3.0 - x) * 0.25; }
+static inline void ns_advance(double s2, double& a, double& b) {
+  const double xa = s2 * a, xb = s2 * b;
+  const double lo = ns_p3(xa) < ns_p3(xb) ? ns_p3(xa) : ns_p3(xb);
+  b = (xa <= 1.0 && xb >= 1.0) ? 1.0 : (ns_p3(xa) > ns_p3(xb) ? ns_p3(xa) : ns_p3(xb));
+  a = lo < b ? lo : b;
+}
+static double ns_bulk_lower(double c, double sumsq, double trace, int m) {
+  double a_lo = 1.0;
+  const double fro = std::sqrt(sumsq) / c, tr = trace / c;
+  const double lam1 = fro < 1.0 ? fro : 1.0;
+  if (m > 1 && tr > lam1) a_lo = (tr - lam1) / (m - 1);
+  else a_lo = tr / m * 1e-2;
+  if (!(a_lo > 0.0) || !std::isfinite(a_lo)) a_lo = 1e-12;
+  if (a_lo > 1.0) a_lo = 1.0;
+  return a_lo;
+}
+static int ns_alloc(nk_ctx* ctx, SqrtPlan* plan) {
+  const size_t mm = (size_t)plan->m * plan->m;
+  NK_TRY(arena_alloc_t(ctx, mm, &plan->Xa));
+  NK_TRY(arena_alloc_t(ctx, mm, &plan->Xta));
+  NK_TRY(arena_alloc_t(ctx, mm, &plan->Xb));
+  NK_TRY(arena_alloc_t(ctx, mm, &plan->Xtb));
+  NK_TRY(arena_alloc_t(ctx, mm, &plan->M));
+  NK_TRY(arena_alloc_t(ctx, mm, &plan->T));
+  return NK_OK;
+}
+static bool ns_fast(const SqrtPlan* plan) {
+  const int m = plan->m;
+  TnProblem probe;
+  probe.A = plan->Xta; probe.B = plan->T; probe.C = plan->Xa; probe.lda = probe.ldb = probe.ldc = m; probe.M = probe.N = m;
+  return m >= 128 && tn_fast_ok(probe);
+}
+static int ns_schedule(SqrtPlan* plan, double c, double a_lo, double linv2) {
+  int kmax = 0;
+  double ta = plan->early ? 0.9 * plan->lambda_min_hint / c : 0.5 / (c * linv2), tb = 1.0;
+  if (ta > a_lo) ta = a_lo;
+  const double a_sched = std::pow(a_lo, 0.8) * std::pow(ta, 0.2);
+  double a = a_sched, b = 1.0;
+  int kconv = -1;
+  for (int k = 0; k < 100; ++k) {
+    if (kconv < 0 && ta >= 1.0 - 1e-9 && tb <= 1.0 + 1e-9) kconv = k;
+    plan->checks[k] = a >= 0.5;
+    const double s2 = 3.0 / (a + std::sqrt(a * b) + b);
+    plan->s2s[k] = s2;
+    ns_advance(s2, a, b);
+    ns_advance(s2, ta, tb);
+    if (kconv >= 0 && k >= kconv + 1) { kmax = k + 1; break; }
+  }
+  if (kmax == 0) kmax = 100;
+  return kmax;
+}
+static int ns_queue_setup(nk_ctx* ctx, SqrtPlan* plan) {
+  const int m = plan->m;
+  const double c = plan->c;
+  double* state = plan->d_sc + 5;
+  NK_HIP(hipMemsetAsync(state, 0, 3 * sizeof(double), ctx->stream));
+  {
+    const size_t mt = (size_t)(m + 127) / 128;
+    const size_t need = std::max((size_t)grid_for((int64_t)m * m, ctx->num_cu), mt * (mt + 1) / 2 * 8);
+    NK_TRY(arena_alloc_t(ctx, need, &plan->rpart));
+  }
+  TnSkip skip;
+  skip.state = state; skip.step = 0;
+  NK_TRY(launch_transpose(ctx, plan->P, plan->ldp, plan->M, m, m, m));
+  NK_TRY(launch_axpby2d(ctx, 0.5 / c, plan->P, plan->ldp, 0.5 / c, plan->M, m, m, m));
+  if (plan->checks[0]) {
+    const int npart = grid_for((int64_t)m * m, ctx->num_cu);
+    hipLaunchKernelGGL(frob_mi_partial_kernel, dim3(npart), dim3(256), 0, ctx->stream, plan->M, (int64_t)m, m, plan->rpart,
+                       skip.state, skip.step);
+    hipLaunchKernelGGL(ns_flag_kernel, dim3(1), dim3(256), 0, ctx->stream, plan->rpart, npart, m, 0, state);
+    NK_HIP(hipGetLastError());
+  }
+  const double s2 = plan->s2s[0], sc = std::sqrt(s2);
+  NK_TRY(launch_scale_add_identity(ctx, -0.5 * s2 * sc, plan->M, m, 1.5 * sc, plan->T, m, m, &skip));
+  return NK_OK;
+}
+
+static bool ns_trim_first_product() {
+  const char* e = getenv("NYSKOOP_SQRT_TRIM0");
+  return !(e && e[0] == '0');
+}
+
+int sqrtm_setup(nk_ctx* ctx, SqrtPlan* plan, bool with_linv) {
+  const int m = plan->m;
+  plan->hoisted = false;
+  plan->early = plan->lambda_min_hint > 0.0 && m >= 1024 && m % 2 == 0;
+  if (!plan->early) return NK_OK;
+  NK_HIP(hipEventSynchronize(ctx->ev[EV_SQRT_SCALARS]));
+  const double c = ctx->h_scalars[12], sumsq = ctx->h_scalars[13], trace = ctx->h_scalars[14];
+  if (!(c > 0.0) || !std::isfinite(c)) return NK_OK;
+  NK_TRY(ns_alloc(ctx, plan));
+  if (!ns_fast(plan)) return NK_OK;
+  plan->c = c;
+  plan->kmax = ns_schedule(plan, c, ns_bulk_lower(c, sumsq, trace, m), 0.0);
+  NK_TRY(ns_queue_setup(ctx, plan));
+  if (with_linv) {
+    NK_TRY(arena_alloc_t(ctx, (size_t)m * m, &plan->Linv_full));
+    NK_TRY(launch_transpose(ctx, plan->W + (size_t)m * m, m, plan->Linv_full, m, m, m));
+  }
+  plan->hoisted = true;
+  return NK_OK;
+}
+
 int sqrtm_finish(nk_ctx* ctx, SqrtPlan* plan, double* S, double* Sinv) {
   const int m = plan->m;
-  const size_t mm = (size_t)m * m;
   const int ib = info_base(ctx);
   plan->deferred = false;
   plan->info_slot = ib;
   plan->rc = NK_OK; plan->iters = 0; plan->resid = 0.0;
   plan->early = plan->lambda_min_hint > 0.0 && m >= 1024 && m % 2 == 0;
-  double c, sumsq, trace, linv2 = 0.0;
-  if (plan->early) {
+  double c = plan->c, sumsq = 0.0, trace = 0.0, linv2 = 0.0;
+  if (plan->early && !plan->hoisted) {
     NK_HIP(hipEventSynchronize(ctx->ev[EV_SQRT_SCALARS]));
     c = ctx->h_scalars[12]; sumsq = ctx->h_scalars[13]; trace = ctx->h_scalars[14];
     if (!(c > 0.0) || !std::isfinite(c)) plan->early = false;
@@ -1020,37 +1140,18 @@
     plan->rc = sqrtm_spd_coupled(ctx, plan->P, plan->ldp, m, S, Sinv, &plan->iters, &plan->resid);
     return plan->rc;
   }
-  double *Xa = nullptr, *Xta = nullptr, *Xb = nullptr, *Xtb = nullptr, *M = nullptr, *T = nullptr;
-  NK_TRY(arena_alloc_t(ctx, mm, &Xa));
-  NK_TRY(arena_alloc_t(ctx, mm, &Xta));
-  NK_TRY(arena_alloc_t(ctx, mm, &Xb));
-  NK_TRY(arena_alloc_t(ctx, mm, &Xtb));
-  NK_TRY(arena_alloc_t(ctx, mm, &M));
-  NK_TRY(arena_alloc_t(ctx, mm, &T));
-  double a_lo = 1.0, b_hi = 1.0;
-  {
-    const double fro = std::sqrt(sumsq) / c, tr = trace / c;
-    const double lam1 = fro < 1.0 ? fro : 1.0;
-    if (m > 1 && tr > lam1) a_lo = (tr - lam1) / (m - 1);
-    else a_lo = tr / m * 1e-2;
-    if (!(a_lo > 0.0) || !std::isfinite(a_lo)) a_lo = 1e-12;
-    if (a_lo > 1.0) a_lo = 1.0;
-  }
-  auto p3 = [](double x) { return x * (3.0 - x) * (3.0 - x) * 0.25; };
-  auto advance = [&](double s2, double& a, double& b) {
-    const double xa = s2 * a, xb = s2 * b;
-    const double lo = p3(xa) < p3(xb) ? p3(xa) : p3(xb);
-    b = (xa <= 1.0 && xb >= 1.0) ? 1.0 : (p3(xa) > p3(xb) ? p3(xa) : p3(xb));
-    a = lo < b ? lo : b;
-  };
+  if (!plan->hoisted) {
+    NK_TRY(ns_alloc(ctx, plan));
+    plan->c = c;
+  }
+  double *Xa = plan->Xa, *Xta = plan->Xta, *Xb = plan->Xb, *Xtb = plan->Xtb, *M = plan->M, *T = plan->T;
+  double a_lo = plan->hoisted ? 1.0 : ns_bulk_lower(c, sumsq, trace, m), b_hi = 1.0;
   GemmOpts sym;
   sym.tri = TRI_UPPER_MIRROR;
   const double* X = plan->X0;
   const double* Xt = plan->X0t;
   double *Xn = Xa, *Xtn = Xta;
-  TnProblem probe;
-  probe.A = Xta; probe.B = T; probe.C = Xa; probe.lda = probe.ldb = probe.ldc = m; probe.M = probe.N = m;
-  const bool fast = m >= 128 && tn_fast_ok(probe);
+  const bool fast = ns_fast(plan);
   const bool queued = fast && m >= 1024;
   if (plan->early && !queued) {
     set_error("sqrtm: internal: early queueing needs the LDS-DMA path");
@@ -1058,42 +1159,20 @@
   }
 
   if (queued) {
-    double s2s[128];
-    bool checks[128];
-    int kmax = 0;
-    {
-      double ta = plan->early ? 0.9 * plan->lambda_min_hint / c : 0.5 / (c * linv2), tb = 1.0;
-      if (ta > a_lo) ta = a_lo;
-      const double a_sched = std::pow(a_lo, 0.8) * std::pow(ta, 0.2);
-      double a = a_sched, b = b_hi;
-      int kconv = -1;
-      for (int k = 0; k < 100; ++k) {
-        if (kconv < 0 && ta >= 1.0 - 1e-9 && tb <= 1.0 + 1e-9) kconv = k;
-        checks[k] = a >= 0.5;
-        const double s2 = 3.0 / (a + std::sqrt(a * b) + b);
-        s2s[k] = s2;
-        advance(s2, a, b);
-        advance(s2, ta, tb);
-        if (kconv >= 0 && k >= kconv + 1) { kmax = k + 1; break; }
-      }
-      if (kmax == 0) kmax = 100;
-    }
+    if (!plan->hoisted) {
+      plan->kmax = ns_schedule(plan, c, a_lo, linv2);
+      NK_TRY(ns_queue_setup(ctx, plan));
+    }
+    const int kmax = plan->kmax;
+    const double* s2s = plan->s2s;
+    const bool* checks = plan->checks;
     double* state = plan->d_sc + 5;
-    NK_HIP(hipMemsetAsync(state, 0, 3 * sizeof(double), ctx->stream));
-    double* rpart = nullptr;
-    {
-      const size_t mt = (size_t)(m + 127) / 128;
-      const size_t need = std::max((size_t)grid_for((int64_t)m * m, ctx->num_cu), mt * (mt + 1) / 2 * 8);
-      NK_TRY(arena_alloc_t(ctx, need, &rpart));
-    }
+    double* rpart = plan->rpart;
     for (int k = 0; k < kmax; ++k) {
       TnSkip skip;
       skip.state = state; skip.step = k;
-      int npart = 0;
-      if (k == 0) {
-        NK_TRY(launch_transpose(ctx, plan->P, plan->ldp, M, m, m, m));
-        NK_TRY(launch_axpby2d(ctx, 0.5 / c, plan->P, plan->ldp, 0.5 / c, M, m, m, m));
-      } else {
+      if (k > 0) {
+        int npart = 0;
         const double s2k = s2s[k], sck = std::sqrt(s2k);
         TnProblem pm;
         pm.A = X; pm.B = X; pm.C = M; pm.lda = pm.ldb = pm.ldc = m; pm.M = pm.N = m; pm.tri = TRI_UPPER_MIRROR;
@@ -1101,22 +1180,19 @@
         TnSkip skip_m = skip;
         skip_m.resid_partials = rpart; skip_m.resid_count = &npart;
         NK_TRY(launch_gemm_tn_multi(ctx, &pm, 1, m, 0, nullptr, true, &skip_m));
-      }
-      if (checks[k]) {
-        if (npart == 0) {
-          npart = grid_for((int64_t)m * m, ctx->num_cu);
-          hipLaunchKernelGGL(frob_mi_partial_kernel, dim3(npart), dim3(256), 0, ctx->stream, M, (int64_t)m, m, rpart,
-                             skip.state, skip.step);
+        if (checks[k]) {
+          if (npart == 0) {
+            npart = grid_for((int64_t)m * m, ctx->num_cu);
+            hipLaunchKernelGGL(frob_mi_partial_kernel, dim3(npart), dim3(256), 0, ctx->stream, M, (int64_t)m, m, rpart,
+                               skip.state, skip.step);
+          }
+          hipLaunchKernelGGL(ns_flag_kernel, dim3(1), dim3(256), 0, ctx->stream, rpart, npart, m, k, state);
+          NK_HIP(hipGetLastError());
         }
-        hipLaunchKernelGGL(ns_flag_kernel, dim3(1), dim3(256), 0, ctx->stream, rpart, npart, m, k, state);
-        NK_HIP(hipGetLastError());
-      }
-      if (k == 0) {
-        const double s2 = s2s[0], sc = std::sqrt(s2);
-        NK_TRY(launch_scale_add_identity(ctx, -0.5 * s2 * sc, M, m, 1.5 * sc, T, m, m, &skip));
       }
       TnProblem pr;
       pr.A = Xt; pr.B = T; pr.C = Xn; pr.lda = pr.ldb = pr.ldc = m; pr.M = pr.N = m; pr.Ct = Xtn; pr.ldct = m;
+      if (k == 0 && ns_trim_first_product()) pr.ktrim = KTRIM_A_LOWER;
       NK_TRY(launch_gemm_tn_multi(ctx, &pr, 1, m, 1, nullptr, true, &skip));
       X = Xn; Xt = Xtn;
       Xn = (Xn == Xa) ? Xb : Xa;
@@ -1127,7 +1203,6 @@
     if (plan->early)
       NK_HIP(hipMemcpyAsync(ctx->h_info + ib, ctx->d_info + ib, sizeof(int), hipMemcpyDeviceToHost, ctx->stream));
     plan->deferred = true;
-    plan->kmax = kmax;
     arena_release(ctx, plan->mark);
     return NK_OK;
   }
@@ -1151,7 +1226,7 @@
     }
     const double s2 = 3.0 / (a_lo + std::sqrt(a_lo * b_hi) + b_hi);
     const double sc = std::sqrt(s2);
-    advance(s2, a_lo, b_hi);
+    ns_advance(s2, a_lo, b_hi);
     NK_TRY(launch_scale_add_identity(ctx, -0.5 * s2 * sc, M, m, 1.5 * sc, T, m, m));
     if (fast) {
       TnProblem pr;
```

Result: no change. 24.64 (-0.4%).
